# Boese0601/Dyadic-Interaction-Modeling

Hardware: AMD Instinct MI355X
Metric: listener clips/sec (T=300, EMOCA-56) (higher is better)
Workload: dtype bf16; 1 GPU; C3: B=256/GPU synthetic dyad clips, T=300, SLMFT.forward(mode='val'): listener VQ encode + encoder + 299-step AR decode (top-k 52 sampling) + VQ decode; global_batch=256, seq_len=300, gather=tokens+coeffs, gather_bytes_per_rank=17452032

## Files before the change

### dyadic-interaction-modeling_amd/csrc/common.hpp

```cpp
#pragma once
#include <hip/hip_runtime.h>
#include <stdint.h>
#include <stdio.h>
#include <string.h>
#include <string>

#include "../../include/dimx.h"

namespace dimx {

void set_error(const char* fmt, ...);
const char* get_error();

#define DIMX_HIP(expr)                                                                       \
    do {                                                                                     \
        hipError_t _e = (expr);                                                              \
        if (_e != hipSuccess) {                                                              \
            dimx::set_error("%s:%d: %s -> %s", __FILE__, __LINE__, #expr, hipGetErrorString(_e)); \
            return DIMX_ERR_HIP;                                                             \
        }                                                                                    \
    } while (0)

#define DIMX_REQUIRE(cond, code, ...)       \
    do {                                    \
// ... 75 lines not shown

template <int CTRL> __device__ __forceinline__ float dpp_f32(float v) {
    return __builtin_bit_cast(float, __builtin_amdgcn_update_dpp(0, __builtin_bit_cast(int, v), CTRL, 0xF, 0xF, true));
}
template <int CTRL> __device__ __forceinline__ int dpp_i32(int v) { return __builtin_amdgcn_update_dpp(0, v, CTRL, 0xF, 0xF, true); }
constexpr int DPP_XOR1 = 0xB1, DPP_XOR2 = 0x4E, DPP_HALF_MIRROR = 0x141, DPP_ROW_MIRROR = 0x140;
__device__ __forceinline__ float lane_f32(float v, int lane) {
    return __builtin_bit_cast(float, __builtin_amdgcn_readlane(__builtin_bit_cast(int, v), lane));
}
__device__ __forceinline__ int wave_lane() { return (int)__builtin_amdgcn_mbcnt_hi(~0u, __builtin_amdgcn_mbcnt_lo(~0u, 0u)); }
template <int O> __device__ __forceinline__ int xor_lane_i32(int v) {
    static_assert(O == 1 || O == 2 || O == 4 || O == 8 || O == 16 || O == 32, "xor distance");
    if constexpr (O == 1) {
        return __builtin_amdgcn_update_dpp(0, v, 0xB1, 0xF, 0xF, false);
    } else if constexpr (O == 2) {
        return __builtin_amdgcn_update_dpp(0, v, 0x4E, 0xF, 0xF, false);
    } else if constexpr (O == 4) {
        const int r = __builtin_amdgcn_update_dpp(0, v, 0x104, 0xF, 0x5, false);
        return __builtin_amdgcn_update_dpp(r, v, 0x114, 0xF, 0xA, false);
    } else if constexpr (O == 8) {
        return __builtin_amdgcn_update_dpp(0, v, 0x128, 0xF, 0xF, false);
    } else if constexpr (O == 16) {
        const auto r = __builtin_amdgcn_permlane16_swap((unsigned)v, (unsigned)v, false, false);
        return ((wave_lane() >> 4) & 1) ? (int)r[0] : (int)r[1];
    } else {
        const auto r = __builtin_amdgcn_permlane32_swap((unsigned)v, (unsigned)v, false, false);
        return wave_lane() >= 32 ? (int)r[0] : (int)r[1];
    }
}
template <int O> __device__ __forceinline__ float xor_lane_f32(float v) {
    return __builtin_bit_cast(float, xor_lane_i32<O>(__builtin_bit_cast(int, v)));
}

__device__ __forceinline__ float group8_sum(float v) {
    v += dpp_f32<DPP_XOR1>(v);
    v += dpp_f32<DPP_XOR2>(v);
    v += dpp_f32<DPP_HALF_MIRROR>(v);
    return v;
}
__device__ __forceinline__ float row16_sum(float v) {
    v = group8_sum(v);
    v += dpp_f32<DPP_ROW_MIRROR>(v);
    return v;
}
__device__ __forceinline__ void wave_argmax(float& v, int& i) {
#define DIMX_ARGMAX_STEP(OV, OI)                          \
    do {                                                  \
        const float ov_ = (OV);                           \
        const int oi_ = (OI);                             \
        if (ov_ > v || (ov_ == v && oi_ < i)) {           \
            v = ov_;                                      \
            i = oi_;                                      \
        }                                                 \
    } while (0)
    DIMX_ARGMAX_STEP(dpp_f32<DPP_XOR1>(v), dpp_i32<DPP_XOR1>(i));
    DIMX_ARGMAX_STEP(dpp_f32<DPP_XOR2>(v), dpp_i32<DPP_XOR2>(i));
    DIMX_ARGMAX_STEP(dpp_f32<DPP_HALF_MIRROR>(v), dpp_i32<DPP_HALF_MIRROR>(i));
    DIMX_ARGMAX_STEP(dpp_f32<DPP_ROW_MIRROR>(v), dpp_i32<DPP_ROW_MIRROR>(i));
    DIMX_ARGMAX_STEP(xor_lane_f32<16>(v), xor_lane_i32<16>(i));
    DIMX_ARGMAX_STEP(xor_lane_f32<32>(v), xor_lane_i32<32>(i));
#undef DIMX_ARGMAX_STEP
}
__device__ __forceinline__ float wave_max(float v) {
    v = fmaxf(v, dpp_f32<DPP_XOR1>(v));
    v = fmaxf(v, dpp_f32<DPP_XOR2>(v));
    v = fmaxf(v, dpp_f32<DPP_HALF_MIRROR>(v));
    v = fmaxf(v, dpp_f32<DPP_ROW_MIRROR>(v));
    return fmaxf(fmaxf(lane_f32(v, 0), lane_f32(v, 16)), fmaxf(lane_f32(v, 32), lane_f32(v, 48)));
}
__device__ __forceinline__ float wave_sum(float v) {
    v += xor_lane_f32<32>(v);
    v += xor_lane_f32<16>(v);
    v += xor_lane_f32<8>(v);
    v += xor_lane_f32<4>(v);
    v += xor_lane_f32<2>(v);
    v += xor_lane_f32<1>(v);
    return v;
}
__device__ __forceinline__ float wave_sum_fast(float v) {
    v = row16_sum(v);
    return (lane_f32(v, 0) + lane_f32(v, 16)) + (lane_f32(v, 32) + lane_f32(v, 48));
}
template <bool FAST> __device__ __forceinline__ float wave_sum_sel(float v) { return FAST ? wave_sum_fast(v) : wave_sum(v); }
template <int O> __device__ __forceinline__ double xor_lane_f64(double v) {
    const unsigned long long u = __builtin_bit_cast(unsigned long long, v);
    const unsigned lo = (unsigned)xor_lane_i32<O>((int)(unsigned)u), hi = (unsigned)xor_lane_i32<O>((int)(unsigned)(u >> 32));
    return __builtin_bit_cast(double, ((unsigned long long)hi << 32) | lo);
}
__device__ __forceinline__ double wave_sum_f64(double v) {
    v += xor_lane_f64<32>(v);
    v += xor_lane_f64<16>(v);
    v += xor_lane_f64<8>(v);
    v += xor_lane_f64<4>(v);
    v += xor_lane_f64<2>(v);
    v += xor_lane_f64<1>(v);
    return v;
}

inline int ceil_div(int a, int b) { return (a + b - 1) / b; }
inline size_t align_up(size_t x, size_t a) { return (x + a - 1) / a * a; }
inline int splitk_nonempty(int nk, int sp) {
    if (nk < 1 || sp < 1) return 1;
    if (sp > nk) sp = nk;
    return ceil_div(nk, ceil_div(nk, sp));
}

struct OutSeg {
    void* ptr;
    long sb, sh, st, sd;
    int D;
};

struct GemmArgs {
    int in_dtype, out_dtype;
    const void* A;
    int lda;
    const void* W;
    int ldw;
    int kloop;
    int M, N, K;
    int conv_T;
    const int32_t* conv_lens;
    int conv_C;
    const float* bias;
    int act;
    const float* residual;
    int ldr;
    const float* rowadd;
    int rowadd_mode;
    float rowadd_scale;
    int rowadd_off, ld_rowadd;
    int rowadd_div;
    int rowT;
    OutSeg seg[3];
    int nseg, seg_width;
    int allow_splitk;
    int splitk;
    int force_simple;
    int cfg;
    int force_splitk;
    int out_slabs;
    long slab_stride;
    int stage_out;
    const float* ln_stats;
    const float* ln_colsum;
    int ln_C;
    unsigned* ln_err;
    int w_tiled;
    const void* w3;
    long w3_plane;
    int x3_decode;
    int vt_pack4;
};

void gemm_args_init(GemmArgs& a);
void gemm_set_plain_out(GemmArgs& a, void* C, int ldc);
int launch_gemm(const GemmArgs& a, hipStream_t s);
bool gemm256_eligible(const GemmArgs& a);
int launch_gemm256(const GemmArgs& a, hipStream_t s);
int launch_gemm256_segs(const GemmArgs& a, const OutSeg* segs, int nseg, int seg_width, hipStream_t s);
bool gemm_use_x3(const GemmArgs& a);
bool gemm_x3_plan(const GemmArgs& a, int* bn_out, int* sp_out);
int launch_gemm_x3(const GemmArgs& a, hipStream_t s);
int launch_split_x3(const float* w, void* planes, size_t n, hipStream_t s);
int gemm_plan_splits(const GemmArgs& a);

int launch_layernorm(int out_dtype, const float* x, void* y, const float* gamma, const float* beta, int M,
                     int C, hipStream_t s);
int launch_add_slabs_layernorm(int out_dtype, float* x, const float* slabs, int nslab, long slab_stride, void* y,
                               const float* gamma, int M, int C, hipStream_t s);
int launch_instnorm(int out_dtype, const float* x, void* y, const int32_t* lens, int B, int T, int C,
                    hipStream_t s);

struct AttnArgs {
    int dtype;
    const void *q, *k, *vt;
    void* o;
    long q_sb, q_st, q_sh;
    long k_sb, k_st, k_sh;
    long v_sb, v_sh, v_sd;
    int v_rows;
    long v_st;
    long o_sb, o_st, o_sh;
    int B, H, Lq, Lk, D;
    float scale;
    int causal;
    const int32_t* lens;
    const uint8_t* kmask;
    int kmask_ld;
    unsigned long long* kwords;
    size_t kwords_cap;
    int kwords_ready;
};
int launch_pack_key_words(const uint8_t* kmask, int kmask_ld, const int32_t* lens, int B, int Lk, unsigned long long* words, size_t cap,
                          hipStream_t s);
int launch_attention(const AttnArgs& a, hipStream_t s);
int launch_attention_tr(const AttnArgs& a, hipStream_t s);
size_t mlp_fused_packed_bytes(int C, int F);
int mlp_fused_pack(const float* w1, const float* b1, const float* w2, int C, int F, uint16_t* out);
int launch_mlp_fused(float* x, const void* packed, const float* b2, const float* ln_g, const float* ln_b, int M, int C, int F, int act,
                     hipStream_t s);

struct DecodeAttnArgs {
    int dtype;
    const void* q;
    int q_ld;
    int q_f32;
    int nslab;
    long slab_stride;
    int force_nsplit;
    int rows_per_clip;
    const void* knew;
    const void* vnew;
    int kv_ld;
    void* kcache;
    void* vcache;
    int Tmax;
    void* out;
    int o_ld;
    int B, H;
    const int32_t* step;
    int n_keys;
    const uint8_t* kmask;
    int kmask_ld;
    float scale;
    const void* tab;
    int tab_ld, tab_koff, tab_voff, tab_rows;
    const int32_t* hist;
    int hist_ld;
    int win, lookahead;
};
int launch_decode_attn(const DecodeAttnArgs& a, hipStream_t s);

int launch_vq_argmin(const float* z, int N, const float* Et , const float* ee ,
                     int32_t* idx, float* best_d, float* margin, hipStream_t s);

struct ChainGemmDesc {
    const void* W;
    int N, K, ldw;
    int cols, rows_pad, ncb, nkt;
};
struct ChainArgs {
    int B;
    ChainGemmDesc g1;
    const void* A1;
    int lda1;
    float* xr;
    float* x;
    int C;
    const float* slabs;
    int nslab;
    long slab_stride;
    void* y;
    const float* gamma;
    ChainGemmDesc g2;
    float* out2;
    int ld_out2;
    unsigned* counters;
    unsigned* seen;
    const int32_t* step;
    unsigned* err;
    int defer;
    float* stats;
    const float* colsum2;
    int nbar;
    int fault;
    int offA1, offW1, offRed1, offA2, offW2, offRed2;
};
struct LayerChainArgs {
    int B, C;
    DecodeAttnArgs sa, ca;
    ChainGemmDesc g_so, g_cq, g_co;
    const void* o;
    int ld_o;
    float* x;
    void* y;
    float* stats;
    const float* colsum_cq;
    float* qc;
    int ld_qc;
    unsigned* counters;
    unsigned* seen;
    const int32_t* step;
    int epoch_add;
    unsigned* err;
    int fault;
    unsigned long long* prof;
    int sc_stride;
    int off_base, off_A1, off_W1, off_A2, off_W2, off_W3, off_A3;
};
bool layer_chain_supported(const LayerChainArgs& a, int cu_count);
int launch_layer_chain(const LayerChainArgs& a, hipStream_t s);
size_t chain_plan(ChainArgs& a);
bool chain_supported(const ChainArgs& a, int cu_count);
int launch_chain(const ChainArgs& a, hipStream_t s);

int launch_cast_pad(int out_dtype, const float* x, int ldx, const float* coladd, void* y, int ldy, int M, int K,
                    hipStream_t s, const uint8_t* zero_rows = nullptr);
int launch_gather_rows(int out_dtype, const float* table, int ld_table, int rows, const int32_t* idx, void* y,
                       int ldy, int M, int C, hipStream_t s);
constexpr int kLstmSave = 6;
size_t lstm_scratch_bytes(int B, int T, int In);
int lstm_layer_run(const float* x, int B, int T, int In, int H, const float* const* w_ih, const float* const* w_hh,
                   const float* const* b_ih, const float* const* b_hh, float* y, void* scratch, size_t scratch_bytes, int flags,
                   int cu_count, int* fault_count, hipStream_t st, float* save = nullptr);
size_t lstm_bwd_scratch_bytes(int B, int T);
int lstm_bwd_run(const float* dy, const float* save, const float* const* w_hh, int B, int T, float* dgates, void* scratch,
                 size_t scratch_bytes, int flags, int cu_count, int* fault_count, hipStream_t st);
int launch_context_concat(int out_dtype, const float* x_s, const float* patch, const float* audio, void* ctx,
                          int M, int dim, int dim_a, hipStream_t s);
int launch_finalize_idx(int32_t* idx, const int32_t* lens, int B, int T, int32_t pad_value, hipStream_t s,
                        int fqn = 1);
int launch_shift_tokens(const int32_t* z, int32_t* inp, int32_t* tgt, int B, int T, hipStream_t s);
int launch_ce_argmax(const float* logits, const int32_t* target, float* row_loss, int32_t* argmax_tok, int R,
                     int V, hipStream_t s);
struct SampleFilter {
    int kind = 0;
    float a = 0.f, b = 0.f;
    uint8_t* keep_out = nullptr;
};
struct SampleArgs {
    const float* logits = nullptr;
    int ld_logits = 0, R = 0, top_k = 0;
    float temperature = 0.f;
    const float* noise = nullptr;
    uint64_t seed = 0;
    const int32_t* step_dev = nullptr;
    uint64_t step_host = 0;
    int32_t* tokens = nullptr;
    int tok_ld = 0, tok_col_from_step = 0, nslab = 0;
    long slab_stride = 0;
    float* logits_out = nullptr;
    int logits_out_ld = 0, row0 = 0, rows_total = 0;
    const float* emb_table = nullptr;
    int emb_C = 0;
    float* x_next = nullptr;
    int32_t* step_rw = nullptr;
    unsigned* done_ctr = nullptr;
    const float* pos_table = nullptr;
    float pos_scale = 0.f;
    int pos_rows = 0;
    const int32_t* dev_params = nullptr;
    void* y_next = nullptr;
    const float* y_gamma = nullptr;
    int y_dtype = DIMX_F32;
    const float* qkv0_table = nullptr;
    float* qkv0_out = nullptr;
    int qkv0_N = 0;
    const int32_t* prompt = nullptr;
    int prompt_ld = 0, prompt_max = 0;
    const int32_t* prompt_len = nullptr;
    int prompt_div = 1;
    int32_t* epoch_rw = nullptr;
    SampleFilter filt;
    int32_t* hist = nullptr;
    int hist_ld = 0;
};
int launch_sample(const SampleArgs& a, hipStream_t s);
struct BeamSelectArgs {
    const float* logits = nullptr;
    int nslab = 1;
    long slab_stride = 0;
    int nclip = 0, W = 0;
    const int32_t* step_dev = nullptr;
    int step_host = 0;
    int32_t* step_rw = nullptr;
    unsigned* done_ctr = nullptr;
    int32_t* epoch_rw = nullptr;
    const int32_t* dev_params = nullptr;
    const int32_t* prompt = nullptr;
    int prompt_ld = 0, prompt_max = 0;
    const int32_t* prompt_len = nullptr;
    const int32_t* lens = nullptr;
    int len_off = 0;
    const int32_t* mode = nullptr;
    const int32_t* forced_tok = nullptr;
    const double* cum_in = nullptr;
    double* cum_out = nullptr;
    int32_t* parent = nullptr;
    int32_t* tokens = nullptr;
    int32_t* backptr = nullptr;
    int tok_ld = 1;
    float* logits_out = nullptr;
    const float* emb_table = nullptr;
    int emb_C = 0;
    float* x_next = nullptr;
    const float* qkv0_table = nullptr;
    float* qkv0_out = nullptr;
    int qkv0_N = 0;
};
bool beam_width_supported(int W);
int launch_beam_select(const BeamSelectArgs& a, hipStream_t s);
struct BeamReorderArgs {
// ... 37 lines not shown
```

### dyadic-interaction-modeling_amd/csrc/mlp_fused.hip

```cpp
#include "common.hpp"

namespace dimx {
namespace {

typedef unsigned u32x4_t __attribute__((ext_vector_type(4)));
typedef __attribute__((address_space(3))) void lds_void_t;
typedef const __attribute__((address_space(1))) void glb_void_t;

constexpr int kC = 384;
constexpr int kKS = kC / 16;
constexpr int kOB = kC / 32;
constexpr int kW1Frags = kKS + 1;
constexpr int kW2Frags = 2 * kOB;
constexpr int kChunkBytes = (kW1Frags + kW2Frags) * 1024;
constexpr int kStages = 3;

template <int ACT> __device__ __forceinline__ float gelu_fast(float x) {
    if (ACT == ACT_GELU_TANH) {
        const float t = x * x;
        const float p = __builtin_fmaf(t, -0.10294324f, -2.3022082f);
        const float e = __builtin_amdgcn_exp2f(x * p);
        return x * __builtin_amdgcn_rcpf(1.0f + e);
    }
    const float t = __builtin_amdgcn_rcpf(__builtin_fmaf(fabsf(x), 0.33267253f, 1.0f));
    const float poly = t * (0.1740121f + t * (-0.0479399f + t * 0.3739278f));
    const float q = poly * __builtin_amdgcn_exp2f(x * x * -0.72134752f);
    return __builtin_fmaf(-fabsf(x), q, fmaxf(x, 0.f));
}

template <int OFF> __device__ __forceinline__ void ds_read128(u32x4_t& v, unsigned addr) {
    asm volatile("ds_read_b128 %0, %1 offset:%2" : "=v"(v) : "v"(addr), "i"(OFF));
}

struct MlpArgs {
    float* x;
    const void* wp;
    const float* b2;
    const float* ln_g;
    const float* ln_b;
    int M, nchunk;
};

template <int ACT, bool BETA> __global__ __launch_bounds__(256) void mlp_fused_kernel(const MlpArgs a) {
    extern __shared__ __attribute__((aligned(1024))) unsigned char smem[];
    const int tid = threadIdx.x, wave = __builtin_amdgcn_readfirstlane(tid >> 6), lane = tid & 63, hf = lane >> 5, l31 = lane & 31;
    const int row = blockIdx.x * 128 + wave * 32 + l31;
    const int rowc = row < a.M ? row : a.M - 1;
    const unsigned lds0 = (unsigned)(size_t)(lds_void_t*)smem;
    const unsigned char* wp = (const unsigned char*)a.wp;

    unsigned char* const ring1 = smem;
    unsigned char* const ring2 = smem + kStages * kW1Frags * 1024;
    const unsigned char* const wlane = wp + lane * 16;
    auto issue_piece = [&](int j, int chunk1, int slot1, int chunk2, int slot2) {
        if (j < 6) {
            const int p = wave + 4 * j;
            __builtin_amdgcn_global_load_lds((glb_void_t*)(wlane + (size_t)chunk1 * kChunkBytes + (size_t)p * 1024),
                                             (lds_void_t*)(ring1 + slot1 * (kW1Frags * 1024) + p * 1024), 16, 0, 0);
        } else if (j < 12) {
            const int p = wave + 4 * (j - 6);
            __builtin_amdgcn_global_load_lds((glb_void_t*)(wlane + (size_t)chunk2 * kChunkBytes + (size_t)(kW1Frags + p) * 1024),
                                             (lds_void_t*)(ring2 + slot2 * (kW2Frags * 1024) + p * 1024), 16, 0, 0);
        } else if (wave == 0) {
            __builtin_amdgcn_global_load_lds((glb_void_t*)(wlane + (size_t)chunk1 * kChunkBytes + (size_t)(kW1Frags - 1) * 1024),
                                             (lds_void_t*)(ring1 + slot1 * (kW1Frags * 1024) + (kW1Frags - 1) * 1024), 16, 0, 0);
        }
    };
    const int nch = a.nchunk;
    auto wrap = [&](int c) { return c < nch ? c : (c - nch < nch ? c - nch : 0); };
    auto issue_preloop = [&]() {
#pragma unroll
        for (int j = 0; j < 13; ++j) issue_piece(j, 0, 0, 0, 0);
#pragma unroll
        for (int j = 0; j < 13; ++j) issue_piece(j, wrap(1), 1, wrap(1), 1);
#pragma unroll
        for (int j = 0; j < 13; ++j)
            if (j < 6 || j == 12) issue_piece(j, wrap(2), 2, 0, 0);
    };
    issue_preloop();

    bf16x8_t xb[kKS + 1];
    f32x16_t o[kOB];
    {
        const float* xr = a.x + (size_t)rowc * kC + 8 * hf;
        f32x4_t v[kKS][2];
#pragma unroll
        for (int s = 0; s < kKS; ++s) {
            v[s][0] = *(const f32x4_t*)(xr + 16 * s);
            v[s][1] = *(const f32x4_t*)(xr + 16 * s + 4);
        }
        float s1 = 0.f;
#pragma unroll
        for (int s = 0; s < kKS; ++s)
#pragma unroll
            for (int j = 0; j < 4; ++j) s1 += v[s][0][j] + v[s][1][j];
        s1 += __shfl_xor(s1, 32);
        const float mean = s1 * (1.0f / kC);
        float s2 = 0.f;
#pragma unroll
        for (int s = 0; s < kKS; ++s)
#pragma unroll
            for (int j = 0; j < 4; ++j) {
                const float d0 = v[s][0][j] - mean, d1 = v[s][1][j] - mean;
                s2 += d0 * d0 + d1 * d1;
            }
        s2 += __shfl_xor(s2, 32);
        const float rstd = rsqrtf(s2 * (1.0f / kC) + 1e-5f);
        const float* g = a.ln_g + 8 * hf;
        const float* be = a.ln_b + 8 * hf;
#pragma unroll
        for (int s = 0; s < kKS; ++s) {
            const f32x4_t g0 = *(const f32x4_t*)(g + 16 * s), g1 = *(const f32x4_t*)(g + 16 * s + 4);
            f32x4_t b0 = {0.f, 0.f, 0.f, 0.f}, b1 = {0.f, 0.f, 0.f, 0.f};
            if (BETA) {
                b0 = *(const f32x4_t*)(be + 16 * s);
                b1 = *(const f32x4_t*)(be + 16 * s + 4);
            }
            const f32x4_t v0 = v[s][0], v1 = v[s][1];
            uint32_t w[4];
#pragma unroll
            for (int j = 0; j < 2; ++j) {
                w[j] = pack_bf16x2((v0[2 * j] - mean) * rstd * g0[2 * j] + b0[2 * j], (v0[2 * j + 1] - mean) * rstd * g0[2 * j + 1] + b0[2 * j + 1]);
                w[2 + j] = pack_bf16x2((v1[2 * j] - mean) * rstd * g1[2 * j] + b1[2 * j], (v1[2 * j + 1] - mean) * rstd * g1[2 * j + 1] + b1[2 * j + 1]);
            }
            const u32x4_t u = {w[0], w[1], w[2], w[3]};
            xb[s] = __builtin_bit_cast(bf16x8_t, u);
// ... 18 lines not shown
        const unsigned base = rd1 + slot * (kW1Frags * 1024);
#pragma unroll
        for (int r = 0; r < 16; ++r) h[r] = 0.f;
        u32x4_t fr[2][5];
#pragma unroll
        for (int q = 0; q < 5; ++q) asm volatile("ds_read_b128 %0, %1 offset:%2" : "=v"(fr[0][q]) : "v"(base), "i"(q * 1024));
#pragma unroll
        for (int g = 0; g < 5; ++g) {
            if (g + 1 < 5) {
#pragma unroll
                for (int q = 0; q < 5; ++q)
                    asm volatile("ds_read_b128 %0, %1 offset:%2" : "=v"(fr[(g + 1) & 1][q]) : "v"(base), "i"(((g + 1) * 5 + q) * 1024));
                asm volatile("s_waitcnt lgkmcnt(5)" ::: "memory");
            } else {
                asm volatile("s_waitcnt lgkmcnt(0)" ::: "memory");
            }
            __builtin_amdgcn_sched_barrier(0);
#pragma unroll
            for (int q = 0; q < 5; ++q)
                h = __builtin_amdgcn_mfma_f32_32x32x16_bf16(__builtin_bit_cast(bf16x8_t, fr[g & 1][q]), xb[g * 5 + q], h, 0, 0, 0);
        }
    };
    auto gelu_pair = [&](const f32x16_t& h, int r) { return pack_bf16x2(gelu_fast<ACT>(h[2 * r]), gelu_fast<ACT>(h[2 * r + 1])); };

    f32x16_t h_mid, h_next;
    uint32_t hbc[8], hbn[8];
    asm volatile("s_waitcnt vmcnt(0)" ::: "memory");
    __builtin_amdgcn_s_barrier();
    gemm1(0, h_next);
#pragma unroll
    for (int r = 0; r < 8; ++r) hbc[r] = gelu_pair(h_next, r);
    gemm1(1, h_mid);

    int s0 = 0, s2 = 2;
    for (int c = 0; c < nch; ++c) {
        asm volatile("s_waitcnt vmcnt(6)" ::: "memory");
        __builtin_amdgcn_s_barrier();
        const int cw1 = wrap(c + 3), cw2 = wrap(c + 2);
        const unsigned b1 = rd1 + s2 * (kW1Frags * 1024);
        const unsigned b2 = rd2 + s0 * (kW2Frags * 1024);
#pragma unroll
        for (int r = 0; r < 16; ++r) h_next[r] = 0.f;
        u32x4_t fr[3][4], fbias;
        asm volatile("ds_read_b128 %0, %1 offset:%2" : "=v"(fbias) : "v"(b1), "i"(kKS * 1024));
#pragma unroll
        for (int gg = 0; gg < 2; ++gg)
#pragma unroll
            for (int q = 0; q < 2; ++q) {
                asm volatile("ds_read_b128 %0, %1 offset:%2" : "=v"(fr[gg][q]) : "v"(b1), "i"((2 * gg + q) * 1024));
                asm volatile("ds_read_b128 %0, %1 offset:%2" : "=v"(fr[gg][2 + q]) : "v"(b2), "i"((2 * gg + q) * 1024));
            }
        issue_piece(12, cw1, s0, cw2, s2);
#pragma unroll
        for (int g = 0; g < kOB; ++g) {
            if (g + 2 < kOB) {
#pragma unroll
                for (int q = 0; q < 2; ++q) {
                    asm volatile("ds_read_b128 %0, %1 offset:%2" : "=v"(fr[(g + 2) % 3][q]) : "v"(b1), "i"((2 * (g + 2) + q) * 1024));
                    asm volatile("ds_read_b128 %0, %1 offset:%2" : "=v"(fr[(g + 2) % 3][2 + q]) : "v"(b2), "i"((2 * (g + 2) + q) * 1024));
                }
                asm volatile("s_waitcnt lgkmcnt(8)" ::: "memory");
            } else if (g + 1 < kOB) {
                asm volatile("s_waitcnt lgkmcnt(4)" ::: "memory");
            } else {
                asm volatile("s_waitcnt lgkmcnt(0)" ::: "memory");
            }
            __builtin_amdgcn_sched_barrier(0);
            const u32x4_t c0 = {hbc[0], hbc[1], hbc[2], hbc[3]}, c1v = {hbc[4], hbc[5], hbc[6], hbc[7]};
            if (g == 0) h_next = __builtin_amdgcn_mfma_f32_32x32x16_bf16(__builtin_bit_cast(bf16x8_t, fbias), xb[kKS], h_next, 0, 0, 0);
            h_next = __builtin_amdgcn_mfma_f32_32x32x16_bf16(__builtin_bit_cast(bf16x8_t, fr[g % 3][0]), xb[2 * g], h_next, 0, 0, 0);
            h_next = __builtin_amdgcn_mfma_f32_32x32x16_bf16(__builtin_bit_cast(bf16x8_t, fr[g % 3][1]), xb[2 * g + 1], h_next, 0, 0, 0);
            issue_piece(g, cw1, s0, cw2, s2);
            o[g] = __builtin_amdgcn_mfma_f32_32x32x16_bf16(__builtin_bit_cast(bf16x8_t, fr[g % 3][2]), __builtin_bit_cast(bf16x8_t, c0), o[g], 0, 0, 0);
            o[g] = __builtin_amdgcn_mfma_f32_32x32x16_bf16(__builtin_bit_cast(bf16x8_t, fr[g % 3][3]), __builtin_bit_cast(bf16x8_t, c1v), o[g], 0, 0, 0);
            if (g >= 2 && g < 10) hbn[g - 2] = gelu_pair(h_mid, g - 2);
        }
#pragma unroll
        for (int r = 0; r < 8; ++r) hbc[r] = hbn[r];
        h_mid = h_next;
        s0 = s0 == 2 ? 0 : s0 + 1;
        s2 = s2 == 2 ? 0 : s2 + 1;
    }

    if (row < a.M) {
        float* xr = a.x + (size_t)row * kC + 4 * hf;
#pragma unroll
        for (int ob = 0; ob < kOB; ++ob)
#pragma unroll
            for (int q = 0; q < 4; ++q) {
                float* p = xr + 32 * ob + 8 * q;
                f32x4_t v = {0.f, 0.f, 0.f, 0.f};
                v = *(const f32x4_t*)p;
#pragma unroll
                for (int t = 0; t < 4; ++t) v[t] += o[ob][4 * q + t];
                *(f32x4_t*)p = v;
            }
    }
}

}

size_t mlp_fused_packed_bytes(int C, int F) { return (C == kC && F % 32 == 0) ? (size_t)(F / 32) * kChunkBytes : 0; }

int mlp_fused_pack(const float* w1, const float* b1, const float* w2, int C, int F, uint16_t* out) {
    DIMX_REQUIRE(C == kC && F % 32 == 0, DIMX_ERR_ARG, "mlp_fused_pack: C = %d F = %d not supported", C, F);
    auto bf = [](uint16_t b) {
        const uint32_t u = (uint32_t)b << 16;
        float f;
        memcpy(&f, &u, 4);
        return f;
    };
    for (int c = 0; c < F / 32; ++c) {
        uint16_t* img = out + (size_t)c * (kChunkBytes / 2);
        for (int s = 0; s < kW1Frags; ++s)
            for (int l = 0; l < 64; ++l)
                for (int j = 0; j < 8; ++j) {
                    const int h = 32 * c + (l & 31), half = l >> 5;
                    uint16_t v = 0;
                    if (s < kKS) {
                        v = host_f32_to_bf16(w1[(size_t)h * C + 16 * s + 8 * half + j]);
                    } else if (half == 0 && j < 2) {
                        const uint16_t hi = host_f32_to_bf16(b1 ? b1[h] : 0.f);
                        v = j == 0 ? hi : host_f32_to_bf16((b1 ? b1[h] : 0.f) - bf(hi));
                    }
                    img[(size_t)s * 512 + l * 8 + j] = v;
                }
        for (int ob = 0; ob < kOB; ++ob)
            for (int s2 = 0; s2 < 2; ++s2)
                for (int l = 0; l < 64; ++l)
                    for (int j = 0; j < 8; ++j) {
                        const int o = 32 * ob + (l & 31), half = l >> 5;
                        const int hid = 32 * c + (2 * s2 + j / 4) * 8 + 4 * half + j % 4;
                        img[(size_t)(kW1Frags + 2 * ob + s2) * 512 + l * 8 + j] = host_f32_to_bf16(w2[(size_t)o * F + hid]);
                    }
    }
    return DIMX_OK;
}

int launch_mlp_fused(float* x, const void* packed, const float* b2, const float* ln_g, const float* ln_b, int M, int C, int F, int act,
                     hipStream_t s) {
    DIMX_REQUIRE(x && packed && b2 && ln_g && M > 0, DIMX_ERR_ARG, "mlp_fused: null argument");
    DIMX_REQUIRE(C == kC && F % 32 == 0 && (act == ACT_GELU_TANH || act == ACT_GELU_ERF), DIMX_ERR_ARG, "mlp_fused: C = %d F = %d act = %d", C, F, act);
    DIMX_REQUIRE(((uintptr_t)x % 16) == 0 && ((uintptr_t)packed % 16) == 0 && ((uintptr_t)b2 % 16) == 0 && ((uintptr_t)ln_g % 16) == 0 &&
                     (!ln_b || ((uintptr_t)ln_b % 16) == 0),
                 DIMX_ERR_ARG, "mlp_fused: operands must be 16-byte aligned");
    MlpArgs a;
    a.x = x; a.wp = packed; a.b2 = b2; a.ln_g = ln_g; a.ln_b = ln_b; a.M = M; a.nchunk = F / 32;
    DIMX_REQUIRE(a.nchunk >= 3, DIMX_ERR_ARG, "mlp_fused: F = %d is too small for the three-deep pipeline", F);
    const size_t lds = (size_t)kStages * kChunkBytes;
    const dim3 grid((M + 127) / 128);
#define MLP_LAUNCH(A, B)                                                                                                              \
    do {                                                                                                                              \
                             \
        DIMX_HIP(hipFuncSetAttribute((const void*)mlp_fused_kernel<A, B>, hipFuncAttributeMaxDynamicSharedMemorySize, (int)lds)); \
        hipLaunchKernelGGL((mlp_fused_kernel<A, B>), grid, dim3(256), lds, s, a);                                                     \
    } while (0)
    if (act == ACT_GELU_TANH) {
        if (ln_b) MLP_LAUNCH(ACT_GELU_TANH, true); else MLP_LAUNCH(ACT_GELU_TANH, false);
    } else {
        if (ln_b) MLP_LAUNCH(ACT_GELU_ERF, true); else MLP_LAUNCH(ACT_GELU_ERF, false);
    }
#undef MLP_LAUNCH
    DIMX_HIP(hipGetLastError());
    return DIMX_OK;
}

}
```

### dyadic-interaction-modeling_amd/csrc/model.hip

```cpp
#include <stdarg.h>
#include <stdlib.h>
#include <set>

#include "model.hpp"

namespace dimx {

static thread_local char g_err[1024] = "";
void set_error(const char* fmt, ...) {
    va_list ap;
    va_start(ap, fmt);
    vsnprintf(g_err, sizeof(g_err), fmt, ap);
    va_end(ap);
}
const char* get_error() { return g_err; }

static std::string vq_prefix(int which) { return which == 0 ? "speaker_vq." : "listener_vq."; }

struct KeySpec {
    std::string name;
    std::vector<int64_t> shape;
};

static void vq_keys(const dimx_dims& d, int which, std::vector<KeySpec>& out) {
// ... 567 lines not shown

static bool qkv_row_v(int at, int D) {
    return at == DIMX_BF16 && D <= 64;
}

static void set_qkv_out(GemmArgs& g, void* q, void* k, void* vt, int T, int H, int D, int Tp, bool rowv = false) {
    const int segw = H * D;
    g.rowT = T;
    g.nseg = 3;
    g.seg_width = segw;
    for (int i = 0; i < (rowv ? 3 : 2); ++i) {
        g.seg[i].ptr = i == 0 ? q : (i == 1 ? k : vt);
        g.seg[i].sb = (long)T * segw;
        g.seg[i].st = segw;
        g.seg[i].sh = D;
        g.seg[i].sd = 1;
        g.seg[i].D = D;
    }
    if (rowv) return;
    g.seg[2].ptr = vt;
    g.seg[2].sb = (long)H * D * Tp;
    g.seg[2].sh = (long)D * Tp;
    g.seg[2].sd = Tp;
    g.seg[2].st = 1;
    g.seg[2].D = D;
}

static void set_attn_packed(AttnArgs& a, int dtype, const void* q, const void* k, const void* vt, void* o, int B,
                            int H, int Lq, int Lk, int D, int Tp_k, bool rowv = false) {
    memset(&a, 0, sizeof(a));
    const int segw = H * D;
    a.dtype = dtype;
    a.q = q;
    a.k = k;
    a.vt = vt;
    a.o = o;
    a.q_sb = (long)Lq * segw;
    a.q_st = segw;
    a.q_sh = D;
    a.k_sb = (long)Lk * segw;
    a.k_st = segw;
    a.k_sh = D;
    a.v_sb = (long)H * D * Tp_k;
    a.v_sh = (long)D * Tp_k;
    a.v_sd = Tp_k;
    if (rowv) {
        a.v_rows = 1;
        a.v_sb = (long)Lk * segw;
        a.v_st = segw;
        a.v_sh = D;
    }
    a.o_sb = (long)Lq * segw;
    a.o_st = segw;
    a.o_sh = D;
    a.B = B;
    a.H = H;
    a.Lq = Lq;
    a.Lk = Lk;
    a.D = D;
}

struct BlockBufs {
    float* h;
    void *y, *q, *k, *vt, *o, *f;
    unsigned long long* kw = nullptr;
    size_t kw_cap = 0;
};

static int linear(const dimx_ctx* c, const void* A, int lda, const Linear& L, int M, int out_dtype, void* out, int ldo, hipStream_t st,
                  int act = ACT_NONE, const float* residual = nullptr) {
    GemmArgs g;
    gemm_lin(c, A, lda, L, M, g);
    g.out_dtype = out_dtype; g.act = act;
    g.residual = residual; g.ldr = residual ? ldo : 0;
    gemm_set_plain_out(g, out, ldo);
    return launch_gemm(g, st);
}
static int residual_linear(const dimx_ctx* c, const void* A, int lda, const Linear& L, int M, float* h, int ld, hipStream_t st) {
    return linear(c, A, lda, L, M, DIMX_F32, h, ld, st, ACT_NONE, h);
}

constexpr int kFusedMlpMinRows = 8192;

static int ff_sublayer(const dimx_ctx* c, const BlockBufs& b, const float* ln_g, const float* ln_b, const Linear& f1,
                       const Linear& f2, const void* mlp, int act, int M, int C, hipStream_t st) {
    if (mlp && M >= kFusedMlpMinRows) return launch_mlp_fused(b.h, mlp, f2.bias, ln_g, ln_b, M, C, f1.N, act, st);
    DIMX_TRY(launch_layernorm(c->at, b.h, b.y, ln_g, ln_b, M, C, st));
    DIMX_TRY(linear(c, b.y, C, f1, M, c->at, b.f, f1.N, st, act));
    return residual_linear(c, b.f, f1.N, f2, M, b.h, C, st);
}

static int self_attn_qkv(const dimx_ctx* c, const BlockBufs& b, const float* ln_g, const float* ln_b, const Linear& qkv, int B,
                         int T, int C, int heads, int D, AttnArgs& a, hipStream_t st) {
    const bool rowv = qkv_row_v(c->at, D);
    DIMX_TRY(launch_layernorm(c->at, b.h, b.y, ln_g, ln_b, B * T, C, st));
    GemmArgs g;
    gemm_lin(c, b.y, C, qkv, B * T, g);
    g.out_dtype = c->at;
    set_qkv_out(g, b.q, b.k, b.vt, T, heads, D, tpad(T), rowv);
    DIMX_TRY(launch_gemm(g, st));
    set_attn_packed(a, c->at, b.q, b.k, b.vt, b.o, B, heads, T, T, D, tpad(T), rowv);
    return DIMX_OK;
}

static int attn_out(const dimx_ctx* c, const BlockBufs& b, AttnArgs& a, const Linear& out, int C, hipStream_t st) {
    a.kwords = b.kw; a.kwords_cap = b.kw_cap;
    DIMX_TRY(launch_attention(a, st));
    return residual_linear(c, b.o, a.H * a.D, out, a.B * a.Lq, b.h, C, st);
}

static int cross_attn_sublayer(const dimx_ctx* c, const BlockBufs& b, const XAttn& x, AttnArgs& a, const uint8_t* ctx_mask, int C,
                               hipStream_t st, const float* v_rows = nullptr) {
    const int M = a.B * a.Lq, Tp = tpad(a.Lk);
    DIMX_TRY(launch_layernorm(c->at, b.h, b.y, x.ln_g, nullptr, M, C, st));
    DIMX_TRY(linear(c, b.y, C, x.qkv, M, c->at, b.q, a.H * a.D, st));
    if (v_rows) DIMX_TRY(launch_kv_rows_to_vt(v_rows, Tp, (float*)a.vt, Tp, a.B, a.Lk, a.H, st));
    a.scale = 1.0f / sqrtf((float)a.D); a.kmask = ctx_mask; a.kmask_ld = a.Lk;
    return attn_out(c, b, a, x.out, C, st);
}

struct VQScratch : BlockBufs {
    void *xa, *h1;
    float *conv, *z;
    int32_t* idx_tmp;
};

static void plan_vq(const dimx_ctx* c, const VQGeom& vg, Arena& ar, int B, int T, VQScratch& s) {
    const size_t M = (size_t)B * T, es = es_of(c);
    const int H = vg.hidden, I = vg.inter, Tp = tpad(T);
    s.xa = ar.take(M * (vg.in_pad > 128 ? vg.in_pad : 128) * es);
    s.h1 = ar.take(M * H * es);
    s.conv = (float*)ar.take(M * H * 4);
    s.y = ar.take(M * H * es);
    s.h = (float*)ar.take(M * H * 4);
    s.q = ar.take(M * H * es);
    s.k = ar.take(M * H * es);
    s.vt = ar.take((size_t)B * H * Tp * es);
    s.o = ar.take(M * H * es);
    s.f = ar.take(M * I * es);
    s.z = (float*)ar.take(M * vg.out_dim * 4);
    s.idx_tmp = (int32_t*)ar.take(M * vg.fqn * 4);
}

static int run_vq_blocks(const dimx_ctx* c, const VQGeom& vg, const VQBlock* blk, VQScratch& s, int B, int T,
                         const int32_t* lens, hipStream_t st) {
    const int M = B * T, Hd = vg.hidden, heads = vg.heads, D = Hd / heads;
    const float scale = 1.0f / sqrtf((float)Hd);
    for (int l = 0; l < vg.layers; ++l) {
        const VQBlock& b = blk[l];
        AttnArgs a;
        DIMX_TRY(self_attn_qkv(c, s, b.ln1_g, b.ln1_b, b.qkv, B, T, Hd, heads, D, a, st));
        a.scale = scale; a.lens = lens;
        DIMX_TRY(attn_out(c, s, a, b.out, Hd, st));
        DIMX_TRY(ff_sublayer(c, s, b.ln2_g, b.ln2_b, b.l1, b.l2, b.mlp, ACT_GELU_TANH, M, Hd, st));
    }
    return DIMX_OK;
}

static int run_vq_front(const dimx_ctx* c, const VQGeom& vg, const void* x_in, int ld_in, const Linear& conv,
                        const Linear& le, const float* pe, int pe_mode, int row_off, VQScratch& s, int B, int T,
                        const int32_t* lens, hipStream_t st, int row_div = 1) {
    const int M = B * T, Hd = vg.hidden;
    GemmArgs g;
    gemm_lin(c, x_in, ld_in, conv, M, g);
    g.conv_T = T;
    g.conv_lens = lens;
    g.conv_C = Hd;
    g.act = ACT_LEAKY;
    g.out_dtype = DIMX_F32;
    gemm_set_plain_out(g, s.conv, Hd);
    DIMX_TRY(launch_gemm(g, st));
    DIMX_TRY(launch_instnorm(c->at, s.conv, s.y, lens, B, T, Hd, st));
    gemm_lin(c, s.y, Hd, le, M, g);
    g.out_dtype = DIMX_F32;
    g.rowT = T;
    g.rowadd = pe;
    g.ld_rowadd = Hd;
    g.rowadd_mode = pe_mode == 0 ? 3 : 2;
    g.rowadd_off = pe_mode == 0 ? 0 : row_off;
    g.rowadd_div = row_div;
    gemm_set_plain_out(g, s.h, Hd);
    DIMX_TRY(launch_gemm(g, st));
    return DIMX_OK;
}

static int run_vq_encode(const dimx_ctx* c, int which, const float* x, const int32_t* lens, int B, int T, int pe_mode,
                         int row_off, VQScratch& s, float* z, int32_t* idx, hipStream_t st) {
    const VQGeom& vg = c->vqg[which];
    const VQNet& v = c->vq[which];
    const int M = B * T, Hd = vg.hidden;
    DIMX_TRY(launch_cast_pad(c->at, x, vg.in_dim, nullptr, s.xa, vg.in_pad, M, vg.in_dim, st));
    DIMX_TRY(linear(c, s.xa, vg.in_pad, v.vm, M, c->at, s.h1, Hd, st, ACT_LEAKY));
    DIMX_TRY(run_vq_front(c, vg, s.h1, Hd, v.conv, v.le, v.pe_enc, pe_mode, row_off, s, B, T, lens, st));
    DIMX_TRY(run_vq_blocks(c, vg, v.enc, s, B, T, lens, st));
    DIMX_TRY(launch_cast_pad(c->at, s.h, Hd, nullptr, s.y, Hd, M, Hd, st));
    DIMX_TRY(linear(c, s.y, Hd, v.post, M, DIMX_F32, z, vg.out_dim, st));
    DIMX_TRY(launch_vq_argmin(z, M * vg.fqn, v.Et, v.ee, idx, nullptr, nullptr, st));
    return DIMX_OK;
}

}

using namespace dimx;

extern "C" {

int dimx_version(void) { return 100; }
const char* dimx_last_error(void) { return get_error(); }

void dimx_legacy_dims(dimx_dims* d) {
    if (!d) return;
    dimx_default_dims(d);
    d->variant = 1;
    d->dim_in = 1024; d->dim = 512; d->dim_a = 0; d->enc_depth = 6; d->dec_depth = 6; d->heads = 8;
    d->max_seq_len = 1024;
    d->spk_in_dim = 824; d->spk_hidden = 768; d->spk_heads = 8; d->spk_inter = 1536; d->spk_face_quan_num = 8;
}

void dimx_default_dims(dimx_dims* d) {
    if (!d) return;
    memset(d, 0, sizeof(*d));
    d->vq_in_dim = 56; d->vq_hidden = 384; d->vq_layers = 6; d->vq_heads = 8; d->vq_inter = 1536;
    d->vq_n_embed = 512; d->vq_zdim = 128;
    d->dim_in = 56; d->dim = 384; d->dim_a = 768; d->enc_depth = 4; d->dec_depth = 4; d->heads = 12;
    d->dim_head = 64; d->num_tokens = 512; d->max_seq_len = 2048; d->ff_mult = 4;
}

int dimx_create(dimx_handle* h, int device_id, const dimx_dims* dims, int numeric_mode) {
    DIMX_REQUIRE(h, DIMX_ERR_ARG, "dimx_create: null handle pointer");
    DIMX_REQUIRE(numeric_mode == DIMX_MODE_PARITY_F32 || numeric_mode == DIMX_MODE_PERF_BF16, DIMX_ERR_ARG,
                 "dimx_create: numeric_mode %d", numeric_mode);
    dimx_dims d;
    dimx_default_dims(&d);
    if (dims) d = *dims;
    DIMX_REQUIRE(d.vq_hidden == 384 && d.vq_heads == 8 && d.vq_zdim == 128 && d.vq_n_embed == 512 && d.vq_in_dim == 56,
                 DIMX_ERR_ARG, "dimx_create: only the DIM-Listener VQ geometry (56/384/8/128/512) is built");
    if (d.variant == 0 || d.variant == 2) {
        DIMX_REQUIRE(d.dim == 384 && d.dim_a == 768 && d.dim_head == 64 && d.heads == 12 && d.num_tokens == 512 &&
                         d.vq_layers <= 8 && d.enc_depth <= 8 && d.dec_depth <= 8 && d.max_seq_len <= 2048,
                     DIMX_ERR_ARG, "dimx_create: only the SLMFT geometry (384+768, 12x64, 512 tokens) is built");
    } else {
        DIMX_REQUIRE(d.variant == 1 && d.dim == 512 && d.dim_a == 0 && d.dim_head == 64 && d.heads == 8 &&
                         d.num_tokens == 512 && d.enc_depth <= 8 && d.dec_depth <= 8 && d.max_seq_len <= 2048 &&
                         d.spk_hidden == 768 && d.spk_heads == 8 && d.spk_in_dim == 824 && d.spk_face_quan_num == 8,
                     DIMX_ERR_ARG, "dimx_create: only the legacy ListenerGenerator geometry (824/768 VQ, 512, 8x64) is built");
    }
    DIMX_REQUIRE(d.mesh_dim == 0 || (d.variant == 2 && d.mesh_dim > 0), DIMX_ERR_ARG,
                 "dimx_create: the mesh head (mesh_dim %d) belongs to a handle of variant 2", d.mesh_dim);
    int ndev = 0;
    DIMX_HIP(hipGetDeviceCount(&ndev));
    DIMX_REQUIRE(device_id >= 0 && device_id < ndev, DIMX_ERR_ARG, "dimx_create: device %d of %d", device_id, ndev);
    DIMX_HIP(hipSetDevice(device_id));
    dimx_ctx* c = new dimx_ctx();
    c->device = device_id;
    c->d = d;
    c->mode = numeric_mode;
    c->at = numeric_mode == DIMX_MODE_PERF_BF16 ? DIMX_BF16 : DIMX_F32;
    c->variant = d.variant;
    const VQGeom lvq = {d.vq_in_dim, 64, d.vq_hidden, d.vq_heads, d.vq_inter, d.vq_layers, d.vq_zdim, 1, d.vq_zdim,
                        d.vq_n_embed, true};
    c->vqg[0] = c->vqg[1] = lvq;
    if (d.variant == 1) {
        c->vqg[0] = {d.spk_in_dim, (d.spk_in_dim + 63) / 64 * 64, d.spk_hidden, d.spk_heads, d.spk_inter, d.vq_layers,
                     d.spk_face_quan_num * d.vq_zdim, d.spk_face_quan_num, d.vq_zdim, d.vq_n_embed, false};
        const int din = d.spk_face_quan_num * d.vq_zdim;
        c->encg[0] = c->encg[1] = {din, din, d.dim, d.heads, d.dim_head, d.enc_depth, d.ff_mult, 0};
        c->decg = {d.dim, d.heads, d.dim_head, d.dec_depth, d.ff_mult, 1, d.num_tokens, d.dim};
    } else {
        const int causal = d.variant == 2 ? 0 : 1, abs_pos = d.variant == 2 ? 1 : 0;
        c->encg[0] = {d.dim_in, 64, d.dim, d.heads, d.dim_head, d.enc_depth, d.ff_mult, causal};
        c->encg[1] = {d.dim, d.dim, d.dim, d.heads, d.dim_head, d.enc_depth, d.ff_mult, causal};
        c->decg = {d.dim + d.dim_a, d.heads, d.dim_head, d.dec_depth, d.ff_mult, abs_pos, d.num_tokens, d.dim + d.dim_a};
    }
    for (const auto& k : all_keys(d)) c->required.push_back(k.name);
    const char* ng = getenv("DIMX_NO_GRAPH");
    c->use_graph = (ng && ng[0] == '1') ? 0 : 1;
    const char* nc = getenv("DIMX_NO_CHAIN");
    c->use_chain = (nc && nc[0] == '1') ? 0 : 1;
    c->use_layer_chain = getenv("DIMX_NO_LAYER_CHAIN") ? 0 : 1;
    c->multi_tr = getenv("DIMX_NO_MULTI_TR") ? 0 : 1;
    c->use_qkv0_table = getenv("DIMX_NO_QKV0_TABLE") ? 0 : 1;
    c->use_kv0_table = getenv("DIMX_NO_KV0_TABLE") ? 0 : 1;
    if (getenv("DIMX_LAYER_PROF")) {
        void* p = nullptr;
        if (hipMalloc(&p, (size_t)8 * 256 * 16 * 8) == hipSuccess) {
            (void)hipMemset(p, 0, (size_t)8 * 256 * 16 * 8);
            c->layer_prof_dev = (unsigned long long*)p;
        }
    }
    if (const char* pg = getenv("DIMX_PREFILL_GROUPS")) {
        const int v = atoi(pg);
        if (v >= 1 && v <= dimx_ctx::kPreGroups) c->prefill_groups = v;
    }
    {
        int cus = 0;
        if (hipDeviceGetAttribute(&cus, hipDeviceAttributeMultiprocessorCount, device_id) == hipSuccess) c->cu_count = cus;
    }
    const char* gg = getenv("DIMX_GEN_GROUPS");
    if (gg && atoi(gg) >= 1 && atoi(gg) <= dimx_ctx::kMaxGroups) c->gen_groups = atoi(gg);
    *h = c;
    return DIMX_OK;
}

int dimx_destroy(dimx_handle h) {
    if (!h) return DIMX_OK;
    (void)hipSetDevice(h->device);
    for (int g = 0; g < dimx_ctx::kMaxGroups; ++g) {
        if (h->graph_multi[g]) (void)hipGraphExecDestroy(h->graph_multi[g]);
        if (h->graph_exec[g]) (void)hipGraphExecDestroy(h->graph_exec[g]);
        if (h->grp_stream[g]) (void)hipStreamDestroy(h->grp_stream[g]);
        if (h->ev_join[g]) (void)hipEventDestroy(h->ev_join[g]);
    }
    if (h->ev_fork) (void)hipEventDestroy(h->ev_fork);
    for (int g = 0; g < dimx_ctx::kPreGroups - 1; ++g) {
        if (h->pre_stream[g]) (void)hipStreamDestroy(h->pre_stream[g]);
        if (h->pre_join[g]) (void)hipEventDestroy(h->pre_join[g]);
    }
    if (h->pre_fork) (void)hipEventDestroy(h->pre_fork);
    if (h->cap_stream) (void)hipStreamDestroy(h->cap_stream);
    if (h->chain_err_ev) (void)hipEventDestroy(h->chain_err_ev);
    if (h->chain_err_dev) (void)hipFree(h->chain_err_dev);
    if (h->chain_stats_dev) (void)hipFree(h->chain_stats_dev);
    if (h->layer_prof_dev) (void)hipFree(h->layer_prof_dev);
    if (h->qkv0_table) (void)hipFree(h->qkv0_table);
    if (h->kv0_image) (void)hipFree(h->kv0_image);
    if (h->chain_err_host) (void)hipHostFree(h->chain_err_host);
    free_packed(h);
    train_forget(h);
    delete h;
    return DIMX_OK;
}

int dimx_numeric_mode(dimx_handle h) { return h ? h->mode : DIMX_ERR_ARG; }

int dimx_set_shard(dimx_handle h, int row_offset, int rows_total) {
    DIMX_REQUIRE(h, DIMX_ERR_ARG, "set_shard: null handle");
    DIMX_REQUIRE(row_offset >= 0 && (rows_total == 0 || rows_total > row_offset), DIMX_ERR_ARG,
                 "set_shard: row_offset %d, rows_total %d", row_offset, rows_total);
    h->shard_row_off = row_offset;
    h->shard_rows_total = rows_total;
    return DIMX_OK;
}

int dimx_begin_checkpoint(dimx_handle h) {
    DIMX_REQUIRE(h, DIMX_ERR_ARG, "dimx_begin_checkpoint: null handle");
    std::set<std::string> spec;
    for (const auto& k : all_keys(h->d)) spec.insert(k.name);
    bool dirty = false;
    for (auto it = h->host.begin(); it != h->host.end();) {
        if (!spec.count(it->first)) {
            it = h->host.erase(it);
            dirty = true;
        } else {
            ++it;
        }
    }
    if (dirty) {
        (void)hipSetDevice(h->device);
        (void)hipDeviceSynchronize();
        free_packed(h);
        h->graph_valid = false;
        h->ctx_ready = false;
    }
// ... 222 lines not shown
    s.xs = ar.take((size_t)B * T * c->encg[0].dim * es);
    s.xl = ar.take((size_t)B * T * c->encg[0].dim * es);
    s.xj = ar.take((size_t)B * 2 * T * c->encg[0].dim * es);
    s.m2 = (uint8_t*)ar.take((size_t)B * 2 * T);
}

static size_t workspace_bytes(const dimx_ctx* c, int B, int T, int S = 1) {
    Arena p(nullptr, 0);
    CtxPersist cp;
    plan_persist(c, p, B, T, cp);
    const size_t persist = align_up(p.off, 256);
    size_t scratch = 0;
    for (int w = 0; w < 2; ++w) {
        Arena a(nullptr, 0);
        VQScratch s;
        plan_vq(c, c->vqg[w], a, B, T, s);
        scratch = a.off > scratch ? a.off : scratch;
    }
    {
        Arena a(nullptr, 0);
        EncScratch s;
        plan_enc(c, a, B, T, s);
        if (c->variant == 0) a.take((size_t)B * T * c->decg.ctx_dim * es_of(c));
        if (c->variant == 1) {
            VQScratch v;
            plan_vq(c, c->vqg[0], a, B, T, v);
            a.take((size_t)B * 4);
        }
        scratch = a.off > scratch ? a.off : scratch;
    }
    if (c->variant == 2) {
        Arena a(nullptr, 0);
        SlmScratch s;
        plan_slm(c, a, B, T, s);
        scratch = a.off > scratch ? a.off : scratch;
    }
    if (c->d.mesh_dim > 0) {
        Arena a(nullptr, 0);
        MeshScratch s;
        plan_mesh(c, a, B, T, s);
        scratch = a.off > scratch ? a.off : scratch;
    }
    if (T >= 2) {
        Arena a(nullptr, 0);
        DecScratch s;
        plan_dec(c, a, B, T, s);
        scratch = a.off > scratch ? a.off : scratch;
        Arena g(nullptr, 0);
        GenScratch gs;
        plan_gen(c, g, B * S, T, gs);
        scratch = g.off > scratch ? g.off : scratch;
    }
    return persist + align_up(scratch, 256) + 4096 + 65536;
}

static size_t workspace_bytes_prompt(const dimx_ctx* c, int B, int T, int S, int P0) {
    const size_t base = workspace_bytes(c, B, T, S);
    if (P0 <= 1 || T < 2) return base;
    Arena p(nullptr, 0);
    CtxPersist cp;
    plan_persist(c, p, B, T, cp);
    Arena g(nullptr, 0);
    GenScratch gs;
    plan_gen(c, g, B * S, T, gs);
    PrefillScratch ps;
    plan_prefill(c, g, B, P0 - 1, T, ps);
    const size_t need = align_up(p.off, 256) + align_up(g.off, 256) + 4096 + 65536;
    return need > base ? need : base;
}

static int run_xenc(const dimx_ctx* c, const EncGeom& eg, const XEnc& e, const void* x_in, int ld_in, EncScratch& s,
                    int B, int T, const uint8_t* mask, int out_dtype, void* out, hipStream_t st) {
    const int M = B * T, dim = eg.dim, heads = eg.heads, D = eg.dim_head;
    GemmArgs g;
    gemm_lin(c, x_in, ld_in, e.proj_in, M, g);
    g.out_dtype = DIMX_F32;
    g.rowT = T;
    g.rowadd = e.pos_emb;
    g.ld_rowadd = dim;
    g.rowadd_mode = 1;
    g.rowadd_scale = 1.0f / sqrtf((float)dim);
    gemm_set_plain_out(g, s.h, dim);
    DIMX_TRY(launch_gemm(g, st));
    for (int l = 0; l < eg.depth; ++l) {
        AttnArgs a;
        DIMX_TRY(self_attn_qkv(c, s, e.attn[l].ln_g, nullptr, e.attn[l].qkv, B, T, dim, heads, D, a, st));
        a.scale = 1.0f / sqrtf((float)D); a.causal = eg.causal; a.kmask = mask; a.kmask_ld = T;
        DIMX_TRY(attn_out(c, s, a, e.attn[l].out, dim, st));
        DIMX_TRY(ff_sublayer(c, s, e.ff[l].ln_g, nullptr, e.ff[l].f1, e.ff[l].f2, e.ff[l].mlp, ACT_GELU_ERF, M, dim, st));
    }
    DIMX_TRY(launch_layernorm(out_dtype, s.h, out, e.final_g, nullptr, M, dim, st));
    return DIMX_OK;
}

static int check_common(dimx_handle h, int B, int T, void* ws, size_t ws_bytes, int need, int S = 1) {
    DIMX_REQUIRE(h, DIMX_ERR_ARG, "null handle");
    DIMX_REQUIRE(B >= 1 && T >= 1 && T <= h->d.max_seq_len, DIMX_ERR_ARG, "B=%d T=%d out of range (T <= %d)", B, T,
                 h->d.max_seq_len);
    DIMX_REQUIRE(ws && ((uintptr_t)ws % 256) == 0, DIMX_ERR_ARG, "workspace must be 256-byte aligned");
    const size_t need_bytes = workspace_bytes(h, B, T, S);
    DIMX_REQUIRE(ws_bytes >= need_bytes, DIMX_ERR_WORKSPACE, "workspace %zu < required %zu", ws_bytes, need_bytes);
    DIMX_HIP(hipSetDevice(h->device));
    DIMX_TRY(ensure_packed(h, need));
    return DIMX_OK;
}

int project_cross_kv(dimx_handle h, const void* ctx, const CtxPersist& cp, int B, int T, int for_generate,
                     hipStream_t st);
int legacy_encode_ctx(dimx_handle h, const float* v_speaker, const uint8_t* mask, int B, int T, int for_generate,
                      float* enc_out, float* x_speaker_out, int32_t* idx_out, void* ws, size_t ws_bytes,
                      hipStream_t st);

struct ClipGroups {
    int G;
    int b0[dimx_ctx::kPreGroups + 1];
    hipStream_t st[dimx_ctx::kPreGroups];
};
static int clip_groups_fork(dimx_handle h, int B, int T, hipStream_t st, ClipGroups& cg, bool one_group = false) {
    int G = one_group ? 1 : h->prefill_groups;
    if (G == 0) {
        const size_t rows = (size_t)B * T;
        G = rows > 196608 ? 1 : rows >= 32768 ? 4 : rows >= 16384 ? 2 : 1;
    }
    if (G > B) G = B;
    cg.G = G;
    for (int g = 0; g <= G; ++g) cg.b0[g] = (int)((long)B * g / G);
    cg.st[0] = st;
    if (G == 1) return DIMX_OK;
    {
        hipStreamCaptureStatus cs = hipStreamCaptureStatusNone;
        if (hipStreamIsCapturing(st, &cs) != hipSuccess || cs != hipStreamCaptureStatusNone) {
            (void)hipGetLastError();
            cg.G = 1;
            cg.b0[1] = B;
            return DIMX_OK;
        }
        if (hipStreamQuery(st) != hipSuccess) (void)hipStreamSynchronize(st);
        (void)hipGetLastError();
    }
    if (!h->pre_fork) DIMX_HIP(hipEventCreateWithFlags(&h->pre_fork, hipEventDisableTiming));
    DIMX_HIP(hipEventRecord(h->pre_fork, st));
    for (int g = 1; g < G; ++g) {
        if (!h->pre_stream[g - 1]) DIMX_HIP(hipStreamCreateWithFlags(&h->pre_stream[g - 1], hipStreamNonBlocking));
        if (!h->pre_join[g - 1]) DIMX_HIP(hipEventCreateWithFlags(&h->pre_join[g - 1], hipEventDisableTiming));
        cg.st[g] = h->pre_stream[g - 1];
        DIMX_HIP(hipStreamWaitEvent(cg.st[g], h->pre_fork, 0));
    }
    return DIMX_OK;
}
static int clip_groups_join(dimx_handle h, const ClipGroups& cg) {
    hipError_t bad = hipSuccess;
    for (int g = 1; g < cg.G; ++g) {
        hipError_t e = hipEventRecord(h->pre_join[g - 1], cg.st[g]);
        if (e == hipSuccess) e = hipStreamWaitEvent(cg.st[0], h->pre_join[g - 1], 0);
        if (e != hipSuccess) {
            (void)hipStreamSynchronize(cg.st[g]);
            bad = e;
        }
    }
    DIMX_HIP(bad);
    return DIMX_OK;
}

static int clip_groups_close(dimx_handle h, const ClipGroups& cg, int rc) {
    const int jrc = clip_groups_join(h, cg);
    return rc != DIMX_OK ? rc : jrc;
}

static Arena scratch_arena(const dimx_ctx* c, void* ws, size_t ws_bytes, int B, int T, CtxPersist* cp) {
    Arena p(ws, ws_bytes);
    CtxPersist tmp;
    plan_persist(c, p, B, T, cp ? *cp : tmp);
    const size_t persist = align_up(p.off, 256);
    return Arena((unsigned char*)ws + persist, ws_bytes - persist);
// ... 13 lines not shown
    return workspace_bytes(h, B, T, n_samples);
}

size_t dimx_workspace_bytes_prompt(dimx_handle h, int B, int T, int n_samples, int P0) {
    if (!h || B < 1 || T < 1 || n_samples < 1 || T > h->d.max_seq_len || P0 < 1 || P0 > (T > 1 ? T - 1 : 1)) return 0;
    return workspace_bytes_prompt(h, B, T, n_samples, P0);
}

int dimx_vq_argmin(dimx_handle h, int which, const float* z, int N, int32_t* idx, float* best_d, float* margin,
                   void* stream) {
    DIMX_REQUIRE(h && (which == 0 || which == 1), DIMX_ERR_ARG, "vq_argmin: bad handle/which");
    DIMX_HIP(hipSetDevice(h->device));
    DIMX_TRY(ensure_packed(h, which == 0 ? COMP_VQ0 : COMP_VQ1));
    return launch_vq_argmin(z, N, h->vq[which].Et, h->vq[which].ee, idx, best_d, margin, (hipStream_t)stream);
}

int dimx_vq_encode(dimx_handle h, int which, const float* x, const int32_t* lens, int B, int T, int pe_mode,
                   int batch_row_offset, int32_t pad_value, int32_t* idx, float* z_out, void* ws, size_t ws_bytes,
                   void* stream) {
    DIMX_REQUIRE(which == 0 || which == 1, DIMX_ERR_ARG, "vq_encode: which must be 0 or 1");
    DIMX_TRY(check_common(h, B, T, ws, ws_bytes, which == 0 ? COMP_VQ0 : COMP_VQ1));
    DIMX_REQUIRE(x && idx, DIMX_ERR_ARG, "vq_encode: null argument");
    DIMX_REQUIRE(pe_mode == 0 || B + batch_row_offset <= 5000, DIMX_ERR_ARG, "vq_encode: positional row out of range");
    hipStream_t st = (hipStream_t)stream;
    const VQGeom& vg = h->vqg[which];
    Arena ar = scratch_arena(h, ws, ws_bytes, B, T, nullptr);
    ClipGroups cg;
    DIMX_TRY(clip_groups_fork(h, B, T, st, cg));
    VQScratch s[dimx_ctx::kPreGroups];
    for (int g = 0; g < cg.G; ++g) plan_vq(h, vg, ar, cg.b0[g + 1] - cg.b0[g], T, s[g]);
    const int rc = [&]() -> int {
        DIMX_REQUIRE(!ar.overflow, DIMX_ERR_WORKSPACE, "vq_encode: workspace overflow");
        for (int g = 0; g < cg.G; ++g) {
            const int b0 = cg.b0[g], nb = cg.b0[g + 1] - b0;
            const size_t r0 = (size_t)b0 * T;
            DIMX_TRY(run_vq_encode(h, which, x + r0 * vg.in_dim, lens ? lens + b0 : nullptr, nb, T, pe_mode, batch_row_offset + b0, s[g],
                                   z_out ? z_out + r0 * vg.out_dim : s[g].z, idx + r0 * vg.fqn, cg.st[g]));
        }
        return DIMX_OK;
    }();
    DIMX_TRY(clip_groups_close(h, cg, rc));
    DIMX_TRY(launch_finalize_idx(idx, lens, B, T, pad_value, st, vg.fqn));
    return DIMX_OK;
}

static int vq_decode_impl(dimx_handle h, int which, const int32_t* idx, const float* z, int B, int L,
                          int batch_row_offset, int rows_per_clip, float* out, void* ws, size_t ws_bytes, void* stream) {
    DIMX_REQUIRE(which == 0 || which == 1, DIMX_ERR_ARG, "vq_decode: which must be 0 or 1");
    DIMX_TRY(check_common(h, B, L, ws, ws_bytes, which == 0 ? COMP_VQ0 : COMP_VQ1));
    DIMX_REQUIRE((idx || z) && out, DIMX_ERR_ARG, "vq_decode: null argument");
    DIMX_REQUIRE(B + batch_row_offset <= 5000 && batch_row_offset >= 0, DIMX_ERR_ARG,
                 "vq_decode: positional row %d out of range", B + batch_row_offset);
    hipStream_t st = (hipStream_t)stream;
    const VQNet& v = h->vq[which];
    const VQGeom& vg = h->vqg[which];
    DIMX_REQUIRE(vg.has_decoder, DIMX_ERR_ARG, "vq_decode: this variant's VQ-VAE %d has no decoder on the path", which);
    DIMX_REQUIRE(rows_per_clip >= 1, DIMX_ERR_ARG, "vq_decode: rows_per_clip must be >= 1");
    Arena ar = scratch_arena(h, ws, ws_bytes, B, L, nullptr);
    ClipGroups cg;
    if (rows_per_clip == 1) {
        DIMX_TRY(clip_groups_fork(h, B, L, st, cg));
    } else {
        cg.G = 1;
        cg.b0[0] = 0;
        cg.b0[1] = B;
        cg.st[0] = st;
    }
    VQScratch sg[dimx_ctx::kPreGroups];
    for (int g = 0; g < cg.G; ++g) plan_vq(h, vg, ar, cg.b0[g + 1] - cg.b0[g], L, sg[g]);
    const int Hd = vg.hidden, zd = vg.zdim;
    const int rc = [&]() -> int {
    DIMX_REQUIRE(!ar.overflow, DIMX_ERR_WORKSPACE, "vq_decode: workspace overflow");
    for (int gi = 0; gi < cg.G; ++gi) {
        VQScratch& s = sg[gi];
        hipStream_t gs = cg.st[gi];
        const int b0 = cg.b0[gi], nb = cg.b0[gi + 1] - b0, M = nb * L;
        const size_t r0 = (size_t)b0 * L;
        if (idx)
            DIMX_TRY(launch_gather_rows(h->at, v.E, zd, vg.n_embed, idx + r0, s.xa, zd, M, zd, gs));
        else
            DIMX_TRY(launch_cast_pad(h->at, z + r0 * zd, zd, nullptr, s.xa, zd, M, zd, gs));
        DIMX_TRY(linear(h, s.xa, zd, v.pre, M, h->at, s.h1, Hd, gs));
        DIMX_TRY(run_vq_front(h, vg, s.h1, Hd, v.dconv, v.dle, v.pe_dec, 1, batch_row_offset + b0, s, nb, L, nullptr, gs, rows_per_clip));
        DIMX_TRY(run_vq_blocks(h, vg, v.dec, s, nb, L, nullptr, gs));
        DIMX_TRY(launch_cast_pad(h->at, s.h, Hd, nullptr, s.y, Hd, M, Hd, gs));
        DIMX_TRY(linear(h, s.y, Hd, v.rev, M, DIMX_F32, out + r0 * vg.in_dim, vg.in_dim, gs));
    }
    return DIMX_OK;
    }();
    return clip_groups_close(h, cg, rc);
}

int dimx_vq_decode(dimx_handle h, int which, const int32_t* idx, int B, int L, int batch_row_offset, int rows_per_clip,
                   float* out, void* ws, size_t ws_bytes, void* stream) {
    DIMX_REQUIRE(idx, DIMX_ERR_ARG, "vq_decode: null argument");
    return vq_decode_impl(h, which, idx, nullptr, B, L, batch_row_offset, rows_per_clip, out, ws, ws_bytes, stream);
}

int dimx_vq_decode_latent(dimx_handle h, int which, const float* z, int B, int L, int batch_row_offset, float* out,
                          void* ws, size_t ws_bytes, void* stream) {
    DIMX_REQUIRE(z, DIMX_ERR_ARG, "vq_decode_latent: null argument");
    return vq_decode_impl(h, which, nullptr, z, B, L, batch_row_offset, 1, out, ws, ws_bytes, stream);
}

int dimx_encode_speaker(dimx_handle h, const float* v_speaker, const uint8_t* mask, int B, int T, float* x_s_out, void* ws,
                        size_t ws_bytes, void* stream) {
    DIMX_REQUIRE(h && h->variant == 0, DIMX_ERR_ARG, "encode_speaker: SLMFT variant only");
    DIMX_TRY(check_common(h, B, T, ws, ws_bytes, COMP_ENC));
    DIMX_REQUIRE(v_speaker && mask && x_s_out, DIMX_ERR_ARG, "encode_speaker: null argument");
    hipStream_t st = (hipStream_t)stream;
    Arena ar = scratch_arena(h, ws, ws_bytes, B, T, nullptr);
    EncScratch s;
    plan_enc(h, ar, B, T, s);
    DIMX_REQUIRE(!ar.overflow, DIMX_ERR_WORKSPACE, "encode_speaker: workspace overflow");
    const int M = B * T, dim = h->d.dim;
    DIMX_TRY(launch_cast_pad(h->at, v_speaker, h->d.dim_in, h->patch_s, s.xa, 64, M, h->d.dim_in, st));
    DIMX_TRY(run_xenc(h, h->encg[0], h->enc_s, s.xa, 64, s, B, T, mask, h->at, s.xa, st));
    DIMX_TRY(run_xenc(h, h->encg[1], h->enc_joint, s.xa, dim, s, B, T, mask, DIMX_F32, s.tmp, st));
    DIMX_TRY(launch_layernorm(DIMX_F32, s.tmp, x_s_out, h->norm_s_g, h->norm_s_b, M, dim, st));
    h->ctx_ready = false;
    return DIMX_OK;
}

int dimx_encode_ctx(dimx_handle h, const float* v_speaker, const float* v_audio, const uint8_t* mask, int B, int T,
                    int for_generate, float* x_s_out, void* ws, size_t ws_bytes, void* stream) {
    DIMX_REQUIRE(!h || h->variant != 2, DIMX_ERR_ARG,
                 "encode_ctx: the SLM variant builds its contexts with dimx_slm_encode + dimx_set_context");
    if (h && h->variant == 1)
        return legacy_encode_ctx(h, v_speaker, mask, B, T, for_generate, x_s_out, nullptr, nullptr, ws, ws_bytes,
                                 (hipStream_t)stream);
    DIMX_TRY(check_common(h, B, T, ws, ws_bytes, COMP_ENC | COMP_DEC));
    DIMX_REQUIRE(v_speaker && v_audio && mask, DIMX_ERR_ARG, "encode_ctx: null argument");
    hipStream_t st = (hipStream_t)stream;
    CtxPersist cp;
    Arena ar = scratch_arena(h, ws, ws_bytes, B, T, &cp);
    const int dim = h->d.dim, dim_a = h->d.dim_a;
    ClipGroups cg;
    DIMX_TRY(clip_groups_fork(h, B, T, st, cg, h->decg.ctx_dim < h->encg[0].in_pad));
    EncScratch sg[dimx_ctx::kPreGroups];
    void* xa_all = nullptr;
    const size_t xa_row = (size_t)h->decg.ctx_dim * es_of(h);
    if (cg.G > 1) xa_all = ar.take((size_t)B * T * xa_row);
    for (int g = 0; g < cg.G; ++g) {
        plan_enc(h, ar, cg.b0[g + 1] - cg.b0[g], T, sg[g]);
        if (cg.G > 1) sg[g].xa = (unsigned char*)xa_all + (size_t)cg.b0[g] * T * xa_row;
    }
    const int grc = [&]() -> int {
    DIMX_REQUIRE(!ar.overflow, DIMX_ERR_WORKSPACE, "encode_ctx: workspace overflow");
    for (int gi = 0; gi < cg.G; ++gi) {
        EncScratch& s = sg[gi];
        hipStream_t gs = cg.st[gi];
        const int b0 = cg.b0[gi], nb = cg.b0[gi + 1] - b0, M = nb * T;
        const size_t r0 = (size_t)b0 * T;
        const uint8_t* gmask = mask + r0;
        DIMX_TRY(launch_cast_pad(h->at, v_speaker + r0 * h->d.dim_in, h->d.dim_in, h->patch_s, s.xa, 64, M, h->d.dim_in, gs));
        DIMX_TRY(run_xenc(h, h->encg[0], h->enc_s, s.xa, 64, s, nb, T, gmask, h->at, s.xa, gs));
        DIMX_TRY(run_xenc(h, h->encg[1], h->enc_joint, s.xa, dim, s, nb, T, gmask, DIMX_F32, s.tmp, gs));
        float* x_s = x_s_out ? x_s_out + r0 * dim : (float*)s.h;
        DIMX_TRY(launch_layernorm(DIMX_F32, s.tmp, x_s, h->norm_s_g, h->norm_s_b, M, dim, gs));
        DIMX_TRY(launch_context_concat(h->at, x_s, h->patch_dec_s, v_audio + r0 * dim_a, s.xa, M, dim, dim_a, gs));
    }
    return DIMX_OK;
    }();
    DIMX_TRY(clip_groups_close(h, cg, grc));
    DIMX_TRY(project_cross_kv(h, sg[0].xa, cp, B, T, for_generate, st));
    h->ctx_ready = true;
    h->ctx_B = B;
    h->ctx_T = T;
    h->ctx_for_generate = for_generate ? 1 : 0;
    h->ctx_ws = ws;
    return DIMX_OK;
}

int dimx_legacy_speaker_features(dimx_handle h, const float* v_speaker, const uint8_t* mask, int B, int T,
                                 float* x_speaker_out, int32_t* idx_out, void* ws, size_t ws_bytes, void* stream) {
    DIMX_REQUIRE(h && h->variant == 1, DIMX_ERR_ARG, "legacy_speaker_features: handle is not the legacy variant");
    DIMX_REQUIRE(x_speaker_out || idx_out, DIMX_ERR_ARG, "legacy_speaker_features: no output requested");
    return legacy_encode_ctx(h, v_speaker, mask, B, T, -1, nullptr, x_speaker_out, idx_out, ws, ws_bytes,
                             (hipStream_t)stream);
}

int dimx_slm_encode(dimx_handle h, const float* v_speaker, const float* v_listener, const uint8_t* mask,
                    const uint8_t* mask_speaker, const uint8_t* mask_listener, int B, int T, float* x_s, float* x_l,
                    float* x_joint, void* ws, size_t ws_bytes, void* stream) {
    DIMX_REQUIRE(h && h->variant == 2, DIMX_ERR_ARG, "slm_encode: handle is not the SLM variant");
    DIMX_TRY(check_common(h, B, T, ws, ws_bytes, COMP_ENC));
    DIMX_REQUIRE(2 * T <= h->d.max_seq_len, DIMX_ERR_ARG, "slm_encode: 2T=%d exceeds max_seq_len", 2 * T);
    DIMX_REQUIRE(v_speaker && v_listener && mask && x_s && x_l && x_joint, DIMX_ERR_ARG, "slm_encode: null argument");
    hipStream_t st = (hipStream_t)stream;
    Arena ar = scratch_arena(h, ws, ws_bytes, B, T, nullptr);
    SlmScratch s;
    plan_slm(h, ar, B, T, s);
    DIMX_REQUIRE(!ar.overflow, DIMX_ERR_WORKSPACE, "slm_encode: workspace overflow");
    const int M = B * T, dim = h->encg[0].dim;
    const size_t es = es_of(h), rowb = (size_t)T * dim * es;
    const EncGeom& e0 = h->encg[0];
    const EncGeom& e1 = h->encg[1];
    DIMX_TRY(launch_cast_pad(h->at, v_speaker, h->d.dim_in, h->patch_s, s.e.xa, e0.in_pad, M, h->d.dim_in, st, mask_speaker));
    DIMX_TRY(run_xenc(h, e0, h->enc_s, s.e.xa, e0.in_pad, s.e, B, T, mask, h->at, s.xs, st));
    DIMX_TRY(launch_cast_pad(h->at, v_listener, h->d.dim_in, h->patch_l, s.e.xa, e0.in_pad, M, h->d.dim_in, st, mask_listener));
    DIMX_TRY(run_xenc(h, e0, h->enc_l, s.e.xa, e0.in_pad, s.e, B, T, mask, h->at, s.xl, st));
    DIMX_HIP(hipMemcpy2DAsync(s.xj, 2 * rowb, s.xs, rowb, rowb, B, hipMemcpyDeviceToDevice, st));
    DIMX_HIP(hipMemcpy2DAsync((unsigned char*)s.xj + rowb, 2 * rowb, s.xl, rowb, rowb, B, hipMemcpyDeviceToDevice, st));
    DIMX_HIP(hipMemcpy2DAsync(s.m2, 2 * T, mask, T, T, B, hipMemcpyDeviceToDevice, st));
    DIMX_HIP(hipMemcpy2DAsync(s.m2 + T, 2 * T, mask, T, T, B, hipMemcpyDeviceToDevice, st));
    DIMX_TRY(run_xenc(h, e1, h->enc_joint, s.xj, dim, s.e, B, 2 * T, s.m2, DIMX_F32, s.e.tmp, st));
    DIMX_TRY(launch_layernorm(DIMX_F32, s.e.tmp, x_joint, h->norm_j_g, h->norm_j_b, 2 * M, dim, st));
    DIMX_TRY(run_xenc(h, e1, h->enc_joint, s.xl, dim, s.e, B, T, mask, DIMX_F32, s.e.tmp, st));
    DIMX_TRY(launch_layernorm(DIMX_F32, s.e.tmp, x_l, h->norm_l_g, h->norm_l_b, M, dim, st));
    DIMX_TRY(run_xenc(h, e1, h->enc_joint, s.xs, dim, s.e, B, T, mask, DIMX_F32, s.e.tmp, st));
    DIMX_TRY(launch_layernorm(DIMX_F32, s.e.tmp, x_s, h->norm_s_g, h->norm_s_b, M, dim, st));
    h->ctx_ready = false;
    return DIMX_OK;
}

int dimx_set_context(dimx_handle h, const float* x, int ldx_rows, int which_patch, const float* v_audio, int B, int T,
                     int for_generate, void* ws, size_t ws_bytes, void* stream) {
    DIMX_REQUIRE(h && h->variant != 1, DIMX_ERR_ARG, "set_context: not available for the legacy variant");
    DIMX_TRY(check_common(h, B, T, ws, ws_bytes, COMP_ENC | COMP_DEC));
    DIMX_REQUIRE(x && v_audio && (which_patch == 0 || (which_patch == 1 && h->variant == 2)) && ldx_rows >= T,
                 DIMX_ERR_ARG, "set_context: bad argument");
    hipStream_t st = (hipStream_t)stream;
    CtxPersist cp;
    Arena ar = scratch_arena(h, ws, ws_bytes, B, T, &cp);
    EncScratch s;
    plan_enc(h, ar, B, T, s);
    DIMX_REQUIRE(!ar.overflow, DIMX_ERR_WORKSPACE, "set_context: workspace overflow");
    const int M = B * T, dim = h->d.dim, dim_a = h->d.dim_a;
    const float* xr = x;
    if (ldx_rows != T) {
        DIMX_HIP(hipMemcpy2DAsync(s.h, (size_t)T * dim * 4, x, (size_t)ldx_rows * dim * 4, (size_t)T * dim * 4, B,
                                  hipMemcpyDeviceToDevice, st));
        xr = s.h;
    }
    DIMX_TRY(launch_context_concat(h->at, xr, which_patch ? h->patch_dec_l : h->patch_dec_s, v_audio, s.xa, M, dim, dim_a, st));
    DIMX_TRY(project_cross_kv(h, s.xa, cp, B, T, for_generate, st));
    h->ctx_ready = true;
    h->ctx_B = B;
    h->ctx_T = T;
    h->ctx_for_generate = for_generate ? 1 : 0;
    h->ctx_ws = ws;
    return DIMX_OK;
}
// ... 40 lines not shown
                g.seg[i].st = D;
                g.seg[i].sd = 1;
                g.seg[i].D = D;
            }
        } else {
            g.seg[0].ptr = cp.ck[l];
            g.seg[0].sb = (long)T * heads * D;
            g.seg[0].st = heads * D;
            g.seg[0].sh = D;
            g.seg[0].sd = 1;
            g.seg[0].D = D;
            g.seg[1].ptr = cp.cv[l];
            g.seg[1].sb = (long)heads * D * Tp;
            g.seg[1].sh = (long)D * Tp;
            g.seg[1].sd = Tp;
            g.seg[1].st = 1;
            g.seg[1].D = D;
        }
        DIMX_TRY(launch_gemm(g, st));
    }
    return DIMX_OK;
}

int legacy_encode_ctx(dimx_handle h, const float* v_speaker, const uint8_t* mask, int B, int T, int for_generate,
                      float* enc_out, float* x_speaker_out, int32_t* idx_out, void* ws, size_t ws_bytes,
                      hipStream_t st) {
    DIMX_TRY(check_common(h, B, T, ws, ws_bytes, for_generate < 0 ? COMP_VQ0 : (COMP_VQ0 | COMP_ENC | COMP_DEC)));
    DIMX_REQUIRE(v_speaker && mask, DIMX_ERR_ARG, "encode_ctx: null argument");
    CtxPersist cp;
    Arena ar = scratch_arena(h, ws, ws_bytes, B, T, &cp);
    EncScratch s;
    VQScratch v;
    plan_enc(h, ar, B, T, s);
    plan_vq(h, h->vqg[0], ar, B, T, v);
    int32_t* lens = (int32_t*)ar.take((size_t)B * 4);
    DIMX_REQUIRE(!ar.overflow, DIMX_ERR_WORKSPACE, "encode_ctx: workspace overflow");
    const VQGeom& vg = h->vqg[0];
    const EncGeom& eg = h->encg[0];
    const int M = B * T;
    DIMX_TRY(launch_mask_lens(mask, lens, B, T, st));
    DIMX_TRY(run_vq_encode(h, 0, v_speaker, lens, B, T, 0, 0, v, v.z, v.idx_tmp, st));
    if (idx_out) {
        DIMX_HIP(hipMemcpyAsync(idx_out, v.idx_tmp, (size_t)M * vg.fqn * 4, hipMemcpyDeviceToDevice, st));
        DIMX_TRY(launch_finalize_idx(idx_out, lens, B, T, -100, st, vg.fqn));
    }
    if (x_speaker_out)
        DIMX_TRY(launch_legacy_scramble(DIMX_F32, h->vq[0].E, v.idx_tmp, lens, x_speaker_out, B, T, vg.fqn, vg.zdim,
                                        vg.n_embed, st));
    if (for_generate < 0) return DIMX_OK;
    DIMX_TRY(launch_legacy_scramble(h->at, h->vq[0].E, v.idx_tmp, lens, s.xa, B, T, vg.fqn, vg.zdim, vg.n_embed, st));
    DIMX_TRY(run_xenc(h, eg, h->enc_s, s.xa, eg.in_pad, s, B, T, mask, h->at, s.y, st));
    if (enc_out) DIMX_TRY(launch_layernorm(DIMX_F32, s.h, enc_out, h->enc_s.final_g, nullptr, M, eg.dim, st));
    DIMX_TRY(project_cross_kv(h, s.y, cp, B, T, for_generate, st));
    h->ctx_ready = true;
    h->ctx_B = B;
    h->ctx_T = T;
    h->ctx_for_generate = for_generate ? 1 : 0;
    h->ctx_ws = ws;
    return DIMX_OK;
}

}

extern "C" {

int dimx_decode_tf(dimx_handle h, const int32_t* z_l, const uint8_t* ctx_mask, const uint8_t* kv_mask, int B, int T,
                   float* logits, float* row_loss, int32_t* argmax_tok, void* ws, size_t ws_bytes, void* stream) {
    DIMX_TRY(check_common(h, B, T, ws, ws_bytes, COMP_DEC));
    DIMX_REQUIRE(z_l && ctx_mask && logits && T >= 2, DIMX_ERR_ARG, "decode_tf: null argument or T < 2");
    DIMX_REQUIRE(h->ctx_ready && h->ctx_B == B && h->ctx_T == T && h->ctx_ws == ws && !h->ctx_for_generate,
                 DIMX_ERR_STATE, "decode_tf: call dimx_encode_ctx(for_generate=0) with the same B, T, ws first");
    hipStream_t st = (hipStream_t)stream;
    CtxPersist cp;
    Arena ar = scratch_arena(h, ws, ws_bytes, B, T, &cp);
    DecScratch s;
    plan_dec(h, ar, B, T, s);
    DIMX_REQUIRE(!ar.overflow, DIMX_ERR_WORKSPACE, "decode_tf: workspace overflow");
    const DecGeom& dg = h->decg;
    const int n = T - 1, M = B * n, DD = dg.dim, heads = dg.heads, D = dg.dim_head;
    const int Tp = tpad(T), V = dg.num_tokens;
    DIMX_TRY(launch_shift_tokens(z_l, s.inp, s.tgt, B, T, st));
    DIMX_TRY(launch_gather_rows(DIMX_F32, h->dec.tok_emb, DD, V, s.inp, s.h, DD, M, DD, st));
    if (dg.abs_pos) DIMX_TRY(launch_add_pos_rows(s.h, h->dec.pos_emb, M, n, DD, 1.0f / sqrtf((float)DD), st));
    for (int l = 0; l < dg.depth; ++l) {
        AttnArgs a;
        DIMX_TRY(self_attn_qkv(h, s, h->dec.self_[l].ln_g, nullptr, h->dec.self_[l].qkv, B, n, DD, heads, D, a, st));
        a.scale = 1.0f / sqrtf((float)D); a.causal = 1; a.kmask = kv_mask; a.kmask_ld = n;
        DIMX_TRY(attn_out(h, s, a, h->dec.self_[l].out, DD, st));
        set_attn_packed(a, h->at, s.q, cp.ck[l], cp.cv[l], s.o, B, heads, n, T, D, Tp);
        DIMX_TRY(cross_attn_sublayer(h, s, h->dec.cross[l], a, ctx_mask, DD, st));
        DIMX_TRY(ff_sublayer(h, s, h->dec.ff[l].ln_g, nullptr, h->dec.ff[l].f1, h->dec.ff[l].f2, nullptr, ACT_GELU_ERF, M, DD, st));
    }
    DIMX_TRY(launch_layernorm(h->at, s.h, s.y, h->dec.final_g, nullptr, M, DD, st));
    DIMX_TRY(linear(h, s.y, DD, h->dec.logits, M, DIMX_F32, logits, V, st));
    if (row_loss || argmax_tok) DIMX_TRY(launch_ce_argmax(logits, s.tgt, row_loss, argmax_tok, M, V, st));
    return DIMX_OK;
}

}

namespace dimx {

static void chain_desc(ChainGemmDesc& d, const Linear& L) { d.W = L.w; d.N = L.N; d.K = L.K; d.ldw = L.Kp; }

static bool gen_use_chain(dimx_handle h, int B, int S, int grp) {
    if (!h->use_chain || h->at != DIMX_BF16 || S != 1 || grp != 0 || h->gen_groups > 1 || !h->chain_err_dev) return false;
    const DecGeom& dg = h->decg;
    ChainArgs c;
    memset(&c, 0, sizeof(c));
    c.B = B;
    c.C = dg.dim;
    const XAttn& sa = h->dec.self_[0];
    const XAttn& ca = h->dec.cross[0];
    chain_desc(c.g1, sa.out);
    c.lda1 = dg.heads * dg.dim_head;
    chain_desc(c.g2, ca.qkv);
    if (!chain_supported(c, h->cu_count)) return false;
    chain_desc(c.g2, h->dec.logits);
    c.g1.W = nullptr;
    return chain_supported(c, h->cu_count) && 3 * dg.depth + 1 <= kChainSites;
}

static bool gen_multi_tr(dimx_handle h, int S) {
    return S > 1 && h->multi_tr && h->at == DIMX_BF16 && h->decg.dim_head == 64;
}

static int slab_gemm_rows(dimx_handle h, int B, hipStream_t st, const void* A, int lda, const Linear& L, float* out, long stride,
                          int* nsl) {
    GemmArgs g;
    gemm_lin(h, A, lda, L, B, g);
    g.x3_decode = 1;
    g.out_dtype = DIMX_F32;
    g.out_slabs = 1;
    static const bool f32_split = getenv("DIMX_F32_NO_SPLIT") == nullptr;
    if (f32_split) g.allow_splitk = 1;
    g.slab_stride = stride;
    gemm_set_plain_out(g, out, L.N);
    *nsl = gemm_plan_splits(g);
    g.force_splitk = *nsl;
    return launch_gemm(g, st);
}

static bool qkv0_table_supported(dimx_handle h) {
    const DecGeom& dg = h->decg;
    const int N = 3 * dg.heads * dg.dim_head;
    return h->use_qkv0_table && !dg.abs_pos && h->dec.self_[0].qkv.N == N && N % 4 == 0 && N <= 12 * 256 && dg.dim % 4 == 0 &&
           dg.dim / 2 <= 16 * 64;
}

static int qkv0_table_build(dimx_handle h, const GenScratch& s, int M, hipStream_t st, int step0 = 0) {
    const DecGeom& dg = h->decg;
    const int DD = dg.dim, V = dg.num_tokens, N = h->dec.self_[0].qkv.N;
    if (h->qkv0_table && h->qkv0_M == M && h->qkv0_at == h->at && h->qkv0_epoch == h->dec_epoch) return DIMX_OK;
    if (!h->qkv0_table) {
        DIMX_HIP(hipMalloc((void**)&h->qkv0_table, (size_t)V * N * sizeof(float)));
        h->graph_valid = false;
    }
    h->qkv0_epoch = 0;
    const int rounds = (V + M - 1) / M;
    int32_t* ids = (int32_t*)s.logits;
    DIMX_TRY(launch_iota_clamp(ids, rounds * M, V, st));
    for (int r = 0; r < rounds; ++r) {
        int ns = 0;
        DIMX_TRY(launch_embed_step(h->dec.tok_emb, DD, V, ids + (size_t)r * M, nullptr, 0, s.step, s.x, M, 1, st, nullptr, 0.f, 1, step0));
        DIMX_TRY(launch_add_slabs_layernorm(h->at, s.x, s.xr, 0, s.st_xr, s.y, h->dec.self_[0].ln_g, M, DD, st));
        DIMX_TRY(slab_gemm_rows(h, M, st, s.y, DD, h->dec.self_[0].qkv, s.qkv, s.st_qkv, &ns));
        DIMX_TRY(launch_sum_slabs_rows(s.qkv, ns, s.st_qkv, h->qkv0_table, r * M, V, M, N, st));
    }
    if (h->use_kv0_table && h->at == DIMX_BF16) {
        const int inner = N / 3;
        if (!h->kv0_image) {
// ... 240 lines not shown
                ta.kwords_ready = 1;
                DIMX_TRY(launch_attention_tr(ta, st));
                goto cross_out;
            }
            DIMX_TRY(slab_gemm(s.y, DD, h->dec.cross[l].qkv, s.qc, s0.st_qc, &ns));
        }
        ca.nslab = ns;
        DIMX_TRY(launch_decode_attn(ca, st));
    cross_out:
        if (chain) {
            DIMX_TRY(chain_site(3 * l + 1, s.o, inner, &h->dec.cross[l].out, 0, h->dec.ff[l].ln_g, nullptr, nullptr, 0));
        } else {
            DIMX_TRY(slab_gemm(s.o, inner, h->dec.cross[l].out, s.xr, s0.st_xr, &pending));
            DIMX_TRY(launch_add_slabs_layernorm(h->at, s.x, s.xr, pending, s0.st_xr, s.y, h->dec.ff[l].ln_g, B, DD, st));
        }
    feed_forward:
        gemm_lin(h, s.y, DD, defer ? h->dec.ff[l].f1_ln : h->dec.ff[l].f1, B, g);
        g.x3_decode = 1;
        if (defer) {
            g.ln_stats = h->chain_stats_dev;
            g.ln_err = h->chain_err_dev;
            g.ln_colsum = h->dec.ff[l].f1_ln_colsum;
            g.ln_C = DD;
        }
        g.out_dtype = h->at;
        g.act = ACT_GELU_ERF;
        gemm_set_plain_out(g, s.f, DD * dg.ff_mult);
        DIMX_TRY(launch_gemm(g, st));
        DIMX_TRY(slab_gemm(s.f, DD * dg.ff_mult, h->dec.ff[l].f2, s.xr, s0.st_xr, &pending));
    }
    int nlg = 0;
    if (chain && !h->dec.logits.bias) {
        DIMX_TRY(chain_site(3 * dg.depth, nullptr, 0, nullptr, pending, h->dec.final_g, &h->dec.logits, s.logits, V));
        nlg = 1;
    } else {
        DIMX_TRY(launch_add_slabs_layernorm(h->at, s.x, s.xr, pending, s0.st_xr, s.y, h->dec.final_g, B, DD, st));
        DIMX_TRY(slab_gemm(s.y, DD, h->dec.logits, s.logits, s0.st_lg, &nlg));
    }
    if (gc.beam) {
        const BeamCall& bm = *gc.beam;
        BeamSelectArgs bs;
        bs.logits = s.logits; bs.nslab = nlg; bs.slab_stride = s0.st_lg; bs.nclip = nclip; bs.W = S;
        bs.step_dev = s.step; bs.step_rw = s.step; bs.done_ctr = (unsigned*)(s.step + 8); bs.epoch_rw = s.step + 9; bs.dev_params = s.step + 2;
        bs.prompt = forced; bs.prompt_ld = pr.ld; bs.prompt_max = pr.Pmax; bs.prompt_len = forced_len;
        bs.lens = bm.lens ? bm.lens + clip0 : nullptr; bs.len_off = T - n;
        bs.cum_in = bm.cum + row0; bs.cum_out = bm.cum + row0; bs.parent = bm.parent + row0;
        bs.tokens = tokens; bs.backptr = bm.backptr ? bm.backptr + (size_t)row0 * n : nullptr; bs.tok_ld = n; bs.logits_out = logits_out;
        bs.emb_table = h->dec.tok_emb; bs.emb_C = DD; bs.x_next = s.x;
        bs.qkv0_table = gc.qkv0; bs.qkv0_out = s.qkv; bs.qkv0_N = 3 * inner;
        DIMX_TRY(launch_beam_select(bs, st));
        if (!gc.qkv0) DIMX_TRY(launch_add_slabs_layernorm(h->at, s.x, s.xr, 0, s0.st_xr, s.y, h->dec.self_[0].ln_g, B, DD, st));
        BeamReorderArgs br;
        for (int l = 0; l < dg.depth; ++l) {
            br.buf[2 * l] = boff(s0.sk[l], (size_t)heads * T * 64 * es);
            br.buf[2 * l + 1] = boff(s0.sv[l], (size_t)heads * T * 64 * es);
        }
        br.nbuf = 2 * dg.depth; br.es = (int)es; br.nclip = nclip; br.W = S; br.H = heads; br.T = T;
        br.parent = bs.parent; br.step_dev = s.step; br.step_back = 1;
        br.tokens = tokens; br.backptr = bs.backptr; br.tok_ld = n;
        return launch_beam_reorder(br, st);
    }
    SampleArgs sm;
    sm.logits = s.logits; sm.ld_logits = V; sm.R = B; sm.nslab = nlg; sm.slab_stride = s0.st_lg; sm.row0 = row0; sm.rows_total = gc.Btot;
    sm.top_k = gc.top_k; sm.noise = gc.noise; sm.filt.kind = h->filter_kind;
    sm.temperature = gc.temperature; sm.seed = gc.seed;
    sm.step_dev = s.step; sm.step_rw = s.step; sm.dev_params = s.step + 2; sm.done_ctr = (unsigned*)(s.step + 8); sm.epoch_rw = s.step + 9;
    sm.tokens = tokens; sm.tok_ld = n; sm.tok_col_from_step = 1; sm.logits_out = logits_out; sm.logits_out_ld = n;
    sm.emb_table = h->dec.tok_emb; sm.emb_C = DD; sm.x_next = s.x; sm.pos_table = pos; sm.pos_scale = pos_scale; sm.pos_rows = n;
    sm.y_next = gc.qkv0 ? nullptr : s.y; sm.y_gamma = gc.qkv0 ? nullptr : h->dec.self_[0].ln_g; sm.y_dtype = h->at;
    sm.qkv0_table = gc.qkv0; sm.qkv0_out = s.qkv; sm.qkv0_N = 3 * inner;
    if (gc.kv0) { sm.hist = s.hist; sm.hist_ld = T; }
    sm.prompt = forced; sm.prompt_ld = pr.ld; sm.prompt_max = pr.Pmax; sm.prompt_len = forced_len; sm.prompt_div = S;
    return launch_sample(sm, st);
}

static int gen_prefill(dimx_handle h, const CtxPersist& cp, const GenScratch& gs, const PrefillScratch& s, const GenPrompt& pr,
                       const uint8_t* ctx_mask, int B, int T, int S, int32_t* tokens, hipStream_t st) {
    const DecGeom& dg = h->decg;
    const int n0 = pr.step0, M = B * n0, DD = dg.dim, heads = dg.heads, D = dg.dim_head;
    const int np = tpad(n0), Tp = tpad(T), V = dg.num_tokens;
    DIMX_TRY(launch_prompt_rows(pr.tok, pr.ld, B, n0, V, S, s.inp, tokens, gen_steps(h, T), st));
    DIMX_TRY(launch_gather_rows(DIMX_F32, h->dec.tok_emb, DD, V, s.inp, s.h, DD, M, DD, st));
    const bool rowv = qkv_row_v(h->at, D);
    for (int l = 0; l < dg.depth; ++l) {
        AttnArgs a;
        DIMX_TRY(self_attn_qkv(h, s, h->dec.self_[l].ln_g, nullptr, h->dec.self_[l].qkv, B, n0, DD, heads, D, a, st));
        DIMX_TRY(launch_kv_rows_to_cache(h->at, s.k, gs.sk[l], B, n0, heads, T, S, st));
        if (rowv)
            DIMX_TRY(launch_kv_rows_to_cache(h->at, s.vt, gs.sv[l], B, n0, heads, T, S, st));
        else
            DIMX_TRY(launch_kv_vt_to_cache((const float*)s.vt, np, (float*)gs.sv[l], B, n0, heads, T, S, st));
        if (l == dg.depth - 1) break;
        a.scale = 1.0f / sqrtf((float)D); a.causal = 1;
        DIMX_TRY(attn_out(h, s, a, h->dec.self_[l].out, DD, st));
        set_attn_packed(a, h->at, s.q, cp.ck[l], rowv ? cp.cv[l] : s.cvt, s.o, B, heads, n0, T, D, Tp, rowv);
        a.k_sb = (long)heads * Tp * D; a.k_sh = (long)Tp * D; a.k_st = D;
        if (rowv) { a.v_sb = a.k_sb; a.v_sh = a.k_sh; a.v_st = D; }
        DIMX_TRY(cross_attn_sublayer(h, s, h->dec.cross[l], a, ctx_mask, DD, st, rowv ? nullptr : (const float*)cp.cv[l]));
        DIMX_TRY(ff_sublayer(h, s, h->dec.ff[l].ln_g, nullptr, h->dec.ff[l].f1, h->dec.ff[l].f2, nullptr, ACT_GELU_ERF, M, DD, st));
    }
    return DIMX_OK;
}

}

extern "C" {

static int generate_impl(dimx_handle h, const dimx::GenPrompt& pr, bool keep_prefill, const uint8_t* ctx_mask, int B, int T, int n_samples,
                         float temperature, int top_k, const float* exp_noise, uint64_t seed, int32_t* tokens,
                         float* logits_out, void* ws, size_t ws_bytes, void* stream, bool* chain_used, bool prefill_only = false,
                         const dimx::BeamCall* beam = nullptr) {
    const int32_t* start = pr.tok;
    const int S = n_samples < 1 ? 1 : n_samples;
    if (h && h->filter_kind != DIMX_FILTER_TOP_K) top_k = 0;
    DIMX_REQUIRE(S == 1 || S == 2 || S == 4 || S == 5 || S == 8 || S == 10, DIMX_ERR_ARG,
                 "generate: n_samples %d not in {1,2,4,5,8,10}", n_samples);
    DIMX_TRY(check_common(h, B, T, ws, ws_bytes, COMP_DEC, S));
    DIMX_REQUIRE(start && ctx_mask && tokens && T >= 2, DIMX_ERR_ARG, "generate: null argument or T < 2");
    DIMX_REQUIRE(h->ctx_ready && h->ctx_B == B && h->ctx_T == T && h->ctx_ws == ws && h->ctx_for_generate,
                 DIMX_ERR_STATE, "generate: call dimx_encode_ctx(for_generate=1) with the same B, T, ws first");
    hipStream_t st = (hipStream_t)stream;
    CtxPersist cp;
    Arena ar = scratch_arena(h, ws, ws_bytes, B, T, &cp);
    GenScratch s;
    const int R = B * S;
    plan_gen(h, ar, R, T, s);
    PrefillScratch ps;
    if (pr.step0 > 0) plan_prefill(h, ar, B, pr.step0, T, ps);
    DIMX_REQUIRE(!ar.overflow, DIMX_ERR_WORKSPACE, "generate: workspace overflow");
    const int n = gen_steps(h, T);
    const int nrun = n - pr.step0;
    if (h->use_chain && h->at == DIMX_BF16 && !h->chain_err_dev) {
        DIMX_HIP(hipMalloc((void**)&h->chain_err_dev, 64));
        DIMX_HIP(hipMemset(h->chain_err_dev, 0, 64));
        DIMX_HIP(hipMalloc((void**)&h->chain_stats_dev, 8 * 32 * 32 * 2 * sizeof(float)));
        DIMX_HIP(hipMemset(h->chain_stats_dev, 0, 8 * 32 * 32 * 2 * sizeof(float)));
        DIMX_HIP(hipHostMalloc((void**)&h->chain_err_host, 64, hipHostMallocDefault));
        *h->chain_err_host = 0;
        DIMX_HIP(hipEventCreateWithFlags(&h->chain_err_ev, hipEventDisableTiming));
    }
    DIMX_HIP(hipMemsetAsync(s.chain_ctr, 0, (size_t)kChainSites * kChainSiteWords * 4, st));
    DIMX_TRY(launch_gen_params(s.step, dimx_ctx::kMaxGroups, temperature, seed, h->shard_row_off * S,
                               h->shard_rows_total * S, st, pr.step0, h->filter_a, h->filter_b));
    if (gen_multi_tr(h, S)) DIMX_TRY(launch_pack_key_words(ctx_mask, T, nullptr, B, T, s.kw, s.kw_cap, st));
    if (beam) {
        DIMX_REQUIRE(h->decg.dim_head == 64 && h->decg.depth <= 8 && !h->decg.abs_pos, DIMX_ERR_ARG,
                     "generate_beam: needs 64-wide heads, at most 8 layers and a decoder without positional embedding");
        DIMX_TRY(launch_beam_init(beam->cum, beam->parent, R, S, st));
        if (beam->backptr && pr.step0 > 0)
            DIMX_HIP(hipMemset2DAsync(beam->backptr, (size_t)n * 4, 0xFF, (size_t)pr.step0 * 4, R, st));
    }
    int G = h->gen_groups < 1 ? 1 : h->gen_groups;
    if (G > B) G = B;
    if (S > 1 || beam) G = 1;
    const float* qkv0 = nullptr;
    if (G == 1 && qkv0_table_supported(h)) {
        DIMX_TRY(qkv0_table_build(h, s, R, st, pr.step0));
        qkv0 = h->qkv0_table;
    }
    const void* kv0 = nullptr;
    if (qkv0 && h->use_kv0_table && !beam && pr.step0 == 0 && pr.Pmax <= 1 && h->decg.dim_head == 64 && h->decg.num_tokens <= 512) {
        kv0 = h->at == DIMX_BF16 ? h->kv0_image : (const void*)h->qkv0_table;
        if (kv0) ++h->kv0_generations;
    }
    if (pr.step0 > 0 && !keep_prefill) {
        if (logits_out)
            DIMX_HIP(hipMemset2DAsync(logits_out, (size_t)n * h->decg.num_tokens * 4, 0, (size_t)pr.step0 * h->decg.num_tokens * 4, R, st));
        DIMX_TRY(gen_prefill(h, cp, s, ps, pr, ctx_mask, B, T, S, tokens, st));
    }
    if (prefill_only) {
        *chain_used = false;
        return DIMX_OK;
    }
    int lo[dimx_ctx::kMaxGroups + 1];
    for (int g = 0; g <= G; ++g) lo[g] = (int)((long)R * g / G);
    hipStream_t gs[dimx_ctx::kMaxGroups];
    if (G == 1) {
        gs[0] = st;
    } else {
        if (!h->ev_fork) DIMX_HIP(hipEventCreateWithFlags(&h->ev_fork, hipEventDisableTiming));
        DIMX_HIP(hipEventRecord(h->ev_fork, st));
// ... 582 lines not shown

static int op_decode_attn_ex(int dtype, const void* q, int q_ld, int q_is_f32, int nslab, long slab_stride, int self_attn, void* kcache,
                             void* vcache, void* out, int o_ld, int B, int H, int Tmax, const int32_t* step_dev, int n_keys,
                             const uint8_t* kmask, int kmask_ld, int rows_per_clip, float scale, int nsplit, int win, int lookahead,
                             void* stream) {
    const int S = rows_per_clip > 1 ? rows_per_clip : 1;
    DIMX_REQUIRE(B > 0 && H > 0 && Tmax > 0, DIMX_ERR_ARG, "op_decode_attn_ex: empty shape");
    DIMX_REQUIRE(nslab >= 1 && nslab <= 8 && (nslab == 1 || q_is_f32), DIMX_ERR_ARG, "op_decode_attn_ex: nslab=%d (1..8, > 1 for f32 q only)",
                 nslab);
    DIMX_REQUIRE(q_ld >= (self_attn ? 3 : 1) * H * 64 && o_ld >= H * 64, DIMX_ERR_ARG, "op_decode_attn_ex: q_ld=%d o_ld=%d too small",
                 q_ld, o_ld);
    DIMX_REQUIRE(nslab == 1 || slab_stride >= (long)B * S * q_ld, DIMX_ERR_ARG, "op_decode_attn_ex: slabs overlap (stride %ld)",
                 slab_stride);
    DIMX_REQUIRE(self_attn ? (step_dev != nullptr && kmask == nullptr && S == 1) : (n_keys >= 1 && n_keys <= Tmax), DIMX_ERR_ARG,
                 "op_decode_attn_ex: self form needs a step counter (no mask, one row per clip); cross form 1 <= n_keys (%d) <= Tmax",
                 n_keys);
    DIMX_REQUIRE(kmask == nullptr || kmask_ld >= n_keys, DIMX_ERR_ARG, "op_decode_attn_ex: kmask_ld=%d < n_keys=%d", kmask_ld, n_keys);
    DecodeAttnArgs a;
    memset(&a, 0, sizeof(a));
    a.dtype = dtype;
    a.q = q;
    a.q_ld = q_ld;
    a.q_f32 = q_is_f32 ? 1 : 0;
    a.nslab = nslab;
    a.slab_stride = slab_stride;
    if (self_attn) {
        const size_t es = q_is_f32 ? 4 : dtype_size(dtype);
        a.knew = (const unsigned char*)q + (size_t)H * 64 * es;
        a.vnew = (const unsigned char*)q + (size_t)2 * H * 64 * es;
        a.kv_ld = q_ld;
        a.step = step_dev;
    } else {
        a.n_keys = n_keys;
        a.kmask = kmask;
        a.kmask_ld = kmask_ld;
    }
    a.kcache = kcache;
    a.vcache = vcache;
    a.Tmax = Tmax;
    a.out = out;
    a.o_ld = o_ld;
    a.B = B;
    a.H = H;
    a.rows_per_clip = rows_per_clip;
    a.scale = scale;
    a.force_nsplit = nsplit;
    if (win) {
        a.win = 1;
        a.lookahead = lookahead;
        a.step = step_dev;
    }
    return launch_decode_attn(a, (hipStream_t)stream);
}

int dimx_op_decode_attn_ex(int dtype, const void* q, int q_ld, int q_is_f32, int nslab, long slab_stride, int self_attn, void* kcache,
                           void* vcache, void* out, int o_ld, int B, int H, int Tmax, const int32_t* step_dev, int n_keys,
                           const uint8_t* kmask, int kmask_ld, int rows_per_clip, float scale, int nsplit, void* stream) {
    return op_decode_attn_ex(dtype, q, q_ld, q_is_f32, nslab, slab_stride, self_attn, kcache, vcache, out, o_ld, B, H, Tmax, step_dev, n_keys,
                             kmask, kmask_ld, rows_per_clip, scale, nsplit, 0, 0, stream);
}

int dimx_op_decode_attn_win(int dtype, const void* q, int q_ld, int q_is_f32, int nslab, long slab_stride, void* kcache, void* vcache,
                            void* out, int o_ld, int B, int H, int Tmax, const int32_t* step_dev, int n_keys, const uint8_t* kmask,
                            int kmask_ld, int rows_per_clip, float scale, int nsplit, int lookahead, void* stream) {
    DIMX_REQUIRE(step_dev != nullptr, DIMX_ERR_ARG, "op_decode_attn_win: the windowed form needs a step counter");
    return op_decode_attn_ex(dtype, q, q_ld, q_is_f32, nslab, slab_stride, 0, kcache, vcache, out, o_ld, B, H, Tmax, step_dev, n_keys, kmask,
                             kmask_ld, rows_per_clip, scale, nsplit, 1, lookahead, stream);
}

size_t dimx_mlp_fused_packed_bytes(int C, int F) { return mlp_fused_packed_bytes(C, F); }

int dimx_mlp_fused_pack(const float* w1_host, const float* b1_host, const float* w2_host, int C, int F, void* out_host, size_t out_bytes) {
    DIMX_REQUIRE(w1_host && w2_host && out_host, DIMX_ERR_ARG, "mlp_fused_pack: null argument");
    DIMX_REQUIRE(mlp_fused_packed_bytes(C, F) > 0 && out_bytes >= mlp_fused_packed_bytes(C, F), DIMX_ERR_ARG,
                 "mlp_fused_pack: C = %d F = %d unsupported or the output buffer is too small", C, F);
    return mlp_fused_pack(w1_host, b1_host, w2_host, C, F, (uint16_t*)out_host);
}

int dimx_op_mlp_fused_packed(float* x, const void* packed, const float* b2, const float* ln_g, const float* ln_b, int M, int C, int F, int act,
                             void* stream) {
    return launch_mlp_fused(x, packed, b2, ln_g, ln_b, M, C, F, act, (hipStream_t)stream);
}

int dimx_op_mlp_fused(float* x, const float* w1_host, const float* b1_host, const float* w2_host, const float* b2, const float* ln_g,
                      const float* ln_b, int M, int C, int F, int act, void* stream) {
    DIMX_REQUIRE(x && w1_host && w2_host && b2 && ln_g && M > 0, DIMX_ERR_ARG, "op_mlp_fused: null argument");
    const size_t bytes = mlp_fused_packed_bytes(C, F);
    DIMX_REQUIRE(bytes > 0, DIMX_ERR_ARG, "op_mlp_fused: C = %d F = %d not supported", C, F);
    std::vector<uint16_t> img(bytes / 2);
    DIMX_TRY(mlp_fused_pack(w1_host, b1_host, w2_host, C, F, img.data()));
    void* p = nullptr;
    DIMX_HIP(hipMalloc(&p, bytes));
    int rc = DIMX_OK;
    if (hipMemcpy(p, img.data(), bytes, hipMemcpyHostToDevice) != hipSuccess) rc = DIMX_ERR_HIP;
    if (rc == DIMX_OK) rc = launch_mlp_fused(x, p, b2, ln_g, ln_b, M, C, F, act, (hipStream_t)stream);
    if (hipStreamSynchronize((hipStream_t)stream) != hipSuccess && rc == DIMX_OK) rc = DIMX_ERR_HIP;
    (void)hipFree(p);
    return rc;
}

int dimx_op_add_slabs_layernorm(int out_dtype, float* x, const float* slabs, int nslab, long slab_stride, void* y,
                                const float* gamma, int M, int C, void* stream) {
    return launch_add_slabs_layernorm(out_dtype, x, slabs, nslab, slab_stride, y, gamma, M, C, (hipStream_t)stream);
}

int dimx_op_chain(const void* A1, int K1, const void* W1, float* x, const float* slabs, int nslab, const float* gamma,
                  void* y, const void* W2, int N2, float* out2, int B, int C, void* scratch, void* stream) {
    DIMX_REQUIRE(scratch && x && y && gamma, DIMX_ERR_ARG, "op_chain: null argument");
    int dev = 0, cus = 0;
    DIMX_HIP(hipGetDevice(&dev));
    DIMX_HIP(hipDeviceGetAttribute(&cus, hipDeviceAttributeMultiprocessorCount, dev));
    ChainArgs c;
    memset(&c, 0, sizeof(c));
    unsigned* u = (unsigned*)scratch;
    c.B = B;
    c.C = C;
    if (W1) {
        c.g1.W = W1; c.g1.N = C; c.g1.K = K1; c.g1.ldw = K1;
        c.A1 = A1; c.lda1 = K1;
        c.xr = (float*)(u + 512);
    }
    c.x = x;
    c.slabs = slabs;
    c.nslab = nslab;
    c.slab_stride = (long)B * C;
    c.y = y;
    c.gamma = gamma;
    if (W2) {
        c.g2.W = W2; c.g2.N = N2; c.g2.K = C; c.g2.ldw = C;
        c.out2 = out2; c.ld_out2 = N2;
    }
    c.counters = u;
    c.seen = u + 256;
    c.step = (const int32_t*)(u + 128);
    c.err = u + 129;
    DIMX_REQUIRE(chain_supported(c, cus), DIMX_ERR_ARG, "op_chain: shape not supported on this device (%d CUs)", cus);
    DIMX_HIP(hipMemsetAsync(u, 0, 512 * 4, (hipStream_t)stream));
    return launch_chain(c, (hipStream_t)stream);
}

int dimx_op_chain_ln(const void* A1, int K1, const void* W1, float* x, void* y, float* stats, const void* W2s,
                     const float* colsum2, int N2, float* out2, int B, int C, void* scratch, void* stream) {
    DIMX_REQUIRE(scratch && x && y && stats && A1 && W1, DIMX_ERR_ARG, "op_chain_ln: null argument");
    int dev = 0, cus = 0;
    DIMX_HIP(hipGetDevice(&dev));
    DIMX_HIP(hipDeviceGetAttribute(&cus, hipDeviceAttributeMultiprocessorCount, dev));
    ChainArgs c;
    memset(&c, 0, sizeof(c));
    unsigned* u = (unsigned*)scratch;
    c.B = B;
    c.C = C;
    c.g1.W = W1; c.g1.N = C; c.g1.K = K1; c.g1.ldw = K1;
    c.A1 = A1; c.lda1 = K1;
    c.xr = (float*)(u + 512);
    c.x = x;
    c.y = y;
    c.gamma = (const float*)x;
    c.defer = 1;
    c.stats = stats;
    if (W2s) {
        c.g2.W = W2s; c.g2.N = N2; c.g2.K = C; c.g2.ldw = C;
        c.out2 = out2; c.ld_out2 = N2;
        c.colsum2 = colsum2;
    }
    c.counters = u;
    c.seen = u + 256;
// ... 88 lines not shown
```

### dyadic-interaction-modeling_amd/csrc/model.hpp

```cpp
#pragma once
#include <map>
#include <string>
#include <vector>

#include "common.hpp"

namespace dimx {

struct Linear {
    void* w = nullptr;
    const float* bias = nullptr;
    int N = 0, K = 0, Kp = 0;
    void* w3 = nullptr;
};

struct VQBlock {
    const float *ln1_g, *ln1_b, *ln2_g, *ln2_b;
    Linear qkv, out, l1, l2;
    const void* mlp = nullptr;
};

struct VQNet {
    Linear vm, conv, le, post;
    VQBlock enc[8];
// ... 72 lines not shown
        if (base && off > cap) overflow = true;
        return p;
    }
};

struct BeamCall {
    double* cum = nullptr;
    int32_t* parent = nullptr;
    int32_t* backptr = nullptr;
    const int32_t* lens = nullptr;
    bool operator==(const BeamCall& o) const { return cum == o.cum && parent == o.parent && backptr == o.backptr && lens == o.lens; }
};

struct GraphKey {
    void* ws;
    int B, T, top_k;
    float temperature;
    const void* noise;
    uint64_t seed;
    const void *start, *mask, *tokens, *logits_out;
    int groups;
    const void* prompt_len;
    int ld_prompt, Pmax;
    int filter_kind;
    BeamCall beam;
    int xwin_on, xwin_lookahead;
    bool operator==(const GraphKey& o) const {
        return xwin_on == o.xwin_on && xwin_lookahead == o.xwin_lookahead && beam == o.beam && groups == o.groups && filter_kind == o.filter_kind && prompt_len == o.prompt_len && ld_prompt == o.ld_prompt && Pmax == o.Pmax && ws == o.ws && B == o.B && T == o.T && top_k == o.top_k && temperature == o.temperature &&
               noise == o.noise && seed == o.seed && start == o.start && mask == o.mask && tokens == o.tokens &&
               logits_out == o.logits_out;
    }
};

}

namespace dimx {
int vq_pe_buffers(dimx_ctx* c, int which, const float** pe_enc, const float** pe_dec);
void train_forget(dimx_ctx* h);
}

struct dimx_ctx {
    int device = 0;
    dimx_dims d;
    int variant = 0;
    dimx::VQGeom vqg[2];
    dimx::EncGeom encg[2];
    dimx::DecGeom decg;
    int mode = 0;
    int at = DIMX_F32;
    std::map<std::string, dimx::HostTensor> host;
    std::vector<std::string> required;
    int packed_mask = 0;
    std::vector<void*> dev_allocs;
    dimx::VQNet vq[2];
    dimx::XEnc enc_s, enc_joint, enc_l;
    dimx::XDec dec;
    const float *patch_s = nullptr, *patch_dec_s = nullptr, *norm_s_g = nullptr, *norm_s_b = nullptr;
    const float *patch_l = nullptr, *patch_dec_l = nullptr, *norm_l_g = nullptr, *norm_l_b = nullptr;
    const float *norm_j_g = nullptr, *norm_j_b = nullptr;
    bool ctx_ready = false;
    int ctx_B = 0, ctx_T = 0, ctx_for_generate = 0;
    void* ctx_ws = nullptr;
    static constexpr int kMaxGroups = 8;
    hipGraphExec_t graph_exec[kMaxGroups] = {};
    hipGraphExec_t graph_multi[kMaxGroups] = {};
    int graph_unroll = 16;
    static constexpr int kPreGroups = 4;
    int prefill_groups = 0;
    hipStream_t pre_stream[kPreGroups - 1] = {};
    hipEvent_t pre_fork = nullptr, pre_join[kPreGroups - 1] = {};
    hipStream_t grp_stream[kMaxGroups] = {};
    hipEvent_t ev_fork = nullptr, ev_join[kMaxGroups] = {};
    int gen_groups = 1;
    hipStream_t cap_stream = nullptr;
    dimx::GraphKey graph_key{};
    bool graph_valid = false;
    int use_graph = 1;
    int use_chain = 1;
    int cu_count = 0;
    float* chain_stats_dev = nullptr;
    int defer_ln = 1;
    unsigned long long* layer_prof_dev = nullptr;
    int multi_tr = 1;
    int use_layer_chain = 1;
    unsigned* chain_err_dev = nullptr;
    unsigned* chain_err_host = nullptr;
    hipEvent_t chain_err_ev = nullptr;
    int chain_faults = 0;
    int chain_fault_inject = 0;
    int use_qkv0_table = 1;
    float* qkv0_table = nullptr;
    int qkv0_M = 0, qkv0_at = -1;
    uint64_t qkv0_epoch = 0;
    uint64_t dec_epoch = 1;
    int qkv0_builds = 0;
    int use_kv0_table = 1;
    void* kv0_image = nullptr;
    int kv0_generations = 0;
    int shard_row_off = 0, shard_rows_total = 0;
    int filter_kind = 0;
    float filter_a = 0.f, filter_b = 0.f;
    int xwin_on = 0, xwin_lookahead = 0;
    dimx::MeshHead mesh;
    int lstm_faults = 0;
    int spk_embed_rows = 0;
};
```

### dyadic-interaction-modeling_amd/csrc/norm.hip

```cpp
#include "common.hpp"

namespace dimx {

template <typename OutT, int C>
__global__ __launch_bounds__(256) void layernorm_kernel(const float* __restrict__ x, OutT* __restrict__ y,
                                                        const float* __restrict__ gamma,
                                                        const float* __restrict__ beta, int M) {
    constexpr int PER = C / 64;
    constexpr int NV = PER / 2;
    const int row = blockIdx.x * 4 + (threadIdx.x >> 6);
    const int lane = threadIdx.x & 63;
    if (row >= M) return;
    const float2* xr = (const float2*)(x + (size_t)row * C);
    const float2* g2 = (const float2*)gamma;
    const float2* b2 = (const float2*)beta;
    float2 v[NV], gv[NV], bv[NV];
    float s = 0.f;
#pragma unroll
    for (int i = 0; i < NV; ++i) {
        v[i] = xr[lane + 64 * i];
        s += v[i].x + v[i].y;
    }
#pragma unroll
    for (int i = 0; i < NV; ++i) {
        gv[i] = g2[lane + 64 * i];
        bv[i] = beta ? b2[lane + 64 * i] : make_float2(0.f, 0.f);
    }
    const float mean = wave_sum_sel<sizeof(OutT) == 2>(s) * (1.0f / C);
    float q = 0.f;
#pragma unroll
    for (int i = 0; i < NV; ++i) {
        const float a = v[i].x - mean, b = v[i].y - mean;
        q += a * a + b * b;
    }
    const float rstd = rsqrtf(wave_sum_sel<sizeof(OutT) == 2>(q) * (1.0f / C) + 1e-5f);
    OutT* yr = y + (size_t)row * C;
#pragma unroll
    for (int i = 0; i < NV; ++i) {
        const int c2 = lane + 64 * i;
        const float o0 = (v[i].x - mean) * rstd * gv[i].x + bv[i].x;
        const float o1 = (v[i].y - mean) * rstd * gv[i].y + bv[i].y;
        if (sizeof(OutT) == 2) {
            *(uint32_t*)(yr + 2 * c2) = pack_bf16x2(o0, o1);
        } else {
            *(float2*)(yr + 2 * c2) = make_float2(o0, o1);
        }
    }
}

template <typename OutT, int C>
__global__ __launch_bounds__(256) void add_slabs_layernorm_kernel(float* __restrict__ x,
                                                                  const float* __restrict__ slabs, int nslab,
                                                                  long slab_stride, OutT* __restrict__ y,
                                                                  const float* __restrict__ gamma, int M) {
    constexpr int NV = C / 128;
    const int row = blockIdx.x * (blockDim.x >> 6) + (threadIdx.x >> 6);
    const int lane = threadIdx.x & 63;
    if (row >= M) return;
    float2* xr = (float2*)(x + (size_t)row * C);
    const float2* g2 = (const float2*)gamma;
    float2 v[NV], gv[NV];
#pragma unroll
    for (int i = 0; i < NV; ++i) {
        v[i] = xr[lane + 64 * i];
        gv[i] = g2[lane + 64 * i];
    }
    for (int s0 = 0; s0 < nslab; s0 += 4) {
        float2 t[4][NV];
#pragma unroll
        for (int k = 0; k < 4; ++k) {
            const bool on = s0 + k < nslab;
            const float2* sr = (const float2*)(slabs + (size_t)(on ? s0 + k : 0) * slab_stride + (size_t)row * C);
#pragma unroll
            for (int i = 0; i < NV; ++i) t[k][i] = sr[lane + 64 * i];
        }
#pragma unroll
        for (int k = 0; k < 4; ++k) {
            if (s0 + k < nslab) {
#pragma unroll
                for (int i = 0; i < NV; ++i) {
                    v[i].x += t[k][i].x;
                    v[i].y += t[k][i].y;
                }
            }
        }
    }
    float s = 0.f;
#pragma unroll
    for (int i = 0; i < NV; ++i) {
        if (nslab > 0) xr[lane + 64 * i] = v[i];
        s += v[i].x + v[i].y;
    }
    const float mean = wave_sum_sel<sizeof(OutT) == 2>(s) * (1.0f / C);
    float q = 0.f;
#pragma unroll
    for (int i = 0; i < NV; ++i) {
        const float a = v[i].x - mean, b = v[i].y - mean;
        q += a * a + b * b;
    }
    const float rstd = rsqrtf(wave_sum_sel<sizeof(OutT) == 2>(q) * (1.0f / C) + 1e-5f);
    OutT* yr = y + (size_t)row * C;
#pragma unroll
    for (int i = 0; i < NV; ++i) {
        const int c2 = lane + 64 * i;
        const float o0 = (v[i].x - mean) * rstd * gv[i].x, o1 = (v[i].y - mean) * rstd * gv[i].y;
        if (sizeof(OutT) == 2) {
            *(uint32_t*)(yr + 2 * c2) = pack_bf16x2(o0, o1);
        } else {
            *(float2*)(yr + 2 * c2) = make_float2(o0, o1);
        }
    }
}

int launch_add_slabs_layernorm(int out_dtype, float* x, const float* slabs, int nslab, long slab_stride, void* y,
                               const float* gamma, int M, int C, hipStream_t s) {
    DIMX_REQUIRE(x && y && gamma && M > 0 && (nslab == 0 || slabs), DIMX_ERR_ARG, "add_slabs_layernorm: null operand");
    DIMX_REQUIRE(C == 1152 || C == 384 || C == 512 || C == 768, DIMX_ERR_ARG, "add_slabs_layernorm: C=%d", C);
    const int wpb = M <= 1024 ? 1 : 4;
    dim3 grid(ceil_div(M, wpb)), block(64 * wpb);
#define ASL(OT, CC) hipLaunchKernelGGL((add_slabs_layernorm_kernel<OT, CC>), grid, block, 0, s, x, slabs, nslab, slab_stride, (OT*)y, gamma, M)
#define ASL_C(OT)                      \
    do {                               \
        if (C == 384) ASL(OT, 384);    \
        else if (C == 512) ASL(OT, 512); \
        else if (C == 768) ASL(OT, 768); \
        else ASL(OT, 1152);            \
    } while (0)
    if (out_dtype == DIMX_BF16) ASL_C(bf16); else ASL_C(float);
#undef ASL_C
#undef ASL
// ... 73 lines not shown
```

### dyadic-interaction-modeling_amd/lib.py

```python
import ctypes
import os
from ctypes import (POINTER, c_char_p, c_float, c_int, c_int32, c_int64, c_size_t, c_uint64,
                    c_void_p)

import torch

HERE = os.path.dirname(os.path.abspath(__file__))
LIB_PATH = os.environ.get("DIMX_LIB", os.path.join(HERE, "libdimx_hip.so"))

MODE_PARITY_F32 = 0
MODE_PERF_BF16 = 1
F32, BF16 = 0, 1
ACT_NONE, ACT_LEAKY, ACT_GELU_TANH, ACT_GELU_ERF = 0, 1, 2, 3


class DimxError(RuntimeError):
    pass


class Dims(ctypes.Structure):
    _fields_ = [(n, c_int) for n in (
        "vq_in_dim", "vq_hidden", "vq_layers", "vq_heads", "vq_inter", "vq_n_embed", "vq_zdim",
        "dim_in", "dim", "dim_a", "enc_depth", "dec_depth", "heads", "dim_head", "num_tokens",
        "max_seq_len", "ff_mult", "variant", "spk_in_dim", "spk_hidden", "spk_heads", "spk_inter",
# ... 48 lines not shown
    "dimx_generate_beam": (c_int, [c_void_p, c_void_p, c_int, c_void_p, c_int, c_int, c_void_p, c_void_p, c_int, c_int, c_int, c_void_p,
                                   c_void_p, c_void_p, c_void_p, c_void_p, c_size_t, c_int, c_void_p, c_size_t, c_void_p]),
    "dimx_train_num_params": (c_int, [c_void_p]),
    "dimx_train_total": (c_int64, [c_void_p]),
    "dimx_train_param_info": (c_int, [c_void_p, c_int, POINTER(c_char_p), POINTER(c_int64), POINTER(c_int64)]),
    "dimx_train_workspace_bytes": (c_size_t, [c_void_p, c_int, c_int]),
    "dimx_train_forward_backward": (c_int, [c_void_p, c_void_p, c_void_p, c_void_p, c_void_p, c_void_p, c_void_p, c_void_p, c_int,
                                            c_int, c_void_p, c_void_p, c_void_p, c_size_t, c_void_p]),
    "dimx_train_graph_stats": (c_int, [c_void_p, c_void_p]),
    "dimx_train_legacy_workspace_bytes": (c_size_t, [c_void_p, c_int, c_int]),
    "dimx_train_legacy_forward_backward": (c_int, [c_void_p, c_void_p, c_void_p, c_void_p, c_void_p, c_void_p, c_void_p, c_void_p, c_void_p,
                                                   c_void_p, c_int, c_int, c_void_p, c_void_p, c_void_p, c_void_p, c_size_t, c_void_p]),
    "dimx_train_slm_workspace_bytes": (c_size_t, [c_void_p, c_int, c_int]),
    "dimx_train_slm_forward_backward": (c_int, [c_void_p] + [c_void_p] * 14 + [c_int, c_int, c_void_p, c_void_p, c_size_t, c_void_p]),
    "dimx_train_vq_num_params": (c_int, [c_void_p, c_int]),
    "dimx_train_vq_total": (c_int64, [c_void_p, c_int]),
    "dimx_train_vq_param_info": (c_int, [c_void_p, c_int, c_int, POINTER(c_char_p), POINTER(c_int64), POINTER(c_int64)]),
    "dimx_train_vq_workspace_bytes": (c_size_t, [c_void_p, c_int, c_int]),
    "dimx_train_vq_forward_backward": (c_int, [c_void_p, c_int, c_void_p, c_void_p, c_void_p, c_int, c_int, c_float, c_float, c_float,
                                               c_uint64, c_int64, c_void_p, c_void_p, c_void_p, c_void_p, c_size_t, c_void_p]),
    "dimx_train_conv_num_params": (c_int, [c_void_p]),
    "dimx_train_conv_total": (c_int64, [c_void_p]),
    "dimx_train_conv_param_info": (c_int, [c_void_p, c_int, POINTER(c_char_p), POINTER(c_int64), POINTER(c_int64)]),
    "dimx_train_conv_workspace_bytes": (c_size_t, [c_void_p, c_int, c_int]),
    "dimx_train_conv_forward_backward": (c_int, [c_void_p, c_void_p, c_void_p, c_void_p, c_void_p, c_void_p, c_void_p, c_int, c_int, c_int,
                                                 c_int, c_void_p, c_void_p, c_void_p, c_size_t, c_void_p]),
    "dimx_train_spk_num_params": (c_int, [c_void_p]),
    "dimx_train_spk_total": (c_int64, [c_void_p]),
    "dimx_train_spk_param_info": (c_int, [c_void_p, c_int, POINTER(c_char_p), POINTER(c_int64), POINTER(c_int64)]),
    "dimx_train_spk_workspace_bytes": (c_size_t, [c_void_p, c_int, c_int]),
    "dimx_train_spk_forward_backward": (c_int, [c_void_p] + [c_void_p] * 9 + [c_int, c_int, c_void_p, c_void_p, c_void_p, c_void_p, c_void_p,
                                                c_size_t, c_void_p]),
    "dimx_op_lstm_layer_bwd": (c_int, [c_int, c_void_p, c_int, c_int, c_int, c_int, POINTER(c_void_p), POINTER(c_void_p),
                                       POINTER(c_void_p), POINTER(c_void_p), c_void_p, c_void_p, POINTER(c_void_p), POINTER(c_void_p),
                                       POINTER(c_void_p), c_int, POINTER(c_int), c_void_p]),
    "dimx_train_adamw": (c_int, [c_void_p, c_void_p, c_void_p, c_void_p, c_int64, c_float, c_float, c_float, c_float, c_float,
                                 c_int, c_float, c_void_p, c_void_p]),
    "dimx_op_train_attention": (c_int, [c_int, c_void_p, c_void_p, c_void_p, c_void_p, c_void_p, c_void_p, c_int, c_int, c_int,
                                        c_int, c_int, c_float, c_void_p, c_void_p, c_void_p, c_void_p, c_void_p, c_void_p,
                                        c_void_p]),
    "dimx_op_train_layernorm_bwd": (c_int, [c_void_p, c_void_p, c_void_p, c_void_p, c_int, c_int, c_int, c_void_p, c_void_p, c_void_p,
                                            c_size_t, c_void_p]),
    "dimx_op_train_colsum": (c_int, [c_void_p, c_int, c_int, c_void_p, c_void_p, c_size_t, c_void_p]),
    "dimx_op_train_prep": (c_int, [c_int, c_int, c_void_p, c_int, c_void_p, c_int, c_void_p, c_void_p, c_int, c_int, c_void_p, c_size_t,
                                   c_void_p, c_size_t, c_void_p, c_size_t, POINTER(c_int), c_void_p]),
    "dimx_op_train_cross_entropy": (c_int, [c_void_p, c_void_p, c_int, c_void_p, c_void_p, c_void_p, c_void_p]),
    "dimx_chain_faults": (c_int, [c_void_p]),
    "dimx_qkv0_table_builds": (c_int, [c_void_p]),
    "dimx_kv0_table_generations": (c_int, [c_void_p]),
    "dimx_lstm_faults": (c_int, [c_void_p]),
    "dimx_mesh_head": (c_int, [c_void_p, c_void_p, c_void_p, c_int, c_int, c_void_p, c_int, c_void_p, c_size_t, c_void_p]),
    "dimx_op_lstm_layer": (c_int, [c_int, c_void_p, c_int, c_int, c_int, c_int, POINTER(c_void_p), POINTER(c_void_p),
                                   POINTER(c_void_p), POINTER(c_void_p), c_void_p, c_int, POINTER(c_int), c_void_p]),
    "dimx_debug_chain_fault": (c_int, [c_void_p, c_int]),
    "dimx_op_gemm_slabs": (c_int, [c_int, c_int, c_int, c_int, c_int]),
    "dimx_op_split_x3": (c_int, [c_void_p, c_void_p, ctypes.c_long, c_void_p]),
    "dimx_op_gemm_x3": (c_int, [c_void_p, c_int, c_void_p, c_void_p, c_int, c_int, c_int, c_int, c_void_p, c_int, c_void_p, c_int, c_int,
                                c_void_p]),
    "dimx_op_gemm": (c_int, [c_int, c_int, c_void_p, c_int, c_void_p, c_int, c_void_p, c_int, c_int, c_int,
                             c_int, c_void_p, c_int, c_void_p, c_int, c_int, c_void_p, c_int, c_void_p]),
    "dimx_op_gemm_headmajor": (c_int, [c_int, c_void_p, c_int, c_void_p, c_int, c_void_p, c_int, c_int, c_int, c_int, c_int,
                                       c_int, c_void_p]),
    "dimx_op_layernorm": (c_int, [c_int, c_void_p, c_void_p, c_void_p, c_void_p, c_int, c_int, c_void_p]),
    "dimx_op_instnorm": (c_int, [c_int, c_void_p, c_void_p, c_void_p, c_int, c_int, c_int, c_void_p]),
    "dimx_op_attention": (c_int, [c_int, c_void_p, c_void_p, c_void_p, c_void_p, c_int, c_int, c_int, c_int,
                                  c_int, c_int, c_int, c_int, c_int, c_float, c_int, c_void_p, c_void_p,
                                  c_void_p]),
    "dimx_op_attention_rowv": (c_int, [c_void_p, c_void_p, c_void_p, c_void_p, c_int, c_int, c_int, c_int, c_int, c_int, c_int,
                                       c_int, c_int, c_float, c_int, c_void_p, c_void_p, c_void_p]),
    "dimx_op_decode_attn": (c_int, [c_int, c_void_p, c_void_p, c_void_p, c_void_p, c_int, c_int, c_int, c_int,
                                    c_float, c_void_p, c_int, c_int, c_void_p]),
    "dimx_op_decode_attn_self": (c_int, [c_int, c_void_p, c_int, c_void_p, c_void_p, c_void_p, c_int, c_int, c_int,
                                         c_void_p, c_float, c_int, c_void_p]),
    "dimx_op_decode_attn_ex": (c_int, [c_int, c_void_p, c_int, c_int, c_int, ctypes.c_long, c_int, c_void_p, c_void_p, c_void_p,
                                       c_int, c_int, c_int, c_int, c_void_p, c_int, c_void_p, c_int, c_int, c_float, c_int,
                                       c_void_p]),
    "dimx_op_decode_attn_win": (c_int, [c_int, c_void_p, c_int, c_int, c_int, ctypes.c_long, c_void_p, c_void_p, c_void_p,
                                        c_int, c_int, c_int, c_int, c_void_p, c_int, c_void_p, c_int, c_int, c_float, c_int,
                                        c_int, c_void_p]),
    "dimx_op_mlp_fused": (c_int, [c_void_p, c_void_p, c_void_p, c_void_p, c_void_p, c_void_p, c_void_p, c_int, c_int, c_int, c_int, c_void_p]),
    "dimx_mlp_fused_packed_bytes": (c_size_t, [c_int, c_int]),
    "dimx_mlp_fused_pack": (c_int, [c_void_p, c_void_p, c_void_p, c_int, c_int, c_void_p, c_size_t]),
    "dimx_op_mlp_fused_packed": (c_int, [c_void_p, c_void_p, c_void_p, c_void_p, c_void_p, c_int, c_int, c_int, c_int, c_void_p]),
    "dimx_op_add_slabs_layernorm": (c_int, [c_int, c_void_p, c_void_p, c_int, ctypes.c_long, c_void_p, c_void_p, c_int,
                                            c_int, c_void_p]),
    "dimx_op_chain": (c_int, [c_void_p, c_int, c_void_p, c_void_p, c_void_p, c_int, c_void_p, c_void_p, c_void_p, c_int,
                              c_void_p, c_int, c_int, c_void_p, c_void_p]),
    "dimx_op_chain_ln": (c_int, [c_void_p, c_int, c_void_p, c_void_p, c_void_p, c_void_p, c_void_p, c_void_p, c_int,
                                 c_void_p, c_int, c_int, c_void_p, c_void_p]),
    "dimx_op_layer_chain": (c_int, [c_void_p, c_int, ctypes.c_long, c_void_p, c_void_p, c_int, c_void_p, c_void_p, c_int, c_int, c_void_p,
                                    c_void_p, c_void_p, c_void_p, c_void_p, c_void_p, c_void_p, c_void_p, c_void_p, c_void_p, c_int,
                                    c_void_p, c_int, c_float, c_void_p, c_void_p, c_void_p]),
    "dimx_op_gemm_ln": (c_int, [c_int, c_void_p, c_void_p, c_void_p, c_int, c_int, c_int, c_void_p, c_int, c_void_p,
                                c_void_p, c_void_p]),
    "dimx_op_fd_select_ws_bytes": (c_size_t, [c_int, c_int, c_int]),
    "dimx_op_fd_select": (c_int, [c_void_p, ctypes.c_long, ctypes.c_long, c_void_p, ctypes.c_long, ctypes.c_long, ctypes.c_long, c_void_p,
                                  c_int, c_int, c_int, c_int, c_int, c_int, c_void_p, c_void_p, c_void_p, c_void_p, c_void_p, c_size_t,
                                  c_void_p]),
    "dimx_op_mesh_metrics_ws_bytes": (c_size_t, [c_int, c_int, c_int, c_int]),
    "dimx_op_mesh_metrics": (c_int, [c_void_p, ctypes.c_long, ctypes.c_long, c_void_p, ctypes.c_long, ctypes.c_long, c_void_p, ctypes.c_long,
                                     POINTER(c_int32), c_int, c_int, c_int, c_void_p, c_int, c_void_p, c_int, c_void_p, c_void_p, c_void_p,
                                     c_void_p, c_size_t, c_void_p]),
    "dimx_op_listener_metrics_ws_bytes": (c_size_t, [c_int, c_int, c_int]),
    "dimx_op_listener_metrics": (c_int, [c_void_p, ctypes.c_long, ctypes.c_long, c_void_p, ctypes.c_long, ctypes.c_long, c_void_p, ctypes.c_long,
                                         ctypes.c_long, c_void_p, c_int, c_int, c_int, c_int, POINTER(c_int32), c_int, c_void_p, c_void_p,
                                         c_void_p, c_size_t, c_void_p]),
    "dimx_op_kmeans_fit_ws_bytes": (c_size_t, [c_int, c_int, c_int]),
    "dimx_op_kmeans_fit": (c_int, [c_void_p, ctypes.c_long, c_int, c_int, c_int, c_int, c_int, c_int, c_void_p, c_int, ctypes.c_double,
                                   c_int, c_void_p, c_void_p, c_void_p, c_void_p, c_void_p, c_size_t, c_void_p]),
    "dimx_op_sid_assign": (c_int, [c_void_p, ctypes.c_long, c_int, c_int, c_int, c_int, c_void_p, c_int, c_void_p, c_void_p, c_void_p,
                                   c_void_p]),
    "dimx_op_seq_logprob": (c_int, [c_void_p, ctypes.c_long, ctypes.c_long, c_void_p, ctypes.c_long, c_void_p, c_void_p, c_int, c_int,
                                    c_int, c_void_p, c_void_p, c_void_p, c_void_p]),
    "dimx_op_score_select": (c_int, [c_void_p, c_void_p, ctypes.c_long, ctypes.c_long, ctypes.c_long, c_void_p, c_void_p, ctypes.c_long,
                                     c_int, c_int, c_int, c_int, c_int, c_void_p, c_void_p, c_void_p, c_void_p, c_void_p]),
    "dimx_op_consensus_select_ws_bytes": (c_size_t, [c_int, c_int, c_int, c_int]),
    "dimx_op_consensus_select": (c_int, [c_void_p, ctypes.c_long, ctypes.c_long, ctypes.c_long, c_void_p, c_int, c_int, c_int, c_int, c_int,
                                         c_int, c_int, c_void_p, c_void_p, c_void_p, c_void_p, c_void_p, c_void_p, ctypes.c_long, c_int,
                                         c_void_p, c_void_p, c_size_t, c_void_p]),
    "dimx_op_pool_desc": (c_int, [c_void_p, ctypes.c_long, ctypes.c_long, c_void_p, c_int, c_int, c_int, c_int, c_void_p, c_void_p,
                                  c_void_p]),
    "dimx_op_nn_search_ws_bytes": (c_size_t, [c_int, c_int, c_int, c_int]),
    "dimx_op_nn_search": (c_int, [c_void_p, ctypes.c_long, c_void_p, c_void_p, ctypes.c_long, c_void_p, c_int, c_int, c_int, c_int,
                                  c_void_p, c_void_p, c_void_p, c_void_p, c_void_p, c_size_t, c_void_p]),
    "dimx_op_nn_gather": (c_int, [c_void_p, c_void_p, ctypes.c_long, ctypes.c_long, c_void_p, c_void_p, c_int, c_int, c_int, c_int,
                                  c_int, c_int, c_void_p, c_void_p, c_void_p]),
    "dimx_op_beam_step": (c_int, [c_void_p, c_void_p, c_void_p, c_void_p, c_int, c_int, c_void_p, c_void_p, c_void_p, c_void_p]),
    "dimx_op_beam_reorder": (c_int, [c_void_p, c_int, c_void_p, c_int, c_int, c_int, c_int, c_int, c_void_p]),
    "dimx_op_sample": (c_int, [c_void_p, c_int, c_int, c_float, c_void_p, c_uint64, c_uint64, c_void_p,
                               c_void_p]),
    "dimx_op_sample_filtered": (c_int, [c_void_p, c_int, c_int, c_int, c_float, c_float, c_float, c_void_p, c_uint64, c_uint64,
                                        c_void_p, c_void_p, c_void_p]),
}

_lib = None


def load(build_if_missing=True):
    global _lib
    if _lib is not None:
        return _lib
    in_tree = "DIMX_LIB" not in os.environ
    if not os.path.exists(LIB_PATH):
        if not build_if_missing or not in_tree:
            raise DimxError("libdimx_hip.so not found at %s (run python __graft_entry__.py build)" % LIB_PATH)
        from . import build as _build
        _build.build()
    elif in_tree:
        from . import build as _build
        if _build.stale():
            if build_if_missing and _build.have_hipcc():
                _build.build()
            elif not os.environ.get("DIMX_ALLOW_STALE_LIB"):
                raise DimxError("libdimx_hip.so at %s was not built from the sources next to it and %s; run "
                                "python __graft_entry__.py build where hipcc exists"
                                % (LIB_PATH, "hipcc is not available" if build_if_missing else "rebuilding was not requested"))
    lib = ctypes.CDLL(LIB_PATH)
    for name, (res, args) in SIGNATURES.items():
        if not in_tree and not hasattr(lib, name):
            setattr(lib, name, _missing_symbol(name))
            continue
        fn = getattr(lib, name)
        fn.restype = res
        fn.argtypes = args
    _lib = lib
    return lib
# ... 49 lines not shown
```

### include/dimx.h

```cpp
#ifndef DIMX_H
#define DIMX_H

#include <stddef.h>
#include <stdint.h>

#ifdef __cplusplus
extern "C" {
#endif

typedef struct dimx_ctx* dimx_handle;

typedef enum {
    DIMX_OK = 0,
    DIMX_ERR_ARG = -1,
    DIMX_ERR_HIP = -2,
    DIMX_ERR_WEIGHT = -3,
    DIMX_ERR_STATE = -4,
    DIMX_ERR_WORKSPACE = -5
} dimx_status;

#define DIMX_MODE_PARITY_F32 0
#define DIMX_MODE_PERF_BF16 1

#define DIMX_F32 0
// ... 120 lines not shown
int dimx_train_slm_forward_backward(dimx_handle h, const float* params, float* grads, const float* v_speaker, const float* v_listener,
                                    const float* v_audio, const uint8_t* mask, const uint8_t* mask_speaker, const uint8_t* mask_listener,
                                    const int32_t* z_s, const int32_t* z_l, const float* codebook_s, const float* codebook_l,
                                    const float* pe_s, const float* pe_l, int B, int T, float* loss_out, void* ws, size_t ws_bytes,
                                    void* stream);
int dimx_train_vq_num_params(dimx_handle h, int which);
int64_t dimx_train_vq_total(dimx_handle h, int which);
int dimx_train_vq_param_info(dimx_handle h, int which, int i, const char** name, int64_t* offset, int64_t* numel);
size_t dimx_train_vq_workspace_bytes(dimx_handle h, int B, int T);
int dimx_train_vq_forward_backward(dimx_handle h, int which, const float* params, float* grads, const float* x, int B, int T, float beta,
                                   float quant_loss_weight, float dropout_p, uint64_t dropout_seed, int64_t step, float* loss_out,
                                   float* pred_out, int32_t* idx_out, void* ws, size_t ws_bytes, void* stream);
int dimx_train_conv_num_params(dimx_handle h);
int64_t dimx_train_conv_total(dimx_handle h);
int dimx_train_conv_param_info(dimx_handle h, int i, const char** name, int64_t* offset, int64_t* numel);
size_t dimx_train_conv_workspace_bytes(dimx_handle h, int B, int T);
int dimx_train_conv_forward_backward(dimx_handle h, const float* params, float* grads, const float* motion, const float* templ,
                                     const float* target, const float* vert_w, int n_mouth, int B, int T, int flags, float* loss_out,
                                     float* mesh_out, void* ws, size_t ws_bytes, void* stream);
int dimx_train_spk_num_params(dimx_handle h);
int64_t dimx_train_spk_total(dimx_handle h);
int dimx_train_spk_param_info(dimx_handle h, int i, const char** name, int64_t* offset, int64_t* numel);
size_t dimx_train_spk_workspace_bytes(dimx_handle h, int B, int T);
int dimx_train_spk_forward_backward(dimx_handle h, const float* params, float* grads, const float* v_emoca, const float* v_audio,
                                    const uint8_t* mask, const int32_t* z, const int32_t* speaker_ids, const float* codebook_s,
                                    const float* pe_s, int B, int T, float* loss_out, float* logits_out, int32_t* idx_out, float* pred_out,
                                    void* ws, size_t ws_bytes, void* stream);
int dimx_op_lstm_layer_bwd(int dtype, const float* x, int B, int T, int In, int H, const float* const* w_ih, const float* const* w_hh,
                           const float* const* b_ih, const float* const* b_hh, const float* dy, float* dx, float* const* dw_ih,
                           float* const* dw_hh, float* const* db, int flags, int* faults_out, void* stream);
int dimx_train_adamw(float* params, const float* grads, float* exp_avg, float* exp_avg_sq, int64_t n, float lr, float beta1,
                     float beta2, float eps, float weight_decay, int step, float max_norm, float* scratch, void* stream);
int dimx_op_train_attention(int mfma, const float* q, const float* k, const float* v, const float* d_o, const uint8_t* kmask,
                            const uint8_t* kmask2, int B, int H, int Lq, int Lk, int causal, float scale, float* o, float* lse,
                            float* delta, float* dq, float* dk, float* dv, void* stream);
int dimx_op_train_layernorm_bwd(const float* x, const float* gamma, const float* dy, float* dx, int accumulate, int M, int C, float* dgamma,
                                float* dbeta, float* scratch, size_t scratch_floats, void* stream);
int dimx_op_train_colsum(const float* dy, int M, int C, float* out, float* scratch, size_t scratch_floats, void* stream);
int dimx_op_train_prep(int dtype, int mode, const float* src, int lds, const float* src2, int lds2, const float* gamma, const float* beta,
                       int rows, int cols, void* o, size_t o_elems, void* t, size_t t_elems, float* colpart, size_t colpart_floats,
                       int* dims3, void* stream);
int dimx_op_train_cross_entropy(const float* logits, const int32_t* targets, int R, float* row_loss, float* dlogits, float* loss_out2,
                                void* stream);


int dimx_op_gemm(int in_dtype, int out_dtype, const void* A, int lda, const void* W, int ldw, void* C,
                 int ldc, int M, int N, int K, const float* bias, int act, const float* residual,
                 int ldr, int conv_T, const int32_t* conv_lens, int flags, void* stream);
int dimx_op_split_x3(const float* w, void* planes, long n, void* stream);
int dimx_op_gemm_x3(const float* A, int lda, const void* planes, float* C, int ldc, int M, int N, int K, const float* bias, int act,
                    const float* residual, int ldr, int flags, void* stream);
int dimx_op_gemm_slabs(int in_dtype, int M, int N, int K, int flags);
int dimx_op_gemm_headmajor(int dtype, const void* A, int lda, const void* W, int ldw, void* out, int M, int N, int K,
                           int rowT, int Tp, int nlayers, void* stream);
int dimx_op_lstm_layer(int dtype, const float* x, int B, int T, int In, int H, const float* const* w_ih, const float* const* w_hh,
                       const float* const* b_ih, const float* const* b_hh, float* y, int flags, int* faults_out, void* stream);
int dimx_op_layernorm(int out_dtype, const float* x, void* y, const float* gamma, const float* beta,
                      int M, int C, void* stream);
int dimx_op_instnorm(int out_dtype, const float* x, void* y, const int32_t* lens, int B, int T, int C,
                     void* stream);
int dimx_op_attention(int dtype, const void* q, const void* k, const void* vt, void* out, int B, int H,
                      int Lq, int Lk, int D, int ldq, int ldk, int ld_vt, int ldo, float scale,
                      int causal, const int32_t* lens, const uint8_t* kmask, void* stream);
int dimx_op_attention_rowv(const void* q, const void* k, const void* v, void* out, int B, int H, int Lq, int Lk, int D, int ldq,
                           int ldk, int ldv, int ldo, float scale, int causal, const int32_t* lens, const uint8_t* kmask,
                           void* stream);
int dimx_op_decode_attn(int dtype, const void* q, const void* kcache, const void* vcache, void* out, int B, int H,
                        int Tmax, int n_keys, float scale, const uint8_t* kmask, int nsplit, int q_is_f32,
                        void* stream);
int dimx_op_decode_attn_self(int dtype, const void* qkv, int ld, void* kcache, void* vcache, void* out, int B, int H,
                             int Tmax, const int32_t* step_dev, float scale, int q_is_f32, void* stream);
int dimx_op_decode_attn_ex(int dtype, const void* q, int q_ld, int q_is_f32, int nslab, long slab_stride, int self_attn, void* kcache,
                           void* vcache, void* out, int o_ld, int B, int H, int Tmax, const int32_t* step_dev, int n_keys,
                           const uint8_t* kmask, int kmask_ld, int rows_per_clip, float scale, int nsplit, void* stream);
int dimx_op_decode_attn_win(int dtype, const void* q, int q_ld, int q_is_f32, int nslab, long slab_stride, void* kcache, void* vcache,
                            void* out, int o_ld, int B, int H, int Tmax, const int32_t* step_dev, int n_keys, const uint8_t* kmask,
                            int kmask_ld, int rows_per_clip, float scale, int nsplit, int lookahead, void* stream);
int dimx_op_mlp_fused(float* x, const float* w1_host, const float* b1_host, const float* w2_host, const float* b2, const float* ln_g,
                      const float* ln_b, int M, int C, int F, int act, void* stream);
size_t dimx_mlp_fused_packed_bytes(int C, int F);
int dimx_mlp_fused_pack(const float* w1_host, const float* b1_host, const float* w2_host, int C, int F, void* out_host, size_t out_bytes);
int dimx_op_mlp_fused_packed(float* x, const void* packed, const float* b2, const float* ln_g, const float* ln_b, int M, int C, int F,
                             int act, void* stream);
int dimx_op_add_slabs_layernorm(int out_dtype, float* x, const float* slabs, int nslab, long slab_stride, void* y,
                                const float* gamma, int M, int C, void* stream);
int dimx_op_chain(const void* A1, int K1, const void* W1, float* x, const float* slabs, int nslab, const float* gamma,
                  void* y, const void* W2, int N2, float* out2, int B, int C, void* scratch, void* stream);
int dimx_op_chain_ln(const void* A1, int K1, const void* W1, float* x, void* y, float* stats, const void* W2s,
                     const float* colsum2, int N2, float* out2, int B, int C, void* scratch, void* stream);
int dimx_op_gemm_ln(int out_dtype, const void* A, const void* Ws, void* C, int M, int N, int K, const float* bias, int act,
                    const float* stats, const float* colsum, void* stream);
int dimx_op_layer_chain(const float* qkv, int nslab, long slab_stride, void* sk, void* sv, int T, const void* ck, const void* cv,
                        int Tp, int n_keys, const uint8_t* kmask, const void* w_so, const void* w_cq, const float* colsum_cq,
                        const void* w_co, float* x, void* y, void* o, float* qc, float* stats, int B, const int32_t* step,
                        int call_index, float scale, void* scratch, void* prof, void* stream);
size_t dimx_op_fd_select_ws_bytes(int B, int S, int F);
int dimx_op_fd_select(const float* y_true, long yt_clip_stride, long yt_frame_stride, const float* y_pred, long yp_clip_stride,
                      long yp_sample_stride, long yp_frame_stride, const int32_t* lens, int B, int S, int L, int W, int c0, int F,
                      double* fd, int32_t* win, uint8_t* ok, float* best, void* workspace, size_t workspace_bytes, void* stream);
size_t dimx_op_mesh_metrics_ws_bytes(int B, int L, int n_mouth, int n_upper);
int dimx_op_mesh_metrics(const float* y_true, long yt_clip_stride, long yt_frame_stride, const float* y_pred, long yp_clip_stride,
                         long yp_frame_stride, const float* templ, long templ_clip_stride, const int32_t* lens, int B, int L, int n_vert,
                         const int32_t* mouth, int n_mouth, const int32_t* upper, int n_upper, double* clip_out, double* frame_max,
                         int32_t* status, void* workspace, size_t workspace_bytes, void* stream);
#define DIMX_LM_ROW 133
size_t dimx_op_listener_metrics_ws_bytes(int B, int n_win, int F);
int dimx_op_listener_metrics(const float* y_true, long yt_clip_stride, long yt_frame_stride, const float* y_pred, long yp_clip_stride,
                             long yp_frame_stride, const float* x, long x_clip_stride, long x_frame_stride, const int32_t* lens, int B,
                             int L, int Wy, int Wx, const int32_t* windows, int n_win, double* fd, double* moments, void* workspace,
                             size_t workspace_bytes, void* stream);
size_t dimx_op_kmeans_fit_ws_bytes(int N, int K, int F);
int dimx_op_kmeans_fit(const float* frames, long frame_stride, int N, int W, int c0, int F, int K, int first_index, const double* U,
                       int trials, double tol, int max_iter, double* centers, int32_t* n_iter, int32_t* status, int32_t* labels,
                       void* workspace, size_t workspace_bytes, void* stream);
int dimx_op_sid_assign(const float* frames, long frame_stride, int M, int W, int c0, int F, const double* centers, int K, int64_t* hist,
                       double* sid, int32_t* labels, void* stream);
int dimx_op_seq_logprob(const float* logits, long row_stride, long step_stride, const int32_t* tokens, long tok_row_stride,
                        const int32_t* first, const int32_t* last, int rows_per_clip, int R, int n, double* tok_logprob, double* score,
                        int32_t* count, void* stream);
int dimx_op_score_select(const double* score, const float* y_pred, long yp_clip_stride, long yp_sample_stride, long yp_frame_stride,
                         const int32_t* lens, const int32_t* tokens, long tok_row_stride, int B, int S, int L, int W, int n,
                         int32_t* win, uint8_t* ok, float* best, int32_t* best_tokens, void* stream);
size_t dimx_op_consensus_select_ws_bytes(int B, int S, int F, int kind);
int dimx_op_consensus_select(const float* y_pred, long yp_clip_stride, long yp_sample_stride, long yp_frame_stride,
                             const int32_t* lens, int B, int S, int L, int W, int c0, int F, int kind ,
                             double* dist , double* risk , int32_t* win, uint8_t* ok,
                             float* best , const int32_t* tokens, long tok_row_stride, int n_tok,
                             int32_t* best_tokens , void* workspace, size_t workspace_bytes, void* stream);
int dimx_op_pool_desc(const float* x, long clip_stride, long frame_stride, const int32_t* lens, int N, int T, int D,
                      int kind , double* desc, double* norm, void* stream);
size_t dimx_op_nn_search_ws_bytes(int Q, int N, int D, int K);
int dimx_op_nn_search(const double* q_desc, long q_row_stride, const double* q_norm, const double* x_desc, long x_row_stride,
                      const double* x_norm, int Q, int N, int D, int K, int32_t* idx, double* sim, int32_t* found,
                      double* sim_out , void* workspace, size_t workspace_bytes, void* stream);
int dimx_op_nn_gather(const int32_t* idx, const float* lib_seq, long clip_stride, long frame_stride, const int32_t* lib_lens,
                      const int32_t* q_lens, int Q, int K, int N, int Lmax, int L, int W, float* out, int32_t* out_len, void* stream);
int dimx_op_beam_step(const float* logits, const double* cum, const int32_t* mode, const int32_t* forced_tok, int B, int W,
                      int32_t* parent, int32_t* token, double* cum_out, void* stream);
int dimx_op_beam_reorder(void* cache, int dtype, const int32_t* parent, int R, int W, int H, int T, int c, void* stream);
int dimx_op_sample(const float* logits, int R, int top_k, float temperature, const float* exp_noise,
                   uint64_t seed, uint64_t step, int32_t* tokens, void* stream);
int dimx_op_sample_filtered(const float* logits, int R, int kind, int top_k, float a, float b, float temperature,
                            const float* exp_noise, uint64_t seed, uint64_t step, int32_t* tokens, uint8_t* keep_out,
                            void* stream);

#ifdef __cplusplus
}
#endif
#endif
```

Before: 1728 clips/s.

## Fuse next-layer LayerNorm into fused MLP epilogue and pack key words once

The fused MLP kernel gains an epilogue that stages output rows through LDS, adds the residual, and writes the next sublayer's LayerNorm (or a cast) to a second buffer. The following attention's separate layernorm launch is then skipped. A norm+context-concat kernel merges the final norm with the context build, and key-mask words are packed once per stack instead of per layer. This cuts launches and activation round-trips, but adds register pressure (32 rows x NV float2 held per lane) and LDS reuse of the weight ring in the epilogue.

```diff
diff --git a/dyadic-interaction-modeling_amd/csrc/common.hpp b/dyadic-interaction-modeling_amd/csrc/common.hpp
--- a/dyadic-interaction-modeling_amd/csrc/common.hpp
+++ b/dyadic-interaction-modeling_amd/csrc/common.hpp
@@ -181,6 +181,75 @@
     return (lane_f32(v, 0) + lane_f32(v, 16)) + (lane_f32(v, 32) + lane_f32(v, 48));
 }
 template <bool FAST> __device__ __forceinline__ float wave_sum_sel(float v) { return FAST ? wave_sum_fast(v) : wave_sum(v); }
+
+template <bool FAST, int R> __device__ __forceinline__ void wave_sum_sel_n(float (&v)[R]) {
+#define DIMX_WSN_STEP(EXPR)                                   \
+    do {                                                      \
+        _Pragma("unroll") for (int r = 0; r < R; ++r) v[r] = (EXPR); \
+        if (R > 1) __builtin_amdgcn_sched_barrier(0);         \
+    } while (0)
+    if (FAST) {
+        DIMX_WSN_STEP(v[r] + dpp_f32<DPP_XOR1>(v[r]));
+        DIMX_WSN_STEP(v[r] + dpp_f32<DPP_XOR2>(v[r]));
+        DIMX_WSN_STEP(v[r] + dpp_f32<DPP_HALF_MIRROR>(v[r]));
+        DIMX_WSN_STEP(v[r] + dpp_f32<DPP_ROW_MIRROR>(v[r]));
+        DIMX_WSN_STEP((lane_f32(v[r], 0) + lane_f32(v[r], 16)) + (lane_f32(v[r], 32) + lane_f32(v[r], 48)));
+    } else {
+        DIMX_WSN_STEP(v[r] + xor_lane_f32<32>(v[r]));
+        DIMX_WSN_STEP(v[r] + xor_lane_f32<16>(v[r]));
+        DIMX_WSN_STEP(v[r] + xor_lane_f32<8>(v[r]));
+        DIMX_WSN_STEP(v[r] + xor_lane_f32<4>(v[r]));
+        DIMX_WSN_STEP(v[r] + xor_lane_f32<2>(v[r]));
+        DIMX_WSN_STEP(v[r] + xor_lane_f32<1>(v[r]));
+    }
+#undef DIMX_WSN_STEP
+}
+
+template <bool FAST, int C, int R>
+__device__ __forceinline__ void layernorm_rows(const float2 (&v)[R][C / 128], const float2 (&gv)[C / 128], const float2 (&bv)[C / 128],
+                                               float2 (&o)[R][C / 128]) {
+    constexpr int NV = C / 128;
+    float s[R], q[R], mean[R], rstd[R];
+#pragma unroll
+    for (int r = 0; r < R; ++r) {
+        s[r] = 0.f;
+#pragma unroll
+        for (int i = 0; i < NV; ++i) s[r] += v[r][i].x + v[r][i].y;
+    }
+    wave_sum_sel_n<FAST, R>(s);
+#pragma unroll
+    for (int r = 0; r < R; ++r) {
+        mean[r] = s[r] * (1.0f / C);
+        q[r] = 0.f;
+#pragma unroll
+        for (int i = 0; i < NV; ++i) {
+            const float a = v[r][i].x - mean[r], b = v[r][i].y - mean[r];
+            q[r] += a * a + b * b;
+        }
+    }
+    wave_sum_sel_n<FAST, R>(q);
+#pragma unroll
+    for (int r = 0; r < R; ++r) {
+        rstd[r] = rsqrtf(q[r] * (1.0f / C) + 1e-5f);
+#pragma unroll
+        for (int i = 0; i < NV; ++i) {
+            o[r][i].x = (v[r][i].x - mean[r]) * rstd[r] * gv[i].x + bv[i].x;
+            o[r][i].y = (v[r][i].y - mean[r]) * rstd[r] * gv[i].y + bv[i].y;
+        }
+    }
+}
+template <bool FAST, int C>
+__device__ __forceinline__ void layernorm_row(const float2 (&v)[C / 128], const float2 (&gv)[C / 128], const float2 (&bv)[C / 128],
+                                              float2 (&o)[C / 128]) {
+    layernorm_rows<FAST, C, 1>(*reinterpret_cast<const float2(*)[1][C / 128]>(&v), gv, bv, *reinterpret_cast<float2(*)[1][C / 128]>(&o));
+}
+template <typename OutT> __device__ __forceinline__ void store_row_pair(OutT* yr, int c2, float o0, float o1) {
+    if (sizeof(OutT) == 2) {
+        *(uint32_t*)(yr + 2 * c2) = pack_bf16x2(o0, o1);
+    } else {
+        *(float2*)(yr + 2 * c2) = make_float2(o0, o1);
+    }
+}
 template <int O> __device__ __forceinline__ double xor_lane_f64(double v) {
     const unsigned long long u = __builtin_bit_cast(unsigned long long, v);
     const unsigned lo = (unsigned)xor_lane_i32<O>((int)(unsigned)u), hi = (unsigned)xor_lane_i32<O>((int)(unsigned)(u >> 32));
@@ -299,6 +368,8 @@
 int mlp_fused_pack(const float* w1, const float* b1, const float* w2, int C, int F, uint16_t* out);
 int launch_mlp_fused(float* x, const void* packed, const float* b2, const float* ln_g, const float* ln_b, int M, int C, int F, int act,
                      hipStream_t s);
+int launch_mlp_fused_y(float* x, const void* packed, const float* b2, const float* ln_g, const float* ln_b, int M, int C, int F, int act,
+                       int y_mode, int y_dtype, void* y, const float* g2, const float* bt2, hipStream_t s);
 
 struct DecodeAttnArgs {
     int dtype;
@@ -408,6 +479,8 @@
                  size_t scratch_bytes, int flags, int cu_count, int* fault_count, hipStream_t st);
 int launch_context_concat(int out_dtype, const float* x_s, const float* patch, const float* audio, void* ctx,
                           int M, int dim, int dim_a, hipStream_t s);
+int launch_norm_context(int out_dtype, const float* x, const float* gamma, const float* beta, float* x_s_out, const float* patch,
+                        const float* audio, void* ctx, int M, int dim, int dim_a, hipStream_t s);
 int launch_finalize_idx(int32_t* idx, const int32_t* lens, int B, int T, int32_t pad_value, hipStream_t s,
                         int fqn = 1);
 int launch_shift_tokens(const int32_t* z, int32_t* inp, int32_t* tgt, int B, int T, hipStream_t s);
diff --git a/dyadic-interaction-modeling_amd/csrc/mlp_fused.hip b/dyadic-interaction-modeling_amd/csrc/mlp_fused.hip
--- a/dyadic-interaction-modeling_amd/csrc/mlp_fused.hip
+++ b/dyadic-interaction-modeling_amd/csrc/mlp_fused.hip
@@ -1,4 +1,6 @@
 #include "common.hpp"
+
+#include <type_traits>
 
 namespace dimx {
 namespace {
@@ -39,9 +41,15 @@
     const float* ln_g;
     const float* ln_b;
     int M, nchunk;
+    void* y;
+    const float* g2;
+    const float* bt2;
 };
 
-template <int ACT, bool BETA> __global__ __launch_bounds__(256) void mlp_fused_kernel(const MlpArgs a) {
+constexpr int kStageLd = kC + 4;
+constexpr int kStageRows = 16;
+
+template <int ACT, bool BETA, int YM> __global__ __launch_bounds__(256) void mlp_fused_kernel(const MlpArgs a) {
     extern __shared__ __attribute__((aligned(1024))) unsigned char smem[];
     const int tid = threadIdx.x, wave = __builtin_amdgcn_readfirstlane(tid >> 6), lane = tid & 63, hf = lane >> 5, l31 = lane & 31;
     const int row = blockIdx.x * 128 + wave * 32 + l31;
@@ -226,6 +234,84 @@
         s2 = s2 == 2 ? 0 : s2 + 1;
     }
 
+    if (YM != 0) {
+        using OutT = typename std::conditional<YM == 1 || YM == 3, bf16, float>::type;
+        constexpr bool kNorm = YM <= 2;
+        constexpr int NV = kC / 128;
+        const int wrow0 = blockIdx.x * 128 + wave * 32;
+        float2 xn[32][NV];
+#pragma unroll
+        for (int r = 0; r < 32; ++r) {
+            const int gr = wrow0 + r < a.M ? wrow0 + r : a.M - 1;
+            const float2* xr = (const float2*)(a.x + (size_t)gr * kC);
+#pragma unroll
+            for (int i = 0; i < NV; ++i) xn[r][i] = xr[lane + 64 * i];
+        }
+        float2 gv[NV], bv[NV];
+#pragma unroll
+        for (int i = 0; i < NV; ++i) {
+            gv[i] = kNorm ? ((const float2*)a.g2)[lane + 64 * i] : make_float2(0.f, 0.f);
+            bv[i] = kNorm && a.bt2 ? ((const float2*)a.bt2)[lane + 64 * i] : make_float2(0.f, 0.f);
+        }
+        asm volatile("s_waitcnt vmcnt(0)" ::: "memory");
+        __syncthreads();
+        float* const stage = (float*)smem + wave * (kStageRows * kStageLd);
+        OutT* const y = (OutT*)a.y;
+        auto rows_out = [&](auto full) {
+#pragma unroll
+            for (int p = 0; p < 32 / kStageRows; ++p) {
+                if (l31 / kStageRows == p) {
+                    float* sr = stage + (l31 % kStageRows) * kStageLd + 4 * hf;
+#pragma unroll
+                    for (int ob = 0; ob < kOB; ++ob)
+#pragma unroll
+                        for (int q = 0; q < 4; ++q) {
+                            const f32x4_t v = {o[ob][4 * q], o[ob][4 * q + 1], o[ob][4 * q + 2], o[ob][4 * q + 3]};
+                            *(f32x4_t*)(sr + 32 * ob + 8 * q) = v;
+                        }
+                }
+                __syncthreads();
+#pragma unroll
+                for (int r4 = 0; r4 < kStageRows; r4 += 4) {
+                    float2 yv[4][NV];
+#pragma unroll
+                    for (int k = 0; k < 4; ++k) {
+                        const int r = kStageRows * p + r4 + k;
+                        const float2* sr = (const float2*)(stage + (r4 + k) * kStageLd);
+#pragma unroll
+                        for (int i = 0; i < NV; ++i) {
+                            const float2 ov = sr[lane + 64 * i];
+                            xn[r][i].x += ov.x;
+                            xn[r][i].y += ov.y;
+                        }
+                    }
+                    if (kNorm) {
+                        layernorm_rows<sizeof(OutT) == 2, kC, 4>(*reinterpret_cast<const float2(*)[4][NV]>(&xn[kStageRows * p + r4]), gv, bv, yv);
+                    } else {
+#pragma unroll
+                        for (int k = 0; k < 4; ++k)
+#pragma unroll
+                            for (int i = 0; i < NV; ++i) yv[k][i] = xn[kStageRows * p + r4 + k][i];
+                    }
+#pragma unroll
+                    for (int k = 0; k < 4; ++k) {
+                        const int r = kStageRows * p + r4 + k, gr = wrow0 + r;
+                        if (decltype(full)::value || gr < a.M) {
+                            float2* xr = (float2*)(a.x + (size_t)gr * kC);
+#pragma unroll
+                            for (int i = 0; i < NV; ++i) {
+                                xr[lane + 64 * i] = xn[r][i];
+                                store_row_pair<OutT>(y + (size_t)gr * kC, lane + 64 * i, yv[k][i].x, yv[k][i].y);
+                            }
+                        }
+                    }
+                }
+                __syncthreads();
+            }
+        };
+        if (wrow0 + 32 <= a.M) rows_out(std::true_type()); else rows_out(std::false_type());
+        return;
+    }
     if (row < a.M) {
         float* xr = a.x + (size_t)row * kC + 4 * hf;
 #pragma unroll
@@ -281,32 +367,56 @@
     return DIMX_OK;
 }
 
-int launch_mlp_fused(float* x, const void* packed, const float* b2, const float* ln_g, const float* ln_b, int M, int C, int F, int act,
-                     hipStream_t s) {
+int launch_mlp_fused_y(float* x, const void* packed, const float* b2, const float* ln_g, const float* ln_b, int M, int C, int F, int act,
+                       int y_mode, int y_dtype, void* y, const float* g2, const float* bt2, hipStream_t s) {
     DIMX_REQUIRE(x && packed && b2 && ln_g && M > 0, DIMX_ERR_ARG, "mlp_fused: null argument");
     DIMX_REQUIRE(C == kC && F % 32 == 0 && (act == ACT_GELU_TANH || act == ACT_GELU_ERF), DIMX_ERR_ARG, "mlp_fused: C = %d F = %d act = %d", C, F, act);
     DIMX_REQUIRE(((uintptr_t)x % 16) == 0 && ((uintptr_t)packed % 16) == 0 && ((uintptr_t)b2 % 16) == 0 && ((uintptr_t)ln_g % 16) == 0 &&
                      (!ln_b || ((uintptr_t)ln_b % 16) == 0),
                  DIMX_ERR_ARG, "mlp_fused: operands must be 16-byte aligned");
+    DIMX_REQUIRE(y_mode >= 0 && y_mode <= 2, DIMX_ERR_ARG, "mlp_fused: y_mode = %d", y_mode);
+    if (y_mode) {
+        DIMX_REQUIRE(y && y != (void*)x && (y_dtype == DIMX_BF16 || y_dtype == DIMX_F32) && (y_mode == 2 || g2), DIMX_ERR_ARG,
+                     "mlp_fused: second output needs y (not x), a dtype and, for the norm, its gamma");
+        DIMX_REQUIRE(((uintptr_t)y % 8) == 0 && (y_mode == 2 || (((uintptr_t)g2 % 8) == 0 && (!bt2 || ((uintptr_t)bt2 % 8) == 0))), DIMX_ERR_ARG,
+                     "mlp_fused: second output operands must be 8-byte aligned");
+    }
     MlpArgs a;
     a.x = x; a.wp = packed; a.b2 = b2; a.ln_g = ln_g; a.ln_b = ln_b; a.M = M; a.nchunk = F / 32;
+    a.y = y_mode ? y : nullptr; a.g2 = y_mode == 1 ? g2 : nullptr; a.bt2 = y_mode == 1 ? bt2 : nullptr;
+    const int ym = y_mode == 0 ? 0 : (y_mode == 1 ? 1 : 3) + (y_dtype == DIMX_BF16 ? 0 : 1);
     DIMX_REQUIRE(a.nchunk >= 3, DIMX_ERR_ARG, "mlp_fused: F = %d is too small for the three-deep pipeline", F);
     const size_t lds = (size_t)kStages * kChunkBytes;
+    static_assert((size_t)4 * kStageRows * kStageLd * 4 <= (size_t)kStages * kChunkBytes, "the epilogue stages rows in the weight rings");
     const dim3 grid((M + 127) / 128);
-#define MLP_LAUNCH(A, B)                                                                                                              \
+#define MLP_LAUNCH(A, B, Y)                                                                                                           \
     do {                                                                                                                              \
                              \
-        DIMX_HIP(hipFuncSetAttribute((const void*)mlp_fused_kernel<A, B>, hipFuncAttributeMaxDynamicSharedMemorySize, (int)lds)); \
-        hipLaunchKernelGGL((mlp_fused_kernel<A, B>), grid, dim3(256), lds, s, a);                                                     \
+        DIMX_HIP(hipFuncSetAttribute((const void*)mlp_fused_kernel<A, B, Y>, hipFuncAttributeMaxDynamicSharedMemorySize, (int)lds)); \
+        hipLaunchKernelGGL((mlp_fused_kernel<A, B, Y>), grid, dim3(256), lds, s, a);                                                  \
+    } while (0)
+#define MLP_LAUNCH_Y(A, B)                \
+    do {                                  \
+        if (ym == 0) MLP_LAUNCH(A, B, 0); \
+        else if (ym == 1) MLP_LAUNCH(A, B, 1); \
+        else if (ym == 2) MLP_LAUNCH(A, B, 2); \
+        else if (ym == 3) MLP_LAUNCH(A, B, 3); \
+        else MLP_LAUNCH(A, B, 4);         \
     } while (0)
     if (act == ACT_GELU_TANH) {
-        if (ln_b) MLP_LAUNCH(ACT_GELU_TANH, true); else MLP_LAUNCH(ACT_GELU_TANH, false);
+        if (ln_b) MLP_LAUNCH_Y(ACT_GELU_TANH, true); else MLP_LAUNCH_Y(ACT_GELU_TANH, false);
     } else {
-        if (ln_b) MLP_LAUNCH(ACT_GELU_ERF, true); else MLP_LAUNCH(ACT_GELU_ERF, false);
-    }
+        if (ln_b) MLP_LAUNCH_Y(ACT_GELU_ERF, true); else MLP_LAUNCH_Y(ACT_GELU_ERF, false);
+    }
+#undef MLP_LAUNCH_Y
 #undef MLP_LAUNCH
     DIMX_HIP(hipGetLastError());
     return DIMX_OK;
 }
 
-}
+int launch_mlp_fused(float* x, const void* packed, const float* b2, const float* ln_g, const float* ln_b, int M, int C, int F, int act,
+                     hipStream_t s) {
+    return launch_mlp_fused_y(x, packed, b2, ln_g, ln_b, M, C, F, act, 0, DIMX_F32, nullptr, nullptr, nullptr, s);
+}
+
+}
diff --git a/dyadic-interaction-modeling_amd/csrc/model.hip b/dyadic-interaction-modeling_amd/csrc/model.hip
--- a/dyadic-interaction-modeling_amd/csrc/model.hip
+++ b/dyadic-interaction-modeling_amd/csrc/model.hip
@@ -673,18 +673,39 @@
 
 constexpr int kFusedMlpMinRows = 8192;
 
+struct FfFollow {
+    int mode = 0;
+    int dtype = DIMX_F32;
+    void* y = nullptr;
+    const float* g = nullptr;
+    const float* b = nullptr;
+};
+static inline FfFollow follow_norm(int dtype, void* y, const float* g, const float* b) {
+    FfFollow f; f.mode = 1; f.dtype = dtype; f.y = y; f.g = g; f.b = b;
+    return f;
+}
+static inline FfFollow follow_cast(int dtype, void* y) {
+    FfFollow f; f.mode = 2; f.dtype = dtype; f.y = y;
+    return f;
+}
 static int ff_sublayer(const dimx_ctx* c, const BlockBufs& b, const float* ln_g, const float* ln_b, const Linear& f1,
-                       const Linear& f2, const void* mlp, int act, int M, int C, hipStream_t st) {
-    if (mlp && M >= kFusedMlpMinRows) return launch_mlp_fused(b.h, mlp, f2.bias, ln_g, ln_b, M, C, f1.N, act, st);
+                       const Linear& f2, const void* mlp, int act, int M, int C, hipStream_t st, const FfFollow& fo = FfFollow(),
+                       bool* y_done = nullptr) {
+    if (y_done) *y_done = false;
+    if (mlp && M >= kFusedMlpMinRows) {
+        const bool y2 = c->mlp_norm && fo.mode && y_done;
+        if (y2) *y_done = true;
+        return launch_mlp_fused_y(b.h, mlp, f2.bias, ln_g, ln_b, M, C, f1.N, act, y2 ? fo.mode : 0, fo.dtype, fo.y, fo.g, fo.b, st);
+    }
     DIMX_TRY(launch_layernorm(c->at, b.h, b.y, ln_g, ln_b, M, C, st));
     DIMX_TRY(linear(c, b.y, C, f1, M, c->at, b.f, f1.N, st, act));
     return residual_linear(c, b.f, f1.N, f2, M, b.h, C, st);
 }
 
 static int self_attn_qkv(const dimx_ctx* c, const BlockBufs& b, const float* ln_g, const float* ln_b, const Linear& qkv, int B,
-                         int T, int C, int heads, int D, AttnArgs& a, hipStream_t st) {
+                         int T, int C, int heads, int D, AttnArgs& a, hipStream_t st, bool have_y = false) {
     const bool rowv = qkv_row_v(c->at, D);
-    DIMX_TRY(launch_layernorm(c->at, b.h, b.y, ln_g, ln_b, B * T, C, st));
+    if (!have_y) DIMX_TRY(launch_layernorm(c->at, b.h, b.y, ln_g, ln_b, B * T, C, st));
     GemmArgs g;
     gemm_lin(c, b.y, C, qkv, B * T, g);
     g.out_dtype = c->at;
@@ -694,20 +715,29 @@
     return DIMX_OK;
 }
 
-static int attn_out(const dimx_ctx* c, const BlockBufs& b, AttnArgs& a, const Linear& out, int C, hipStream_t st) {
-    a.kwords = b.kw; a.kwords_cap = b.kw_cap;
+static int attn_out(const dimx_ctx* c, const BlockBufs& b, AttnArgs& a, const Linear& out, int C, hipStream_t st, bool kw_ready = false) {
+    a.kwords = b.kw; a.kwords_cap = b.kw_cap; a.kwords_ready = kw_ready ? 1 : 0;
     DIMX_TRY(launch_attention(a, st));
     return residual_linear(c, b.o, a.H * a.D, out, a.B * a.Lq, b.h, C, st);
 }
 
+static int pack_stack_key_words(const dimx_ctx* c, const BlockBufs& b, const uint8_t* mask, int mask_ld, int B, int Lk, int D,
+                                hipStream_t st, bool* ready) {
+    *ready = false;
+    if (!c->pack_kw_once || !mask || !b.kw || !qkv_row_v(c->at, D)) return DIMX_OK;
+    DIMX_TRY(launch_pack_key_words(mask, mask_ld, nullptr, B, Lk, b.kw, b.kw_cap, st));
+    *ready = true;
+    return DIMX_OK;
+}
+
 static int cross_attn_sublayer(const dimx_ctx* c, const BlockBufs& b, const XAttn& x, AttnArgs& a, const uint8_t* ctx_mask, int C,
-                               hipStream_t st, const float* v_rows = nullptr) {
+                               hipStream_t st, const float* v_rows = nullptr, bool kw_ready = false) {
     const int M = a.B * a.Lq, Tp = tpad(a.Lk);
     DIMX_TRY(launch_layernorm(c->at, b.h, b.y, x.ln_g, nullptr, M, C, st));
     DIMX_TRY(linear(c, b.y, C, x.qkv, M, c->at, b.q, a.H * a.D, st));
     if (v_rows) DIMX_TRY(launch_kv_rows_to_vt(v_rows, Tp, (float*)a.vt, Tp, a.B, a.Lk, a.H, st));
     a.scale = 1.0f / sqrtf((float)a.D); a.kmask = ctx_mask; a.kmask_ld = a.Lk;
-    return attn_out(c, b, a, x.out, C, st);
+    return attn_out(c, b, a, x.out, C, st, kw_ready);
 }
 
 struct VQScratch : BlockBufs {
@@ -734,17 +764,20 @@
 }
 
 static int run_vq_blocks(const dimx_ctx* c, const VQGeom& vg, const VQBlock* blk, VQScratch& s, int B, int T,
-                         const int32_t* lens, hipStream_t st) {
+                         const int32_t* lens, hipStream_t st, const FfFollow& last, bool* last_done) {
     const int M = B * T, Hd = vg.hidden, heads = vg.heads, D = Hd / heads;
     const float scale = 1.0f / sqrtf((float)Hd);
+    bool have_y = false;
     for (int l = 0; l < vg.layers; ++l) {
         const VQBlock& b = blk[l];
         AttnArgs a;
-        DIMX_TRY(self_attn_qkv(c, s, b.ln1_g, b.ln1_b, b.qkv, B, T, Hd, heads, D, a, st));
+        DIMX_TRY(self_attn_qkv(c, s, b.ln1_g, b.ln1_b, b.qkv, B, T, Hd, heads, D, a, st, have_y));
         a.scale = scale; a.lens = lens;
         DIMX_TRY(attn_out(c, s, a, b.out, Hd, st));
-        DIMX_TRY(ff_sublayer(c, s, b.ln2_g, b.ln2_b, b.l1, b.l2, b.mlp, ACT_GELU_TANH, M, Hd, st));
-    }
+        const FfFollow fo = l + 1 < vg.layers ? follow_norm(c->at, s.y, blk[l + 1].ln1_g, blk[l + 1].ln1_b) : last;
+        DIMX_TRY(ff_sublayer(c, s, b.ln2_g, b.ln2_b, b.l1, b.l2, b.mlp, ACT_GELU_TANH, M, Hd, st, fo, &have_y));
+    }
+    *last_done = have_y;
     return DIMX_OK;
 }
 
@@ -783,8 +816,9 @@
     DIMX_TRY(launch_cast_pad(c->at, x, vg.in_dim, nullptr, s.xa, vg.in_pad, M, vg.in_dim, st));
     DIMX_TRY(linear(c, s.xa, vg.in_pad, v.vm, M, c->at, s.h1, Hd, st, ACT_LEAKY));
     DIMX_TRY(run_vq_front(c, vg, s.h1, Hd, v.conv, v.le, v.pe_enc, pe_mode, row_off, s, B, T, lens, st));
-    DIMX_TRY(run_vq_blocks(c, vg, v.enc, s, B, T, lens, st));
-    DIMX_TRY(launch_cast_pad(c->at, s.h, Hd, nullptr, s.y, Hd, M, Hd, st));
+    bool cast_done = false;
+    DIMX_TRY(run_vq_blocks(c, vg, v.enc, s, B, T, lens, st, follow_cast(c->at, s.y), &cast_done));
+    if (!cast_done) DIMX_TRY(launch_cast_pad(c->at, s.h, Hd, nullptr, s.y, Hd, M, Hd, st));
     DIMX_TRY(linear(c, s.y, Hd, v.post, M, DIMX_F32, z, vg.out_dim, st));
     DIMX_TRY(launch_vq_argmin(z, M * vg.fqn, v.Et, v.ee, idx, nullptr, nullptr, st));
     return DIMX_OK;
@@ -870,6 +904,8 @@
     c->use_chain = (nc && nc[0] == '1') ? 0 : 1;
     c->use_layer_chain = getenv("DIMX_NO_LAYER_CHAIN") ? 0 : 1;
     c->multi_tr = getenv("DIMX_NO_MULTI_TR") ? 0 : 1;
+    c->mlp_norm = getenv("DIMX_NO_MLP_NORM") ? 0 : 1;
+    c->pack_kw_once = getenv("DIMX_NO_KW_ONCE") ? 0 : 1;
     c->use_qkv0_table = getenv("DIMX_NO_QKV0_TABLE") ? 0 : 1;
     c->use_kv0_table = getenv("DIMX_NO_KV0_TABLE") ? 0 : 1;
     if (getenv("DIMX_LAYER_PROF")) {
@@ -1258,14 +1294,18 @@
     g.rowadd_scale = 1.0f / sqrtf((float)dim);
     gemm_set_plain_out(g, s.h, dim);
     DIMX_TRY(launch_gemm(g, st));
+    bool kw_ready = false;
+    DIMX_TRY(pack_stack_key_words(c, s, mask, T, B, T, D, st, &kw_ready));
+    bool have_y = false;
     for (int l = 0; l < eg.depth; ++l) {
         AttnArgs a;
-        DIMX_TRY(self_attn_qkv(c, s, e.attn[l].ln_g, nullptr, e.attn[l].qkv, B, T, dim, heads, D, a, st));
+        DIMX_TRY(self_attn_qkv(c, s, e.attn[l].ln_g, nullptr, e.attn[l].qkv, B, T, dim, heads, D, a, st, have_y));
         a.scale = 1.0f / sqrtf((float)D); a.causal = eg.causal; a.kmask = mask; a.kmask_ld = T;
-        DIMX_TRY(attn_out(c, s, a, e.attn[l].out, dim, st));
-        DIMX_TRY(ff_sublayer(c, s, e.ff[l].ln_g, nullptr, e.ff[l].f1, e.ff[l].f2, e.ff[l].mlp, ACT_GELU_ERF, M, dim, st));
-    }
-    DIMX_TRY(launch_layernorm(out_dtype, s.h, out, e.final_g, nullptr, M, dim, st));
+        DIMX_TRY(attn_out(c, s, a, e.attn[l].out, dim, st, kw_ready));
+        const FfFollow fo = l + 1 < eg.depth ? follow_norm(c->at, s.y, e.attn[l + 1].ln_g, nullptr) : follow_norm(out_dtype, out, e.final_g, nullptr);
+        DIMX_TRY(ff_sublayer(c, s, e.ff[l].ln_g, nullptr, e.ff[l].f1, e.ff[l].f2, e.ff[l].mlp, ACT_GELU_ERF, M, dim, st, fo, &have_y));
+    }
+    if (!have_y) DIMX_TRY(launch_layernorm(out_dtype, s.h, out, e.final_g, nullptr, M, dim, st));
     return DIMX_OK;
 }
 
@@ -1445,8 +1485,9 @@
             DIMX_TRY(launch_cast_pad(h->at, z + r0 * zd, zd, nullptr, s.xa, zd, M, zd, gs));
         DIMX_TRY(linear(h, s.xa, zd, v.pre, M, h->at, s.h1, Hd, gs));
         DIMX_TRY(run_vq_front(h, vg, s.h1, Hd, v.dconv, v.dle, v.pe_dec, 1, batch_row_offset + b0, s, nb, L, nullptr, gs, rows_per_clip));
-        DIMX_TRY(run_vq_blocks(h, vg, v.dec, s, nb, L, nullptr, gs));
-        DIMX_TRY(launch_cast_pad(h->at, s.h, Hd, nullptr, s.y, Hd, M, Hd, gs));
+        bool cast_done = false;
+        DIMX_TRY(run_vq_blocks(h, vg, v.dec, s, nb, L, nullptr, gs, follow_cast(h->at, s.y), &cast_done));
+        if (!cast_done) DIMX_TRY(launch_cast_pad(h->at, s.h, Hd, nullptr, s.y, Hd, M, Hd, gs));
         DIMX_TRY(linear(h, s.y, Hd, v.rev, M, DIMX_F32, out + r0 * vg.in_dim, vg.in_dim, gs));
     }
     return DIMX_OK;
@@ -1519,9 +1560,8 @@
         DIMX_TRY(launch_cast_pad(h->at, v_speaker + r0 * h->d.dim_in, h->d.dim_in, h->patch_s, s.xa, 64, M, h->d.dim_in, gs));
         DIMX_TRY(run_xenc(h, h->encg[0], h->enc_s, s.xa, 64, s, nb, T, gmask, h->at, s.xa, gs));
         DIMX_TRY(run_xenc(h, h->encg[1], h->enc_joint, s.xa, dim, s, nb, T, gmask, DIMX_F32, s.tmp, gs));
-        float* x_s = x_s_out ? x_s_out + r0 * dim : (float*)s.h;
-        DIMX_TRY(launch_layernorm(DIMX_F32, s.tmp, x_s, h->norm_s_g, h->norm_s_b, M, dim, gs));
-        DIMX_TRY(launch_context_concat(h->at, x_s, h->patch_dec_s, v_audio + r0 * dim_a, s.xa, M, dim, dim_a, gs));
+        DIMX_TRY(launch_norm_context(h->at, s.tmp, h->norm_s_g, h->norm_s_b, x_s_out ? x_s_out + r0 * dim : nullptr, h->patch_dec_s,
+                                     v_audio + r0 * dim_a, s.xa, M, dim, dim_a, gs));
     }
     return DIMX_OK;
     }();
@@ -1728,11 +1768,13 @@
     DIMX_TRY(launch_shift_tokens(z_l, s.inp, s.tgt, B, T, st));
     DIMX_TRY(launch_gather_rows(DIMX_F32, h->dec.tok_emb, DD, V, s.inp, s.h, DD, M, DD, st));
     if (dg.abs_pos) DIMX_TRY(launch_add_pos_rows(s.h, h->dec.pos_emb, M, n, DD, 1.0f / sqrtf((float)DD), st));
+    bool kw_ready = false;
+    DIMX_TRY(pack_stack_key_words(h, s, kv_mask, n, B, n, D, st, &kw_ready));
     for (int l = 0; l < dg.depth; ++l) {
         AttnArgs a;
         DIMX_TRY(self_attn_qkv(h, s, h->dec.self_[l].ln_g, nullptr, h->dec.self_[l].qkv, B, n, DD, heads, D, a, st));
         a.scale = 1.0f / sqrtf((float)D); a.causal = 1; a.kmask = kv_mask; a.kmask_ld = n;
-        DIMX_TRY(attn_out(h, s, a, h->dec.self_[l].out, DD, st));
+        DIMX_TRY(attn_out(h, s, a, h->dec.self_[l].out, DD, st, kw_ready));
         set_attn_packed(a, h->at, s.q, cp.ck[l], cp.cv[l], s.o, B, heads, n, T, D, Tp);
         DIMX_TRY(cross_attn_sublayer(h, s, h->dec.cross[l], a, ctx_mask, DD, st));
         DIMX_TRY(ff_sublayer(h, s, h->dec.ff[l].ln_g, nullptr, h->dec.ff[l].f1, h->dec.ff[l].f2, nullptr, ACT_GELU_ERF, M, DD, st));
@@ -2139,6 +2181,8 @@
     DIMX_TRY(launch_prompt_rows(pr.tok, pr.ld, B, n0, V, S, s.inp, tokens, gen_steps(h, T), st));
     DIMX_TRY(launch_gather_rows(DIMX_F32, h->dec.tok_emb, DD, V, s.inp, s.h, DD, M, DD, st));
     const bool rowv = qkv_row_v(h->at, D);
+    bool kw_ready = false;
+    if (dg.depth > 1) DIMX_TRY(pack_stack_key_words(h, s, ctx_mask, T, B, T, D, st, &kw_ready));
     for (int l = 0; l < dg.depth; ++l) {
         AttnArgs a;
         DIMX_TRY(self_attn_qkv(h, s, h->dec.self_[l].ln_g, nullptr, h->dec.self_[l].qkv, B, n0, DD, heads, D, a, st));
@@ -2153,7 +2197,7 @@
         set_attn_packed(a, h->at, s.q, cp.ck[l], rowv ? cp.cv[l] : s.cvt, s.o, B, heads, n0, T, D, Tp, rowv);
         a.k_sb = (long)heads * Tp * D; a.k_sh = (long)Tp * D; a.k_st = D;
         if (rowv) { a.v_sb = a.k_sb; a.v_sh = a.k_sh; a.v_st = D; }
-        DIMX_TRY(cross_attn_sublayer(h, s, h->dec.cross[l], a, ctx_mask, DD, st, rowv ? nullptr : (const float*)cp.cv[l]));
+        DIMX_TRY(cross_attn_sublayer(h, s, h->dec.cross[l], a, ctx_mask, DD, st, rowv ? nullptr : (const float*)cp.cv[l], kw_ready));
         DIMX_TRY(ff_sublayer(h, s, h->dec.ff[l].ln_g, nullptr, h->dec.ff[l].f1, h->dec.ff[l].f2, nullptr, ACT_GELU_ERF, M, DD, st));
     }
     return DIMX_OK;
@@ -2902,6 +2946,12 @@
     return launch_mlp_fused(x, packed, b2, ln_g, ln_b, M, C, F, act, (hipStream_t)stream);
 }
 
+int dimx_op_mlp_fused_packed_y(float* x, const void* packed, const float* b2, const float* ln_g, const float* ln_b, int M, int C, int F,
+                               int act, int y_mode, int y_dtype, void* y, const float* g2, const float* bt2, void* stream) {
+    DIMX_REQUIRE(y_mode == 1 || y_mode == 2, DIMX_ERR_ARG, "op_mlp_fused_packed_y: y_mode must be 1 (LayerNorm) or 2 (cast)");
+    return launch_mlp_fused_y(x, packed, b2, ln_g, ln_b, M, C, F, act, y_mode, y_dtype, y, g2, bt2, (hipStream_t)stream);
+}
+
 int dimx_op_mlp_fused(float* x, const float* w1_host, const float* b1_host, const float* w2_host, const float* b2, const float* ln_g,
                       const float* ln_b, int M, int C, int F, int act, void* stream) {
     DIMX_REQUIRE(x && w1_host && w2_host && b2 && ln_g && M > 0, DIMX_ERR_ARG, "op_mlp_fused: null argument");
diff --git a/dyadic-interaction-modeling_amd/csrc/model.hpp b/dyadic-interaction-modeling_amd/csrc/model.hpp
--- a/dyadic-interaction-modeling_amd/csrc/model.hpp
+++ b/dyadic-interaction-modeling_amd/csrc/model.hpp
@@ -178,6 +178,8 @@
     int defer_ln = 1;
     unsigned long long* layer_prof_dev = nullptr;
     int multi_tr = 1;
+    int mlp_norm = 1;
+    int pack_kw_once = 1;
     int use_layer_chain = 1;
     unsigned* chain_err_dev = nullptr;
     unsigned* chain_err_host = nullptr;
diff --git a/dyadic-interaction-modeling_amd/csrc/norm.hip b/dyadic-interaction-modeling_amd/csrc/norm.hip
--- a/dyadic-interaction-modeling_amd/csrc/norm.hip
+++ b/dyadic-interaction-modeling_amd/csrc/norm.hip
@@ -14,38 +14,73 @@
     const float2* xr = (const float2*)(x + (size_t)row * C);
     const float2* g2 = (const float2*)gamma;
     const float2* b2 = (const float2*)beta;
-    float2 v[NV], gv[NV], bv[NV];
-    float s = 0.f;
-#pragma unroll
-    for (int i = 0; i < NV; ++i) {
-        v[i] = xr[lane + 64 * i];
-        s += v[i].x + v[i].y;
-    }
+    float2 v[NV], gv[NV], bv[NV], o[NV];
+#pragma unroll
+    for (int i = 0; i < NV; ++i) v[i] = xr[lane + 64 * i];
 #pragma unroll
     for (int i = 0; i < NV; ++i) {
         gv[i] = g2[lane + 64 * i];
         bv[i] = beta ? b2[lane + 64 * i] : make_float2(0.f, 0.f);
     }
-    const float mean = wave_sum_sel<sizeof(OutT) == 2>(s) * (1.0f / C);
-    float q = 0.f;
-#pragma unroll
-    for (int i = 0; i < NV; ++i) {
-        const float a = v[i].x - mean, b = v[i].y - mean;
-        q += a * a + b * b;
-    }
-    const float rstd = rsqrtf(wave_sum_sel<sizeof(OutT) == 2>(q) * (1.0f / C) + 1e-5f);
+    layernorm_row<sizeof(OutT) == 2, C>(v, gv, bv, o);
     OutT* yr = y + (size_t)row * C;
 #pragma unroll
-    for (int i = 0; i < NV; ++i) {
-        const int c2 = lane + 64 * i;
-        const float o0 = (v[i].x - mean) * rstd * gv[i].x + bv[i].x;
-        const float o1 = (v[i].y - mean) * rstd * gv[i].y + bv[i].y;
-        if (sizeof(OutT) == 2) {
-            *(uint32_t*)(yr + 2 * c2) = pack_bf16x2(o0, o1);
-        } else {
-            *(float2*)(yr + 2 * c2) = make_float2(o0, o1);
-        }
-    }
+    for (int i = 0; i < NV; ++i) store_row_pair<OutT>(yr, lane + 64 * i, o[i].x, o[i].y);
+}
+
+template <typename OutT, int C>
+__global__ __launch_bounds__(256) void norm_context_kernel(const float* __restrict__ x, const float* __restrict__ gamma,
+                                                           const float* __restrict__ beta, float* __restrict__ x_s_out,
+                                                           const float* __restrict__ patch, const float* __restrict__ audio,
+                                                           OutT* __restrict__ ctx, int M, int dim_a) {
+    constexpr int NV = C / 128;
+    const int row = blockIdx.x * 4 + (threadIdx.x >> 6);
+    const int lane = threadIdx.x & 63;
+    if (row >= M) return;
+    const float2* xr = (const float2*)(x + (size_t)row * C);
+    float2 v[NV], gv[NV], bv[NV], pv[NV], o[NV];
+#pragma unroll
+    for (int i = 0; i < NV; ++i) v[i] = xr[lane + 64 * i];
+#pragma unroll
+    for (int i = 0; i < NV; ++i) {
+        gv[i] = ((const float2*)gamma)[lane + 64 * i];
+        bv[i] = ((const float2*)beta)[lane + 64 * i];
+        pv[i] = ((const float2*)patch)[lane + 64 * i];
+    }
+    layernorm_row<false, C>(v, gv, bv, o);
+    OutT* cr = ctx + (size_t)row * (C + dim_a);
+#pragma unroll
+    for (int i = 0; i < NV; ++i) {
+        if (x_s_out) ((float2*)(x_s_out + (size_t)row * C))[lane + 64 * i] = o[i];
+        store_row_pair<OutT>(cr, lane + 64 * i, o[i].x + pv[i].x, o[i].y + pv[i].y);
+    }
+    const float2* ar = (const float2*)(audio + (size_t)row * dim_a);
+    for (int c2 = lane; c2 < dim_a / 2; c2 += 64) {
+        const float2 a = ar[c2];
+        store_row_pair<OutT>(cr + C, c2, a.x, a.y);
+    }
+}
+
+int launch_norm_context(int out_dtype, const float* x, const float* gamma, const float* beta, float* x_s_out, const float* patch,
+                        const float* audio, void* ctx, int M, int dim, int dim_a, hipStream_t s) {
+    DIMX_REQUIRE(x && gamma && beta && patch && audio && ctx && M > 0, DIMX_ERR_ARG, "norm_context: null operand");
+    DIMX_REQUIRE((dim == 384 || dim == 512 || dim == 768 || dim == 1152) && dim_a >= 0 && dim_a % 2 == 0, DIMX_ERR_ARG,
+                 "norm_context: dim=%d not in {384,512,768,1152} or dim_a=%d odd", dim, dim_a);
+    dim3 grid(ceil_div(M, 4)), block(256);
+#define NC_LAUNCH(OT, CC) \
+    hipLaunchKernelGGL((norm_context_kernel<OT, CC>), grid, block, 0, s, x, gamma, beta, x_s_out, patch, audio, (OT*)ctx, M, dim_a)
+#define NC_C(OT)                             \
+    do {                                     \
+        if (dim == 384) NC_LAUNCH(OT, 384);    \
+        else if (dim == 512) NC_LAUNCH(OT, 512); \
+        else if (dim == 768) NC_LAUNCH(OT, 768); \
+        else NC_LAUNCH(OT, 1152);            \
+    } while (0)
+    if (out_dtype == DIMX_BF16) NC_C(bf16); else NC_C(float);
+#undef NC_C
+#undef NC_LAUNCH
+    DIMX_HIP(hipGetLastError());
+    return DIMX_OK;
 }
 
 template <typename OutT, int C>
diff --git a/dyadic-interaction-modeling_amd/lib.py b/dyadic-interaction-modeling_amd/lib.py
--- a/dyadic-interaction-modeling_amd/lib.py
+++ b/dyadic-interaction-modeling_amd/lib.py
@@ -154,6 +154,8 @@
     "dimx_mlp_fused_packed_bytes": (c_size_t, [c_int, c_int]),
     "dimx_mlp_fused_pack": (c_int, [c_void_p, c_void_p, c_void_p, c_int, c_int, c_void_p, c_size_t]),
     "dimx_op_mlp_fused_packed": (c_int, [c_void_p, c_void_p, c_void_p, c_void_p, c_void_p, c_int, c_int, c_int, c_int, c_void_p]),
+    "dimx_op_mlp_fused_packed_y": (c_int, [c_void_p, c_void_p, c_void_p, c_void_p, c_void_p, c_int, c_int, c_int, c_int, c_int, c_int,
+                                           c_void_p, c_void_p, c_void_p, c_void_p]),
     "dimx_op_add_slabs_layernorm": (c_int, [c_int, c_void_p, c_void_p, c_int, ctypes.c_long, c_void_p, c_void_p, c_int,
                                             c_int, c_void_p]),
     "dimx_op_chain": (c_int, [c_void_p, c_int, c_void_p, c_void_p, c_void_p, c_int, c_void_p, c_void_p, c_void_p, c_int,
diff --git a/include/dimx.h b/include/dimx.h
--- a/include/dimx.h
+++ b/include/dimx.h
@@ -226,6 +226,8 @@
 int dimx_mlp_fused_pack(const float* w1_host, const float* b1_host, const float* w2_host, int C, int F, void* out_host, size_t out_bytes);
 int dimx_op_mlp_fused_packed(float* x, const void* packed, const float* b2, const float* ln_g, const float* ln_b, int M, int C, int F,
                              int act, void* stream);
+int dimx_op_mlp_fused_packed_y(float* x, const void* packed, const float* b2, const float* ln_g, const float* ln_b, int M, int C, int F,
+                               int act, int y_mode, int y_dtype, void* y, const float* g2, const float* bt2, void* stream);
 int dimx_op_add_slabs_layernorm(int out_dtype, float* x, const float* slabs, int nslab, long slab_stride, void* y,
                                 const float* gamma, int M, int C, void* stream);
 int dimx_op_chain(const void* A1, int K1, const void* W1, float* x, const float* slabs, int nslab, const float* gamma,
```

Result: no change. 1734 clips/s, median of 6 (+0.3%).
